# imkaywu/MVSKit

Hardware: AMD Instinct MI355X
Metric: patches/s (propagate+optim iteration), 12-view 1080p (higher is better)
Workload: dtype f32

## Files before the change

include/mvskit_engine.h:

```cpp
#ifndef MVSKIT_ENGINE_H
#define MVSKIT_ENGINE_H

#include <stddef.h>
#include <stdint.h>

#ifdef __cplusplus
extern "C" {
#endif

#ifndef MVS_MAX_IMAGES
#define MVS_MAX_IMAGES 32
#endif
#define MVS_LIST_CAP 16

typedef enum mvs_status {
    MVS_OK = 0,
    MVS_ERR_ARG = -1,
    MVS_ERR_STATE = -2,
    MVS_ERR_HIP = -3,
    MVS_ERR_CAPACITY = -4,
    MVS_ERR_NO_DEVICE = -5
} mvs_status;

typedef struct mvs_patch {
// ... 141 lines not shown
typedef struct mvs_fused_point {
    float xyz[3];
    float normal[3];
    float conf;
    uint8_t rgb[3];
    uint8_t view;
} mvs_fused_point;
int mvs_engine_fused_points(mvs_engine* e, const mvs_maps_config* c, int64_t cap, mvs_fused_point* out , int64_t* n);

typedef struct mvs_volume {
    float origin[3];
    float voxel;
    int32_t dims[3];
    float trunc;
    int32_t min_count;
    int32_t pad;
} mvs_volume;
int mvs_engine_tsdf(mvs_engine* e, const mvs_maps_config* c, const mvs_volume* vol, float* tsdf , int32_t* count );
int mvs_engine_extract_mesh(mvs_engine* e, const mvs_volume* vol, const float* tsdf, const int32_t* count , int64_t cap_v,
                            float* verts , int64_t cap_t, int32_t* tris , int64_t* n_v, int64_t* n_t);
int mvs_engine_mesh(mvs_engine* e, const mvs_maps_config* c, const mvs_volume* vol, int64_t cap_v, float* verts, int64_t cap_t, int32_t* tris,
                    int64_t* n_v, int64_t* n_t);

int mvs_engine_propagate(mvs_engine* e, int iter, mvs_counters* out);

int mvs_engine_filter(mvs_engine* e, int64_t* removed4);
typedef struct mvs_filter_stats {
    float outside_ms, exact_ms, neighbor_ms, groups_ms;
    float rebuild_ms;
    float total_ms;
    int64_t patches_in;
    int64_t exact_patches;
    int64_t exact_view_evals;
    int64_t neighbor_patches;
    int64_t neighbor_tasks;
    int64_t neighbor_entries;
    int64_t neighbor_visited;
    int64_t neighbor_accepted;
    int64_t neighbor_retried;
    int64_t exchange_bytes;
} mvs_filter_stats;
int mvs_engine_filter_stats(mvs_engine* e, mvs_filter_stats* out);

int mvs_engine_pass(mvs_engine* e, int iter, int pass, mvs_counters* out);
int mvs_engine_export_counts(mvs_engine* e, int64_t* n_new, int64_t* n_kill, int32_t* per_view_new );
int mvs_engine_export_device(mvs_engine* e, void* d_new_records, int64_t cap_new, void* d_kill_ids, int64_t cap_kill);
int mvs_engine_commit_device(mvs_engine* e, const void* d_new_records, int64_t n_new, const void* d_kill_ids, int64_t n_kill);
int mvs_engine_commit_local(mvs_engine* e);

#define MVS_COMM_ID_BYTES 128
int mvs_comm_unique_id(void* id_out );
int mvs_engine_comm_init(mvs_engine* e, const void* id , int rank, int world);
int mvs_engine_comm_attach(mvs_engine* e, void* nccl_comm , int rank, int world);
int mvs_engine_comm_release(mvs_engine* e);
int mvs_engine_exchange(mvs_engine* e);
int mvs_engine_comm_info(mvs_engine* e, int* rank, int* world, int* comm_count, int* comm_rank);

int mvs_engine_depth_normal_map(mvs_engine* e, int view, int kind, float* depth, float* normal, int32_t* ids);

typedef enum mvs_probe_op {
    MVS_PROBE_NCC = 0,
    MVS_PROBE_PREPROCESS = 1,
    MVS_PROBE_REFINE = 2,
    MVS_PROBE_POSTPROCESS = 3,
    MVS_PROBE_COST = 4,
    MVS_PROBE_MATH = 5,
    MVS_PROBE_REFINE_X = 6
} mvs_probe_op;
int mvs_engine_probe(mvs_engine* e, int op, int64_t n, const mvs_patch* in_rec, const float* in_f,
                     mvs_patch* out_rec, float* out_f, int32_t* out_i);

typedef struct mvs_timing {
    float index_ms;
    float sweep_ms;
    float commit_ms;
    int32_t sweep_launches;
    float exchange_ms;
    int32_t sweep_jobs_listed;
    int64_t exchange_bytes;
    int64_t check_retried_cells;
} mvs_timing;
int mvs_engine_last_timing(mvs_engine* e, mvs_timing* t);

#ifdef __cplusplus
}
#endif
#endif
```

mvskit_amd/csrc/mvs_device.cuh:

```cuda
#pragma once
#include <hip/hip_runtime.h>
#include <limits.h>
#include "mvs_types.h"

namespace mvsdev {

struct F3 { float x, y, z; };
struct F4 { float x, y, z, w; };

#define DEV __device__ __forceinline__

DEV int lane_id() { return (int)(threadIdx.x & 63u); }
DEV float fma_(float a, float b, float c) { return __builtin_fmaf(a, b, c); }
DEV int rli(int x, int l) { return __builtin_amdgcn_readlane(x, l); }
DEV float rlf(float x, int l) { return __int_as_float(__builtin_amdgcn_readlane(__float_as_int(x), l)); }
DEV int rfl(int x) { return __builtin_amdgcn_readfirstlane(x); }
DEV unsigned long long ballot(bool p) { return __ballot(p); }
#if MVS_LISTCAP > 32
typedef unsigned long long vmask_t;
DEV int vpop(vmask_t m) { return __popcll(m); }
#define MVS_VBITS 64
#else
typedef unsigned vmask_t;
DEV int vpop(vmask_t m) { return __popc(m); }
// ... 69 lines not shown
#define MVS_PIO4 0.78539816339744830962f
#define MVS_PI 3.14159265358979323846f
DEV float k_sinf(float x) {
    float z = x * x;
    float p = -1.9515295891e-4f * z + 8.3321608736e-3f;
    p = p * z - 1.6666654611e-1f;
    return x + x * z * p;
}
DEV float k_cosf(float x) {
    float z = x * x;
    float p = 2.443315711809948e-5f * z - 1.388731625493765e-3f;
    p = p * z + 4.166664568298827e-2f;
    return (1.0f - 0.5f * z) + z * z * p;
}
DEV float pm_sinf(float x) {
    float a = fabsf(x), r;
    if (a <= MVS_PIO4) r = k_sinf(a);
    else if (a <= 3.0f * MVS_PIO4) r = k_cosf((MVS_PIO2_HI - a) + MVS_PIO2_LO);
    else r = k_sinf(MVS_PI - a);
    return x < 0.0f ? -r : r;
}
DEV float pm_cosf(float x) {
    float a = fabsf(x);
    if (a <= MVS_PIO4) return k_cosf(a);
    if (a <= 3.0f * MVS_PIO4) return k_sinf((MVS_PIO2_HI - a) + MVS_PIO2_LO);
    return -k_cosf(MVS_PI - a);
}
DEV void pm_sincosf(float x, float& s, float& c) {
    const float a = fabsf(x);
    const bool r0 = a <= MVS_PIO4, r1 = a <= 3.0f * MVS_PIO4;
    const float t = r0 ? a : (r1 ? (MVS_PIO2_HI - a) + MVS_PIO2_LO : MVS_PI - a);
    const float ks = k_sinf(t), kc = k_cosf(t);
    const float sr = (r0 || !r1) ? ks : kc;
    s = x < 0.0f ? -sr : sr;
    c = r0 ? kc : (r1 ? ks : -kc);
}
DEV float pm_asinf(float x) {
    float a = fabsf(x);
    if (a > 1.0f) a = 1.0f;
    float z, xx;
    bool flag = a > 0.5f;
    if (flag) { z = 0.5f * (1.0f - a); xx = sqrt_rn(z); }
    else { z = a * a; xx = a; }
    float p = 4.2163199048e-2f * z + 2.4181311049e-2f;
    p = p * z + 4.5470025998e-2f;
    p = p * z + 7.4953002686e-2f;
    p = p * z + 1.6666752422e-1f;
    float r = p * z * xx + xx;
    if (flag) { r = r + r; r = (MVS_PIO2_HI - r) + MVS_PIO2_LO; }
    return x < 0.0f ? -r : r;
}
DEV float pm_acosf(float x) {
    if (x < -0.5f) return MVS_PI - 2.0f * pm_asinf(sqrt_rn(0.5f * (1.0f + x)));
    if (x > 0.5f) return 2.0f * pm_asinf(sqrt_rn(0.5f * (1.0f - x)));
    return MVS_PIO2_HI - pm_asinf(x);
}
DEV float pm_atanf(float v) {
    float x = fabsf(v), y;
    if (x > 2.414213562373095f) { y = MVS_PIO2_HI; x = -(1.0f / x); }
    else if (x > 0.4142135623730950f) { y = MVS_PIO4; x = (x - 1.0f) / (x + 1.0f); }
    else y = 0.0f;
    float z = x * x;
    float p = 8.05374449538e-2f * z - 1.38776856032e-1f;
    p = p * z + 1.99777106478e-1f;
    p = p * z - 3.33329491539e-1f;
    y = y + (p * z * x + x);
    return v < 0.0f ? -y : y;
}

DEV uint32_t mix32(uint32_t h) {
    h ^= h >> 16; h *= 0x7feb352du; h ^= h >> 15; h *= 0x846ca68bu; h ^= h >> 16;
    return h;
}
DEV float rng_uniform(uint32_t seed, uint32_t a, uint32_t b, uint32_t c, uint32_t d, uint32_t e) {
    uint32_t h = mix32(seed ^ 0x9e3779b9u);
    h = mix32(h ^ a) + 0x85ebca6bu;
    h = mix32(h ^ b) + 0xc2b2ae35u;
    h = mix32(h ^ c) + 0x27d4eb2fu;
    h = mix32(h ^ d) + 0x165667b1u;
    h = mix32(h ^ e);
    return (float)(h >> 8) * (1.0f / 16777216.0f) - 0.5f;
}

DEV F3 project(const DView* vw, F4 X, int level) {
    const float* P = vw->P[level];
    float r0 = fma_(P[3], X.w, fma_(P[2], X.z, fma_(P[1], X.y, P[0] * X.x)));
    float r1 = fma_(P[7], X.w, fma_(P[6], X.z, fma_(P[5], X.y, P[4] * X.x)));
    float r2 = fma_(P[11], X.w, fma_(P[10], X.z, fma_(P[9], X.y, P[8] * X.x)));
    if (r2 <= 0.0f) return {-65535.0f, -65535.0f, -1.0f};
    const float lo = (float)(INT_MIN + 3.0f), hi = (float)(INT_MAX - 3.0f);
    const float inv = rcp_rn(r2);
    F3 ic{r0 * inv, r1 * inv, 1.0f};
    ic.x = fmaxf(lo, fminf(hi, ic.x));
    ic.y = fmaxf(lo, fminf(hi, ic.y));
    return ic;
}
DEV F3 project_regs(const float (&P)[12], F4 X) {
    const float r0 = fma_(P[3], X.w, fma_(P[2], X.z, fma_(P[1], X.y, P[0] * X.x)));
    const float r1 = fma_(P[7], X.w, fma_(P[6], X.z, fma_(P[5], X.y, P[4] * X.x)));
    const float r2 = fma_(P[11], X.w, fma_(P[10], X.z, fma_(P[9], X.y, P[8] * X.x)));
    const float lo = (float)(INT_MIN + 3.0f), hi = (float)(INT_MAX - 3.0f);
    const float inv = rcp_rn(r2);
    F3 ic{fmaxf(lo, fminf(hi, r0 * inv)), fmaxf(lo, fminf(hi, r1 * inv)), 1.0f};
    if (r2 <= 0.0f) ic = {-65535.0f, -65535.0f, -1.0f};
    return ic;
}
DEV void load_P(const DView* vw, int level, float (&P)[12]) {
#pragma unroll
    for (int k = 0; k < 12; ++k) P[k] = vw->P[level][k];
}
DEV F4 unproject(const DView* vw, F3 ic, int level) {
    const float* P = vw->P[level];
    const float* M = vw->Minv;
    F3 b{ic.x - P[3], ic.y - P[7], ic.z - P[11]};
    return {fma_(M[2], b.z, fma_(M[1], b.y, M[0] * b.x)), fma_(M[5], b.z, fma_(M[4], b.y, M[3] * b.x)),
            fma_(M[8], b.z, fma_(M[7], b.y, M[6] * b.x)), 1.0f};
}
DEV float get_unit(const DParams& prm, const DView* vw, F4 coord) {
    const float fz = norm4(sub4(coord, ld4(vw->center)));
    const float ips = vw->ipscale;
    if (ips == 0.0f) return 1.0f;
    return div_rn(2.0f * fz * (float)(1 << prm.level), ips);
}
DEV void cell_of(const DParams& prm, const DView* vw, F4 coord, int& ix, int& iy) {
    float P[12];
    load_P(vw, prm.level, P);
    const F3 ic = project_regs(P, coord);
    ix = ((int)floorf(ic.x + 0.5f)) / prm.csize;
    iy = ((int)floorf(ic.y + 0.5f)) / prm.csize;
}
template <int LANE> DEV float row_bcast_f(float x) {
    return __int_as_float(__builtin_amdgcn_update_dpp(0, __float_as_int(x), 0x150 + LANE, 0xf, 0xf, false));
}
DEV void get_paxes(const DParams& prm, const DView* vw, F4 coord, F4 normal, F4& px, F4& py) {
    const F4 ctr = ld4(vw->center);
    const float ips = vw->ipscale;
    const F3 xax = ld3(vw->xaxis);
    float P[12];
    load_P(vw, prm.level, P);
    float pscale = 1.0f;
    if (ips != 0.0f) pscale = div_rn(2.0f * norm4(sub4(coord, ctr)) * (float)(1 << prm.level), ips);
    F3 n3{normal.x, normal.y, normal.z};
    F3 y3 = cross3(n3, xax);
    y3 = nrm3(y3);
    F3 x3 = cross3(y3, n3);
    px = {x3.x * pscale, x3.y * pscale, x3.z * pscale, 0.0f};
    py = {y3.x * pscale, y3.y * pscale, y3.z * pscale, 0.0f};
    const int j = lane_id() & 15;
    const float a = j == 1 ? 1.0f : 0.0f, b = j == 2 ? 1.0f : 0.0f;
    const F4 X{fma_(b, py.x, fma_(a, px.x, coord.x)), fma_(b, py.y, fma_(a, px.y, coord.y)), fma_(b, py.z, fma_(a, px.z, coord.z)), coord.w};
    const F3 ic = project_regs(P, X);
    const F3 c0{row_bcast_f<0>(ic.x), row_bcast_f<0>(ic.y), row_bcast_f<0>(ic.z)};
    const float inv = rcp_rn(norm3(sub3(ic, c0)));
    px = scl4(px, row_bcast_f<1>(inv));
    py = scl4(py, row_bcast_f<2>(inv));
}
DEV float robustincc(float incc) { return div_rn(incc, 1 + 3 * incc); }
DEV float unrobustincc(float r) { return div_rn(r, 1 - 3 * r); }

struct Frame {
    float tlx, tly, dxx, dxy, dyx, dyy;
    int w;
    int ok;
    unsigned img_lo, img_hi;
};
DEV int level_diff(const DParams& prm, float ratio) {
    static_assert(0x3504F3 == (0x3FB504F3 & 0x7FFFFF), "mantissa of 1.414213562373095f");
    const int k = ((__float_as_int(ratio) + (0x800000 - 0x3504F3)) >> 23) - 127;
    const int ld = max(-4, min(2, k));
    return max(-prm.level, min(2, ld));
}
DEV float pow2_level(int ld) { return __int_as_float((127 + ld) << 23); }
DEV Frame make_frame(const DParams& prm, F4 coord, F4 px, F4 py, F4 pz, int v, bool active) {
    const DView* vw = prm.views + (active ? v : 0);
    const F4 ctr = ld4(vw->center);
    float P[12];
#pragma unroll
    for (int k = 0; k < 12; ++k) P[k] = vw->P[prm.level][k];
    const int W0 = vw->W[0], H0 = vw->H[0];
    const unsigned long long base_level = (unsigned long long)vw->img[prm.level];
    const F4 ray = nrm4(sub4(ctr, coord));
    const float weight = fmaxf(0.0f, dot4(ray, pz));
    F3 center = project_regs(P, coord);
    F3 dx = sub3(project_regs(P, add4(coord, px)), center);
    F3 dy = sub3(project_regs(P, add4(coord, py)), center);
    const float ratio = (norm3(dx) + norm3(dy)) / 2.0f;
    const int ld = level_diff(prm, ratio);
    const float iscale = pow2_level(-ld);
    const int newLevel = prm.level + ld;
    const unsigned long long base_new = (unsigned long long)vw->img[newLevel];
    center = scl3(center, iscale);
    dx = scl3(dx, iscale);
    dy = scl3(dy, iscale);
    const float m = (float)(prm.wsize / 2);
    const float ax = dx.x * m, bx = dy.x * m, ay = dx.y * m, by = dy.y * m;
    const float tlx = (center.x - ax) - bx, tly = (center.y - ay) - by;
    const float minx = (center.x - fabsf(ax)) - fabsf(bx), maxx = (center.x + fabsf(ax)) + fabsf(bx);
    const float miny = (center.y - fabsf(ay)) - fabsf(by), maxy = (center.y + fabsf(ay)) + fabsf(by);
    const int margin2 = 2;
    const int W = W0 >> newLevel, H = H0 >> newLevel;
    const bool inside = !(minx < margin2 || W - 1 - margin2 <= maxx || miny < margin2 || H - 1 - margin2 <= maxy);
    const bool ok = active && !(weight < prm.cosAngle1) && inside;
    Frame f;
    f.tlx = ok ? tlx : 0.0f; f.tly = ok ? tly : 0.0f;
    f.dxx = ok ? dx.x : 0.0f; f.dxy = ok ? dx.y : 0.0f; f.dyx = ok ? dy.x : 0.0f; f.dyy = ok ? dy.y : 0.0f;
    f.w = ok ? W : (W0 >> prm.level);
    f.ok = ok ? 1 : 0;
    const unsigned long long a = ok ? base_new : base_level;
    f.img_lo = (unsigned)(a & 0xffffffffull); f.img_hi = (unsigned)(a >> 32);
    return f;
}

struct __attribute__((packed, aligned(4))) Texel2 { uint32_t a, b; };

struct ClsConst {
    unsigned cs[3];
    int fb;
    int xbase, nx;
};
struct WaveCtx {
    int lane;
    ClsConst cc;
    unsigned evals, view_evals;
#ifdef MVS_STAGE_TIMING
    unsigned long long st_acc[8];
    unsigned long long st_t;
#endif
};
#ifdef MVS_STAGE_TIMING
#define WC_T0(wc) { (wc).st_t = (unsigned long long)__builtin_amdgcn_s_memtime(); }
#define WC_ADD(wc, k) { const unsigned long long t1_ = (unsigned long long)__builtin_amdgcn_s_memtime(); (wc).st_acc[k] += t1_ - (wc).st_t; (wc).st_t = t1_; }
#else
#define WC_T0(wc)
#define WC_ADD(wc, k)
#endif

#define MVS_PIVOT_LDS4 192
#define MVS_FRAME_LDS_BYTES (64 * 48 + 16 * 16)
// ... 73 lines not shown
#define MVS_ROW_STEP(x, C) x = x + dpp_f<C>(x);
#define MVS_ROW_STEP5(C) { const float t0 = dpp0_f<C>(s1r), t1 = dpp0_f<C>(s1g), t2 = dpp0_f<C>(s1b), t3 = dpp0_f<C>(s2), t4 = dpp0_f<C>(s01); \
                           s1r = s1r + t0; s1g = s1g + t1; s1b = s1b + t2; s2 = s2 + t3; s01 = s01 + t4; }
#define MVS_ROW_STEP4(C) { const float t0 = dpp0_f<C>(s1r), t1 = dpp0_f<C>(s1g), t2 = dpp0_f<C>(s1b), t3 = dpp0_f<C>(s2); \
                           s1r = s1r + t0; s1g = s1g + t1; s1b = s1b + t2; s2 = s2 + t3; }
DEV void eval_steps4(const DParams& prm, WaveCtx& wc, const ClsConst& cc, const Frame& f, int n, unsigned (&okm)[4], float& incc_l) {
    frames_publish(wc, f, 64);
    const unsigned long long okb = ballot(f.ok != 0);
#pragma unroll
    for (int g = 0; g < 4; ++g) okm[g] = (unsigned)((okb >> (16 * g)) & 0xffffull);
#pragma unroll
    for (int g = 0; g < 4; ++g) wc.view_evals += (okm[g] & 1u) ? (unsigned)__popc(okm[g]) : 0u;
    const int fb = cc.fb;
    const int lc = wc.lane & 15;
    float c0[3][3];
    ClsPend pend[3];
    float P1r, P1g, P1b, P2, P01 = 0.0f;
    const int vlast = max(n - 1, 0);
    {
        const ClsFrame fr = cls_frame(fb);
#pragma unroll
        for (int j = 0; j < 3; ++j) pend[j] = cls_issue(fr, cls_opaque(cc.cs[j]));
    }
    {
        const float4 pv = mvs_dyn_lds4[MVS_PIVOT_LDS4];
        const ClsFrame fn = cls_frame(fb + min(1, vlast));
        float s1r = 0.0f, s1g = 0.0f, s1b = 0.0f, s2 = 0.0f;
#pragma unroll
        for (int j = 0; j < 3; ++j) {
            const unsigned cs = cls_opaque(cc.cs[j]);
            float r, g, b;
            cls_colour(pend[j], cs, pv.x, pv.y, pv.z, r, g, b);
            pend[j] = cls_issue(fn, cs);
            c0[j][0] = r; c0[j][1] = g; c0[j][2] = b;
            s1r += r; s1g += g; s1b += b;
            s2 = fma_(r, r, s2); s2 = fma_(g, g, s2); s2 = fma_(b, b, s2);
        }
        MVS_ROW_STEP4(0xB1) MVS_ROW_STEP4(0x4E) MVS_ROW_STEP4(0x141) MVS_ROW_STEP4(0x140)
        P1r = s1r; P1g = s1g; P1b = s1b; P2 = s2;
    }
    for (int k = 1; k < n; ++k) {
        const float4 pv = mvs_dyn_lds4[MVS_PIVOT_LDS4 + k];
        const ClsFrame fn = cls_frame(fb + min(k + 1, vlast));
        float s1r = 0.0f, s1g = 0.0f, s1b = 0.0f, s2 = 0.0f, s01 = 0.0f;
#pragma unroll
        for (int j = 0; j < 3; ++j) {
            const unsigned cs = cls_opaque(cc.cs[j]);
            float r, g, b;
            cls_colour(pend[j], cs, pv.x, pv.y, pv.z, r, g, b);
            pend[j] = cls_issue(fn, cs);
            s1r += r; s1g += g; s1b += b;
            s2 = fma_(r, r, s2); s2 = fma_(g, g, s2); s2 = fma_(b, b, s2);
            s01 = fma_(r, c0[j][0], s01); s01 = fma_(g, c0[j][1], s01); s01 = fma_(b, c0[j][2], s01);
        }
        MVS_ROW_STEP5(0xB1) MVS_ROW_STEP5(0x4E) MVS_ROW_STEP5(0x141) MVS_ROW_STEP5(0x140)
        if (lc == k) { P1r = s1r; P1g = s1g; P1b = s1b; P2 = s2; P01 = s01; }
    }
    const int a0 = (wc.lane & 48) << 2;
    if (cc.nx > 0) {
        const float4 pv = mvs_dyn_lds4[MVS_PIVOT_LDS4 + lc];
        ClsFrame fr;
        fr.tlx = f.tlx; fr.tly = f.tly; fr.dxx = f.dxx; fr.dxy = f.dxy; fr.dyx = f.dyx; fr.dyy = f.dyy; fr.w = f.w;
        fr.base = ((unsigned long long)f.img_hi << 32) | (unsigned long long)f.img_lo;
        {
            const int q = cc.xbase;
            const unsigned cs = (unsigned)(q % prm.wsize) | ((unsigned)(q / prm.wsize) << 8) | (1u << 16);
            const ClsPend pe = cls_issue(fr, cs);
            float r, g, b;
            cls_colour(pe, cs, pv.x, pv.y, pv.z, r, g, b);
            const float r0 = bperm_f(a0, r), g0 = bperm_f(a0, g), b0 = bperm_f(a0, b);
            P1r += r; P1g += g; P1b += b;
            P2 = fma_(r, r, P2); P2 = fma_(g, g, P2); P2 = fma_(b, b, P2);
            P01 = fma_(r, r0, P01); P01 = fma_(g, g0, P01); P01 = fma_(b, b0, P01);
        }
    }
    const float m_r = P1r * prm.inv_sz, m_g = P1g * prm.inv_sz, m_b = P1b * prm.inv_sz;
    const float ssd = fmaxf(P2 - fma_(P1b, m_b, fma_(P1g, m_g, P1r * m_r)), 0.0f);
    const float inv_l = inv_msd(prm, ssd);
    const float m0r = bperm_f(a0, m_r), m0g = bperm_f(a0, m_g), m0b = bperm_f(a0, m_b), inv0 = bperm_f(a0, inv_l);
    const float dot = P01 - fma_(P1b, m0b, fma_(P1g, m0g, P1r * m0r));
    incc_l = 1.0f - (dot * (inv0 * inv_l)) * prm.inv_3sz;
}

DEV void cls_raw(const ClsPend& p, unsigned cs, float& r, float& g, float& b) {
    const Texel2 q0 = p.q0, q1 = p.q1;
    const float fm = cvt_ub2(cs);
    const float dx1 = p.dx1 * fm, dx0 = fm - dx1, dy1 = p.dy1, dy0 = 1.0f - dy1;
    const float f00 = dx0 * dy0, f01 = dx0 * dy1, f10 = dx1 * dy0, f11 = dx1 * dy1;
    r = fma_((float)(q1.b & 255u), f11, fma_((float)(q0.b & 255u), f10, fma_((float)(q1.a & 255u), f01, (float)(q0.a & 255u) * f00)));
    g = fma_((float)((q1.b >> 8) & 255u), f11, fma_((float)((q0.b >> 8) & 255u), f10, fma_((float)((q1.a >> 8) & 255u), f01, (float)((q0.a >> 8) & 255u) * f00)));
    b = fma_((float)((q1.b >> 16) & 255u), f11, fma_((float)((q0.b >> 16) & 255u), f10, fma_((float)((q1.a >> 16) & 255u), f01, (float)((q0.a >> 16) & 255u) * f00)));
}
#define MVS_ROW_STEP3(C) { const float t0 = dpp0_f<C>(s1r), t1 = dpp0_f<C>(s1g), t2 = dpp0_f<C>(s1b); s1r = s1r + t0; s1g = s1g + t1; s1b = s1b + t2; }
#define MVS_ROW_STEP2(C) { const float t0 = dpp0_f<C>(sq), t1 = dpp0_f<C>(dt); sq = sq + t0; dt = dt + t1; }

#define MVS_PAIR_MFMA (MVS_LISTCAP > 16)
#if MVS_PAIR_MFMA
#define MVS_GRAM_SCRATCH (MVS_LISTCAP > 32 ? 2 : 1)
#define MVS_GRAM_CH 16
#define MVS_GRAM_NCH (MVS_LISTCAP / 16)
#define MVS_GRAM_NT (MVS_GRAM_NCH * (MVS_GRAM_NCH + 1) / 2)
#define MVS_GRAM_KSP 40
#define MVS_GRAM_T(p, c) ((c) * ((c) + 1) / 2 + (p))
#define MVS_GRAM_KK 4
#define MVS_GRAM_KS ((147 + MVS_GRAM_KK - 1) / MVS_GRAM_KK)
#define MVS_GRAM_NACC 4
typedef float gram_acc_t __attribute__((ext_vector_type(MVS_GRAM_NACC)));
DEV gram_acc_t gram_mfma(float a, float b, gram_acc_t c) { return __builtin_amdgcn_mfma_f32_16x16x4f32(a, b, c, 0, 0, 0); }
DEV int gram_col(int lane) { return lane & 15; }
DEV int gram_row(int lane, int r) { return (lane >> 4) * 4 + r; }
template <int N> struct GramIC { static constexpr int value = N; };
#endif
template <bool PIV = false>
DEV void eval_views(const DParams& prm, WaveCtx& wc, const Frame& f, int n, vmask_t (&okm)[1], float& incc_l, float* piv = nullptr,
                    float* texs = nullptr, int tstride = 0, float* ssd_out = nullptr) {
#if MVS_PAIR_MFMA
#if MVS_GRAM_SCRATCH == 2
    float gops[MVS_GRAM_NCH * MVS_GRAM_KSP];
#elif MVS_GRAM_SCRATCH
    gram_acc_t gacc[MVS_GRAM_NT];
    float gops[(MVS_GRAM_NCH - 1) * MVS_GRAM_KSP];
#pragma unroll
    for (int q = 0; q < MVS_GRAM_NT; ++q)
#pragma unroll
        for (int r = 0; r < MVS_GRAM_NACC; ++r) gacc[q][r] = 0.0f;
#endif
    const int gK = 3 * prm.wsz, gtp = 3 * tstride;
    const int gk0 = wc.lane / MVS_GRAM_CH;
    const float* const grow = texs + (wc.lane & (MVS_GRAM_CH - 1)) * gtp;
#endif
    const ClsConst& cc = wc.cc;
    frames_publish(wc, f, MVS_LISTCAP > 16 ? MVS_LISTCAP : 16);
    okm[0] = vballot(f.ok != 0);
    wc.view_evals += (okm[0] & 1u) ? (unsigned)vpop(okm[0]) : 0u;
    const int row = wc.lane >> 4, lc = wc.lane & 15;
    float fxr = 0.0f, fxg = 0.0f, fxb = 0.0f;
    unsigned xcs = 0u;
    ClsPend pe;
    if (cc.nx > 0) {
        ClsFrame fr;
        fr.tlx = f.tlx; fr.tly = f.tly; fr.dxx = f.dxx; fr.dxy = f.dxy; fr.dyx = f.dyx; fr.dyy = f.dyy; fr.w = f.w;
        fr.base = ((unsigned long long)f.img_hi << 32) | (unsigned long long)f.img_lo;
        xcs = (unsigned)(cc.xbase % prm.wsize) | ((unsigned)(cc.xbase / prm.wsize) << 8) | (1u << 16);
        pe = cls_issue(fr, xcs);
    }
    float d0[3][3], d0x[3] = {0.0f, 0.0f, 0.0f};
    float ssd_l = 1.0f, dot_l = 0.0f, mr_l = 128.0f, mg_l = 128.0f, mb_l = 128.0f;
    ClsPend pend[3];
    {
        const int last = max(n - 1, 0);
        const ClsFrame fr = cls_frame(min(row, last));
#pragma unroll
        for (int j = 0; j < 3; ++j) pend[j] = cls_issue(fr, cls_opaque(cc.cs[j]));
    }
    if (cc.nx > 0) cls_raw(pe, xcs, fxr, fxg, fxb);
    const int rounds = (n + 3) >> 2;
    auto round_body = [&](const int t) {
        const int v = 4 * t + row, vq = min(v, max(n - 1, 0));
        const ClsFrame fn = cls_frame(min(v + 4, max(n - 1, 0)));
        float cr[3], cg[3], cb[3];
        float s1r = 0.0f, s1g = 0.0f, s1b = 0.0f;
#pragma unroll
        for (int j = 0; j < 3; ++j) {
            const unsigned cs = cls_opaque(cc.cs[j]);
            cls_raw(pend[j], cs, cr[j], cg[j], cb[j]);
            pend[j] = cls_issue(fn, cs);
// ... 491 lines not shown
    float incc_l;
    fv[1] = fv[2] = fv[3] = 2.0;
    if (four) {
        wc.evals += (unsigned)__popc(rows);
        unsigned okm[4];
        eval_steps4(prm, wc, *cc, f, sz, okm, incc_l);
        const float val_l = robustincc(incc_l);
        const int gl = wc.lane & 3;
        const unsigned okl = gl == 1 ? okm[1] : (gl == 2 ? okm[2] : (gl == 3 ? okm[3] : okm[0]));
        double num = 0.0;
        int den = 0;
        for (int i = 1; i < sz; ++i) {
            const float v = bperm_f(4 * (16 * gl + i), val_l);
            const bool ok = (okl >> i) & 1u;
            num = ok ? num + (double)v : num;
            den += ok ? 1 : 0;
        }
        const double q = num / (double)den;
#pragma unroll
        for (int j = 0; j < 4; ++j) fv[j] = ((okm[j] & 1u) && rli(den, j) >= minimum - 1) ? rld(q, j) : 2.0;
    } else {
        wc.evals += 1;
        vmask_t okm[1];
        if (piv) eval_views<true>(prm, wc, f, sz, okm, incc_l, piv);
        else eval_views(prm, wc, f, sz, okm, incc_l);
        const float val_l = robustincc(incc_l);
        fv[0] = cost_of_group(prm, wc, (unsigned)okm[0], val_l, 0, sz, minimum);
    }
}
DEV void refine_patch(const DParams& prm, WaveCtx& wc, Cand& c, uint32_t k0, uint32_t k1, uint32_t k2, uint32_t k3, float* w_out = nullptr) {
    RefineCtx rc;
    rc.center = c.coord;
    rc.ref = rli(c.img, 0);
    rc.ray = nrm4(sub4(c.coord, ld4((prm.views + rc.ref)->center)));
    rc.dscale = c.dscale;
    rc.ascale = prm.ascaleConst;
    const float w = compute_weights(prm, wc, c.coord, c.normal, c.img, c.nimg);
    const int imgx = __shfl(c.img, wc.lane & 15);
    float x[3];
    encode(prm, rc, c.coord, c.normal, x);
    const float amin = -23.99999f, amax = 23.99999f;
    x[1] = fmaxf(fminf(x[1], amax), amin);
    x[2] = fmaxf(fminf(x[2], amax), amin);
    float bx0 = x[0], bx1 = x[1], bx2 = x[2];
    double fv[4];
    float piv[3] = {128.0f, 128.0f, 128.0f};
    cost_func4(prm, wc, rc, imgx, c.nimg, false, bx0, bx1, bx2, fv, piv);
    __syncthreads();
    if (wc.lane < 16) mvs_dyn_lds4[MVS_PIVOT_LDS4 + wc.lane] = make_float4(piv[0], piv[1], piv[2], 0.0f);
    __syncthreads();
    double fbest = fv[0];
    const ClsConst cc = wc.cc;
    float rd = prm.rd0, ra = prm.ra0;
    const int g = wc.lane >> 4;
    const uint32_t gj = (uint32_t)min(g, 2);
    for (int k = 0; k < prm.refine_steps; ++k) {
        const uint32_t draw = 16u + ((uint32_t)(k * 3) + gj) * 3u;
        const float u0 = 2.0f * rng_uniform(prm.seed, k0, k1, k2, k3, draw + 0);
        const float u1 = 2.0f * rng_uniform(prm.seed, k0, k1, k2, k3, draw + 1);
        const float u2 = 2.0f * rng_uniform(prm.seed, k0, k1, k2, k3, draw + 2);
        float cx0 = (gj == 1u) ? bx0 : fma_(u0, rd, bx0);
        float cx1 = (gj == 0u) ? bx1 : fmaxf(fminf(fma_(u1, ra, bx1), amax), amin);
        float cx2 = (gj == 0u) ? bx2 : fmaxf(fminf(fma_(u2, ra, bx2), amax), amin);
        if (g == 3) {
            cx0 = bx0 - (cx0 - bx0);
            cx1 = fmaxf(fminf(bx1 - (cx1 - bx1), amax), amin);
            cx2 = fmaxf(fminf(bx2 - (cx2 - bx2), amax), amin);
        }
        cost_func4(prm, wc, rc, imgx, c.nimg, true, cx0, cx1, cx2, fv, nullptr, &cc);
        int jb = 0;
        double fstep = fv[0];
#pragma unroll
        for (int j = 1; j < 4; ++j) if (fv[j] < fstep) { fstep = fv[j]; jb = j; }
        if (fstep < fbest) { fbest = fstep; bx0 = rlf(cx0, 16 * jb); bx1 = rlf(cx1, 16 * jb); bx2 = rlf(cx2, 16 * jb); }
        rd *= 0.5f; ra *= 0.5f;
    }
    x[0] = bx0; x[1] = bx1; x[2] = bx2;
    decode(prm, rc, x[0], x[1], x[2], c.coord, c.normal);
    c.normal.w = 0.0f;
    if (w_out) *w_out = w;
    else c.ncc = 1.0f - unrobustincc(compute_incc(prm, wc, c.coord, c.normal, c.img, c.nimg, w, 1));
}

DEV int refine_patch_simplex(const DParams& prm, WaveCtx& wc, Cand& c, int max_evals, float xtol, float* w_out = nullptr,
                               float* x_out = nullptr, double* f_out = nullptr) {
    RefineCtx rc;
    rc.center = c.coord;
    rc.ref = rli(c.img, 0);
    rc.ray = nrm4(sub4(c.coord, ld4((prm.views + rc.ref)->center)));
    rc.dscale = c.dscale;
    rc.ascale = prm.ascaleConst;
    const float w = compute_weights(prm, wc, c.coord, c.normal, c.img, c.nimg);
    const int imgx = __shfl(c.img, wc.lane & 15);
    float x[3];
    encode(prm, rc, c.coord, c.normal, x);
    const float amin = -23.99999f, amax = 23.99999f;
    x[1] = fmaxf(fminf(x[1], amax), amin);
    x[2] = fmaxf(fminf(x[2], amax), amin);
    double fv[4];
    float piv[3] = {128.0f, 128.0f, 128.0f};
    cost_func4(prm, wc, rc, imgx, c.nimg, false, x[0], x[1], x[2], fv, piv);
    __syncthreads();
    if (wc.lane < 16) mvs_dyn_lds4[MVS_PIVOT_LDS4 + wc.lane] = make_float4(piv[0], piv[1], piv[2], 0.0f);
    __syncthreads();
    const double f0 = fv[0];
    const ClsConst cc = wc.cc;
    const int g = wc.lane >> 4;
    float vx0 = g == 1 ? x[0] + prm.rd0 : x[0];
    float vx1 = g == 2 ? fmaxf(fminf(x[1] + prm.ra0, amax), amin) : x[1];
    float vx2 = g == 3 ? fmaxf(fminf(x[2] + prm.ra0, amax), amin) : x[2];
    cost_func4(prm, wc, rc, imgx, c.nimg, true, vx0, vx1, vx2, fv, nullptr, &cc, 0xEu);
    double vf = g == 0 ? f0 : (g == 1 ? fv[1] : (g == 2 ? fv[2] : fv[3]));
    int evals = 4;
    bool ok = false;
    int b = 0;
    for (;;) {
        double f[4];
#pragma unroll
        for (int j = 0; j < 4; ++j) f[j] = rld(vf, 16 * j);
        b = 0;
        int wv = 0;
#pragma unroll
        for (int j = 1; j < 4; ++j) {
            if (f[j] < (b == 1 ? f[1] : (b == 2 ? f[2] : f[0]))) b = j;
            if (f[j] >= (wv == 1 ? f[1] : (wv == 2 ? f[2] : f[0]))) wv = j;
        }
        const float b0 = rlf(vx0, 16 * b), b1 = rlf(vx1, 16 * b), b2 = rlf(vx2, 16 * b);
        {
            float lo0 = rlf(vx0, 0), hi0 = lo0, lo1 = rlf(vx1, 0), hi1 = lo1, lo2 = rlf(vx2, 0), hi2 = lo2;
#pragma unroll
            for (int j = 1; j < 4; ++j) {
                const float a0 = rlf(vx0, 16 * j), a1 = rlf(vx1, 16 * j), a2 = rlf(vx2, 16 * j);
                lo0 = fminf(lo0, a0); hi0 = fmaxf(hi0, a0);
                lo1 = fminf(lo1, a1); hi1 = fmaxf(hi1, a1);
                lo2 = fminf(lo2, a2); hi2 = fmaxf(hi2, a2);
            }
            if (hi0 - lo0 <= xtol * fmaxf(1.0f, fabsf(b0)) && hi1 - lo1 <= xtol * fmaxf(1.0f, fabsf(b1)) &&
                hi2 - lo2 <= xtol * fmaxf(1.0f, fabsf(b2))) { ok = true; break; }
        }
        if (evals + 4 > max_evals) break;
        const double fb = rld(vf, 16 * b), fw = rld(vf, 16 * wv);
        double fsw = wv == 0 ? f[1] : f[0];
#pragma unroll
        for (int j = 0; j < 4; ++j) if (j != wv) fsw = fmax(fsw, f[j]);
        const int r0 = wv == 0 ? 1 : 0, r1 = wv <= 1 ? 2 : 1, r2 = wv <= 2 ? 3 : 2;
        const float c0 = ((rlf(vx0, 16 * r0) + rlf(vx0, 16 * r1)) + rlf(vx0, 16 * r2)) / 3.0f;
        const float c1 = ((rlf(vx1, 16 * r0) + rlf(vx1, 16 * r1)) + rlf(vx1, 16 * r2)) / 3.0f;
        const float c2 = ((rlf(vx2, 16 * r0) + rlf(vx2, 16 * r1)) + rlf(vx2, 16 * r2)) / 3.0f;
        const float d0 = c0 - rlf(vx0, 16 * wv), d1 = c1 - rlf(vx1, 16 * wv), d2 = c2 - rlf(vx2, 16 * wv);
        const float k = g == 0 ? 1.0f : (g == 1 ? 2.0f : (g == 2 ? 0.5f : -0.5f));
        const float t0 = c0 + k * d0;
        const float t1 = fmaxf(fminf(c1 + k * d1, amax), amin);
        const float t2 = fmaxf(fminf(c2 + k * d2, amax), amin);
        cost_func4(prm, wc, rc, imgx, c.nimg, true, t0, t1, t2, fv, nullptr, &cc);
        evals += 4;
        int acc = -1;
        if (fv[0] < fb) acc = fv[1] < fv[0] ? 1 : 0;
        else if (fv[0] < fsw) acc = 0;
        else if (fv[0] < fw) acc = fv[2] <= fv[0] ? 2 : -1;
        else acc = fv[3] < fw ? 3 : -1;
        if (acc >= 0) {
            const float a0 = rlf(t0, 16 * acc), a1 = rlf(t1, 16 * acc), a2 = rlf(t2, 16 * acc);
            const double fa = acc == 0 ? fv[0] : (acc == 1 ? fv[1] : (acc == 2 ? fv[2] : fv[3]));
            if (g == wv) { vx0 = a0; vx1 = a1; vx2 = a2; vf = fa; }
            continue;
        }
// ... 288 lines not shown
```

mvskit_amd/csrc/mvs_engine.cpp:

```cpp
#include <hip/hip_runtime.h>
#include <dlfcn.h>
#include <rccl/rccl.h>

#include <algorithm>
#include <climits>
#include <cmath>
#include <cstdio>
#include <cstdlib>
#include <cstring>
#include <string>
#include <vector>

#include "mvskit_engine.h"
#include "mvs_kernels.h"
#include "mvs_types.h"

static_assert(sizeof(mvs_patch) == sizeof(DPatch), "mvs_patch and DPatch must be the same bytes");
static_assert((MVS_LISTCAP == 16 || MVS_LISTCAP == 32 || MVS_LISTCAP == 64) && MVS_LISTCAP <= MVS_MAXI && MVS_MAX_IMAGES == MVS_MAXI, "limits out of sync");

namespace {
thread_local std::string g_err;

#define HIPCHK(expr)                                                                                       \
    do {                                                                                                   \
// ... 89 lines not shown
    MVS_SYM(GroupEnd, "ncclGroupEnd"); MVS_SYM(GetErrorString, "ncclGetErrorString");
    MVS_SYM(CommCount, "ncclCommCount"); MVS_SYM(CommUserRank, "ncclCommUserRank");
#undef MVS_SYM
    r.ok = r.GetUniqueId && r.CommInitRank && r.CommDestroy && r.AllGather && r.Broadcast && r.GroupStart && r.GroupEnd && r.GetErrorString;
    return r;
}
#define NCCLCHK(expr)                                                                                      \
    do {                                                                                                   \
        ncclResult_t _r = (expr);                                                                          \
        if (_r != ncclSuccess) {                                                                           \
            g_err = std::string(#expr) + ": " + rccl().GetErrorString(_r);                                 \
            return MVS_ERR_HIP;                                                                            \
        }                                                                                                  \
    } while (0)

struct Roctx {
    int (*push)(const char*) = nullptr;
    int (*pop)() = nullptr;
};
Roctx& roctx() {
    static Roctx r;
    static bool tried = false;
    if (tried) return r;
    tried = true;
    void* h = nullptr;
    const char* names[] = {"libroctx64.so", "libroctx64.so.4", "/opt/rocm/lib/libroctx64.so.4"};
    for (const char* n : names) if (!h) h = dlopen(n, RTLD_NOW | RTLD_NOLOAD);
    for (const char* n : names) if (!h) h = dlopen(n, RTLD_NOW | RTLD_LOCAL);
    if (!h) return r;
    r.push = reinterpret_cast<int (*)(const char*)>(dlsym(h, "roctxRangePushA"));
    r.pop = reinterpret_cast<int (*)()>(dlsym(h, "roctxRangePop"));
    if (!r.push || !r.pop) { r.push = nullptr; r.pop = nullptr; }
    return r;
}
struct Range {
    bool on;
    explicit Range(const char* name) : on(roctx().push != nullptr) { if (on) roctx().push(name); }
    ~Range() { if (on) roctx().pop(); }
    Range(const Range&) = delete;
    Range& operator=(const Range&) = delete;
};
}

struct mvs_engine {
    mvs_config cfg{};
    mvs_refiner refiner{MVS_REFINE_HALVING, 500, 1e-4f};
    DParams prm{};
    hipStream_t stream = nullptr;
    bool have_views = false;
    std::vector<DView> hviews;
    DevBuf<DView> dviews;
    std::vector<DevBuf<uint32_t>> img_bufs;
    std::vector<DevBuf<uint8_t>> mask_bufs;
    int total_cells = 0;
    DevBuf<DPatch> pool, pool_alt;
    DevBuf<uint8_t> kill;
    int64_t pool_n = 0;
    bool ncc_dirty = false;
    DevBuf<int32_t> cnt, cursor, vcnt, vcursor;
    DevBuf<csr_off_t> start, vstart;
    DevBuf<csr_off_t> start_raw;
    DevBuf<int32_t> id32_raw;
    DevBuf<int64_t> scan_tmp;
    DevBuf<unsigned long long> ids;
    DevBuf<ListKey> key;
    DevBuf<int32_t> id32, vid32;
    DevBuf<int32_t> uf_parent, uf_size;
    DevBuf<int32_t> group_edges;
    DevBuf<int32_t> cnt_alive, vcnt_alive;
    DevBuf<unsigned long long> dpgrid, best;
    DevBuf<uint32_t> dirty;
    bool dirty_marked = false;
    DevBuf<float4> geo;
    DevBuf<uint8_t> geo_ref;
    bool geo_valid = false;
    bool lists_dense[2] = {false, false};
    DevBuf<DPatch> staging;
    DevBuf<int32_t> job_stage, job_nstage, job_cnt, job_base_scan, kill_cnt, kill_base;
    DevBuf<unsigned long long> misc;
    DevBuf<DCounters> counters;
    DevBuf<int32_t> error_flag;
    DevBuf<int32_t> big_tables, retry_jobs;
    DevBuf<int32_t> job_list;
    int64_t retried_cells = 0;
    int64_t pass_retried = 0;
    SweepArgs sa{};
    bool staged = false;
    bool counted = false;
    int64_t n_new = 0, n_kill = 0;
    std::vector<int32_t> h_per_view;
    DevBuf<DPatch> tmp_rec_in, tmp_rec_out;
    DevBuf<float> tmp_f_in, tmp_f_out;
    DevBuf<int32_t> tmp_i;
    DevBuf<uint8_t> tmp_bytes;
    hipEvent_t ev[6] = {nullptr, nullptr, nullptr, nullptr, nullptr, nullptr};
    mvs_timing timing{};
    mvs_filter_stats fstats{};
    int64_t fstats_exchange_bytes = 0;
    DevBuf<unsigned long long> fstat_buf;
    hipEvent_t fev[10] = {nullptr, nullptr, nullptr, nullptr, nullptr, nullptr, nullptr, nullptr, nullptr, nullptr};
    ncclComm_t comm = nullptr;
    bool comm_owned = false;
    int comm_rank = 0, comm_world = 1;
    DevBuf<int64_t> comm_counts;
    DevBuf<int32_t> comm_kill_ids;
    int pass_status = MVS_OK;
    std::string pass_error;
    bool fault_fired = false;
};

namespace {

RefineSel refine_sel(const mvs_engine* e) {
    return RefineSel{e->refiner.mode == MVS_REFINE_CONVERGED ? 1 : 0, e->refiner.max_evals, e->refiner.xtol};
}

void derive_params(mvs_engine* e) {
    const mvs_config& c = e->cfg;
    DParams& p = e->prm;
    p.nviews = c.nviews; p.level = c.level; p.csize = c.csize; p.wsize = c.wsize; p.wsz = c.wsize * c.wsize;
    p.minImageNum = c.minImageNum;
    p.tau = std::min(c.minImageNum * 2, c.nviews);
    p.max_propag = c.max_propag;
    p.cap = c.max_propag * c.csize * c.csize;
    p.depth = c.depth; p.enable_check = c.enable_check; p.view_propagation = c.view_propagation ? 1 : 0;
    p.seed = c.seed; p.refine_steps = c.refine_steps; p.rd0 = c.refine_rd0; p.ra0 = c.refine_ra0;
    p.nccThreshold = c.nccThreshold;
    p.nccThresholdBefore = c.nccThreshold - 0.3f;
    volatile float a0 = (float)(60.0f * M_PI / 180.0f), a1 = (float)(60.0f * M_PI / 180.0f);
    volatile double amin = (double)c.maxAngleThreshold, amax = (double)a1;
    volatile float typo = (float)(120.0f / M_PI * 180.0f);
    volatile double d120 = 120.0f * M_PI / 180.0f, d10 = 10.0f * M_PI / 180.0f;
    p.cosAngle0 = cosf(a0);
    p.cosAngle1 = cosf(a1);
    p.cosMinAngle = (float)cos(amin);
    p.cosMaxAngle = (float)cos(amax);
    p.cosNeighborTypo = cosf(typo);
    p.cosNeighbor120 = (float)cos(d120);
    p.sortThreshold = (float)(1.0f - cos(d10));
    p.ascaleConst = (float)(M_PI / 48.0f);
    p.inv_sz = 1.0f / (float)(c.wsize * c.wsize);
    p.inv_3sz = 1.0f / (float)(3 * c.wsize * c.wsize);
    p.neighborThreshold = 0.5f; p.neighborThreshold1 = 1.0f;
    p.quadThreshold = c.quadThreshold;
    p.list_n = std::min<int>(MVS_LISTCAP, c.nviews);
    p.gram_ld = (p.list_n + 15) / 16 * 16;
}

void invert3(const float* P, float* Minv) {
    double a = P[0], b = P[1], c = P[2], d = P[4], e = P[5], f = P[6], g = P[8], h = P[9], i = P[10];
    double A = e * i - f * h, B = -(d * i - f * g), C = d * h - e * g;
    double det = a * A + b * B + c * C;
    double inv[9] = {A, -(b * i - c * h), b * f - c * e, B, a * i - c * g, -(a * f - c * d), C, -(a * h - b * g), a * e - b * d};
    for (int k = 0; k < 9; ++k) Minv[k] = (float)(inv[k] / det);
}
inline float hfma(float a, float b, float c) { return __builtin_fmaf(a, b, c); }
inline float hdot3(const float* a, const float* b) { return hfma(a[2], b[2], hfma(a[1], b[1], a[0] * b[0])); }
inline float hdot4(const float* a, const float* b) { return hfma(a[3], b[3], hfma(a[2], b[2], hfma(a[1], b[1], a[0] * b[0]))); }
inline void hcross(const float* a, const float* b, float* o) {
    o[0] = a[1] * b[2] - a[2] * b[1]; o[1] = a[2] * b[0] - a[0] * b[2]; o[2] = a[0] * b[1] - a[1] * b[0];
}

void setup_camera(const mvs_engine* e, DView& vw, const float* P0) {
    const int maxLevel = e->cfg.level + 3;
    for (int k = 0; k < 12; ++k) vw.P[0][k] = P0[k];
    for (int l = 1; l < maxLevel; ++l) {
// ... 1398 lines not shown
        a.sweep_views[a.nsweep_views] = v;
        a.job_base[a.nsweep_views] = (int32_t)nj;
        ++a.nsweep_views;
        nj += (int64_t)((e->hviews[v].gw + 1) / 2) * e->hviews[v].gh;
    }
    a.njobs = nj;
    a.job_lo = 0; a.job_hi = nj;
    if (ranged) {
        const int split_mode = getenv("MVS_SPLIT_PROXY") ? atoi(getenv("MVS_SPLIT_PROXY")) : 2;
        const int N = e->cfg.shard_count, R = e->cfg.shard_index;
        std::vector<int32_t> cuts(N + 1, -1);
        int64_t total_work = 0;
        if (split_mode > 0 && nj > 0) {
            const DParams p0 = current_params(e);
            int shift = 0;
            while ((((int64_t)3 * e->prm.cap * e->prm.max_propag * 32 * nj) >> shift) + nj >= (int64_t)INT32_MAX) ++shift;
            mvsk_job_work(p0, a, split_mode, shift, e->job_cnt.p, st);
            mvsk_exclusive_scan(e->job_cnt.p, e->job_base_scan.p, nj, reinterpret_cast<int32_t*>(e->scan_tmp.p), st);
            if (int r = e->tmp_i.ensure(N + 1)) return r;
            HIPCHK(hipMemsetAsync(e->tmp_i.p, 0xff, (size_t)(N + 1) * sizeof(int32_t), st));
            mvsk_job_cuts(e->job_base_scan.p, nj, N, e->tmp_i.p, st);
            int32_t tw = 0;
            HIPCHK(hipMemcpyAsync(cuts.data(), e->tmp_i.p, (size_t)(N + 1) * sizeof(int32_t), hipMemcpyDeviceToHost, st));
            HIPCHK(hipMemcpyAsync(&tw, e->job_base_scan.p + nj, sizeof tw, hipMemcpyDeviceToHost, st));
            HIPCHK(hipStreamSynchronize(st));
            total_work = tw;
        }
        cuts[0] = 0; cuts[N] = (int32_t)nj;
        for (int r = 1; r < N; ++r) {
            if (total_work <= 0 || cuts[r] < 0) cuts[r] = (int32_t)(nj * r / N);
            cuts[r] = std::max(cuts[r], cuts[r - 1]);
        }
        a.job_lo = cuts[R];
        a.job_hi = cuts[R + 1];
    }
    a.staging = e->staging.p; a.staging_cap = e->staging.cap;
    a.stage_counter = e->misc.p + misc::stage_counter;
    a.job_stage = e->job_stage.p; a.job_nstage = e->job_nstage.p;
    a.maxstage = (e->prm.view_propagation ? 3 : 2) * e->prm.cap * e->prm.max_propag;
    a.kill = e->kill.p;
    a.counters = e->counters.p;
    a.error_flag = e->error_flag.p;
    if (want_vgrid(e)) {
        if (int r = e->big_tables.ensure((int64_t)256 * 16384)) return r;
        if (int r = e->retry_jobs.ensure(std::max<int64_t>(nj, 16))) return r;
    }
    a.big_tables = e->big_tables.p; a.retry_jobs = e->retry_jobs.p; a.nretry = reinterpret_cast<int32_t*>(e->misc.p + misc::sweep_retry);
    HIPCHK(hipMemsetAsync(e->misc.p + misc::sweep_retry, 0, sizeof(unsigned long long), st));
    HIPCHK(hipMemsetAsync(e->misc.p + misc::stage_counter, 0, sizeof(unsigned long long), st));
    a.cursors = reinterpret_cast<uint32_t*>(e->misc.p + misc::sweep_cursors);
    HIPCHK(hipMemsetAsync(e->misc.p + misc::sweep_cursors, 0, (misc::sweep_cursor_words + misc::sweep_list_bound_words) * sizeof(unsigned long long), st));
    HIPCHK(hipMemsetAsync(e->counters.p, 0, MVS_COUNTER_SLOTS * sizeof(DCounters), st));
    HIPCHK(hipMemsetAsync(e->error_flag.p, 0, sizeof(int32_t), st));
    const DParams p = current_params(e);
    const RefineSel rs = refine_sel(e);
    if (int r = e->job_list.ensure(std::max<int64_t>(nj, 16))) return r;
    if (e->job_cnt.ensure(nj + misc::job_list_pad) || e->job_base_scan.ensure(nj + misc::job_list_pad)) return MVS_ERR_HIP;
    int32_t* list_bounds = reinterpret_cast<int32_t*>(e->misc.p + misc::sweep_list_bounds);
    a.job_list = e->job_list.p; a.list_bounds = list_bounds;
    mvsk_job_list(p, a, e->job_cnt.p, e->job_base_scan.p, reinterpret_cast<int32_t*>(e->scan_tmp.p), e->job_list.p, list_bounds, st);
    HIPCHK(hipEventRecord(e->ev[1], st));
    Range rg_sweep(pass & 1 ? "mvs:sweep colour 1" : "mvs:sweep colour 0");
    mvsk_sweep(p, a, rs, st);
    e->pass_retried = 0;
    if (want_vgrid(e)) {
        int32_t nretry = 0;
        HIPCHK(hipMemcpyAsync(&nretry, a.nretry, sizeof nretry, hipMemcpyDeviceToHost, st));
        HIPCHK(hipStreamSynchronize(st));
        e->pass_retried = nretry;
        if (nretry > 0) { mvsk_sweep_retry(p, a, nretry, rs, st); e->retried_cells += nretry; }
    }
    HIPCHK(hipEventRecord(e->ev[2], st));
    std::vector<DCounters> hcs(MVS_COUNTER_SLOTS);
    int32_t herr = 0;
    unsigned long long fill[2] = {0, 0};
    HIPCHK(hipMemcpyAsync(fill, e->misc.p + misc::fill_evals, sizeof fill, hipMemcpyDeviceToHost, st));
    HIPCHK(hipMemcpyAsync(hcs.data(), e->counters.p, hcs.size() * sizeof(DCounters), hipMemcpyDeviceToHost, st));
    HIPCHK(hipMemcpyAsync(&herr, e->error_flag.p, sizeof herr, hipMemcpyDeviceToHost, st));
    int32_t hbounds[MVS_SWEEP_QUEUES + 1];
    HIPCHK(hipMemcpyAsync(hbounds, list_bounds, sizeof hbounds, hipMemcpyDeviceToHost, st));
    HIPCHK(hipStreamSynchronize(st));
    HIPCHK(hipGetLastError());
    mvs_counters sum{};
    for (const DCounters& c : hcs) add_counters(sum, c);
    sum.evals += fill[0]; sum.view_evals += fill[1]; sum.trimmed = (int64_t)trimmed;
    float ms = 0.0f;
    (void)hipEventElapsedTime(&ms, e->ev[0], e->ev[1]); e->timing.index_ms = ms;
    (void)hipEventElapsedTime(&ms, e->ev[1], e->ev[2]); e->timing.sweep_ms = ms;
    e->timing.commit_ms = 0.0f; e->timing.sweep_launches = 1; e->timing.exchange_ms = 0.0f; e->timing.exchange_bytes = 0;
    e->timing.check_retried_cells = e->pass_retried;
    e->timing.sweep_jobs_listed = hbounds[MVS_SWEEP_QUEUES];
    e->staged = true; e->counted = false;
    if (out) *out = sum;
#ifdef MVS_JOBLIST_COUNTS
    fprintf(stderr, "[job list] iter %d colour %d: jobs %lld, with any source entry %llu, listed %llu\n", iter, pass & 1, (long long)(a.job_hi - a.job_lo),
            hcs[0].stage[0], hcs[0].stage[1]);
#endif
#ifdef MVS_STAGE_TIMING
    {
        unsigned long long stage[16] = {0};
        for (const DCounters& c : hcs)
            for (int k = 0; k < 16; ++k) stage[k] = (k == 12 || k == 13) ? std::max(stage[k], c.stage[k]) : stage[k] + c.stage[k];
        static const char* nm[8] = {"wave", "generate", "pre", "refine", "post", "check", "stage", "prologue"};
        fprintf(stderr, "[stage cycles]");
        for (int k = 0; k < 8; ++k) fprintf(stderr, " %s %.1f%%", nm[k], 100.0 * (double)stage[k] / (double)(stage[0] ? stage[0] : 1));
        static const char* nm2[4] = {"gain", "search", "sort", "quad"};
        for (int k = 0; k < 4; ++k) fprintf(stderr, " %s %.1f%%", nm2[k], 100.0 * (double)stage[8 + k] / (double)(stage[0] ? stage[0] : 1));
        fprintf(stderr, " setRefImage pairs %.1f%% choice %.1f%%", 100.0 * (double)stage[14] / (double)(stage[0] ? stage[0] : 1), 100.0 * (double)stage[15] / (double)(stage[0] ? stage[0] : 1));
        fprintf(stderr, "  (wave cycles %.3e; max visited %llu, max neighbours %llu)\n", (double)stage[0], stage[12], stage[13]);
    }
#endif
#ifdef MVS_FAULT_INJECTION
    if (const char* f = getenv("MVS_FAULT_PASS")) {
        int fr = -1, fi = -1, fp = -1;
        if (!e->fault_fired && sscanf(f, "%d:%d:%d", &fr, &fi, &fp) == 3 && fr == (e->cfg.shard_count > 1 ? e->cfg.shard_index : 0) && fi == iter && fp == pass) {
            e->fault_fired = true;
            g_err = "mvs_engine_pass: capacity failure injected by MVS_FAULT_PASS";
            return MVS_ERR_CAPACITY;
        }
    }
#endif
    if (herr & 3) { g_err = "mvs_engine_pass: staging capacity exceeded (raise mvs_config.max_patches)"; return MVS_ERR_CAPACITY; }
    if (herr & 4) {
        g_err = "mvs_engine_pass: Optim::check met more than 14336 patches around one patch, or more than 4064 neighbours (engine limit)";
        return MVS_ERR_CAPACITY;
    }
    return MVS_OK;
}

int mvs_engine_export_counts(mvs_engine* e, int64_t* n_new, int64_t* n_kill, int32_t* per_view_new) {
    if (!e || !e->staged) { g_err = "mvs_engine_export_counts: no pass to export"; return MVS_ERR_STATE; }
    HIPCHK(hipSetDevice(e->cfg.device));
    if (int r = ensure_counts(e)) return r;
    if (n_new) *n_new = e->n_new;
    if (n_kill) *n_kill = e->n_kill;
    if (per_view_new) for (int v = 0; v < e->cfg.nviews; ++v) per_view_new[v] = e->h_per_view[v];
    return MVS_OK;
}

int mvs_engine_export_device(mvs_engine* e, void* d_new, int64_t cap_new, void* d_kill, int64_t cap_kill) {
    if (!e || !e->staged) { g_err = "mvs_engine_export_device: no pass to export"; return MVS_ERR_STATE; }
    HIPCHK(hipSetDevice(e->cfg.device));
    if (int r = ensure_counts(e)) return r;
    if (e->n_new > cap_new || e->n_kill > cap_kill) { g_err = "mvs_engine_export_device: buffers too small"; return MVS_ERR_CAPACITY; }
    if (e->n_new > 0) mvsk_commit_copy(e->sa, e->job_base_scan.p, (DPatch*)d_new, cap_new, nullptr, 1, e->stream);
    if (e->n_kill > 0) mvsk_kill_export(e->kill.p, e->pool_n, e->kill_base.p, (int32_t*)d_kill, cap_kill, e->stream);
    HIPCHK(hipStreamSynchronize(e->stream));
    return MVS_OK;
}

int mvs_engine_commit_device(mvs_engine* e, const void* d_new, int64_t n_new, const void* d_kill, int64_t n_kill) {
    if (!e || !e->have_views) return MVS_ERR_STATE;
    HIPCHK(hipSetDevice(e->cfg.device));
    hipStream_t st = e->stream;
    if (e->pool_n + n_new > e->pool.cap) { g_err = "mvs_engine_commit_device: patch pool capacity exceeded (raise mvs_config.max_patches)"; return MVS_ERR_CAPACITY; }
    return commit_pool(e, [&](int64_t* added) -> int {
        mvsk_apply_kill_ids(e->pool.p, (const int32_t*)d_kill, n_kill, e->pool_n, st);
        mvsk_append_records(e->pool.p, e->pool_n, (const DPatch*)d_new, n_new, st);
        if (e->pool_n > 0) HIPCHK(hipMemsetAsync(e->kill.p, 0, (size_t)e->pool_n, st));
        *added = n_new;
        return MVS_OK;
    });
}

int mvs_engine_commit_local(mvs_engine* e) {
    if (!e || !e->staged) { g_err = "mvs_engine_commit_local: no pass to commit"; return MVS_ERR_STATE; }
    HIPCHK(hipSetDevice(e->cfg.device));
// ... 255 lines not shown
            if (fr.live()) mvsk_filter_neighbor_retry(current_params(e), e->kill.p, e->uf_parent.p, nr, e->error_flag.p, e->fstat_buf.p + fstat::neighbor_parts, st);
            FRHIP(hipGetLastError());
            FRHIP(hipEventRecord(e->fev[5], st));
#ifdef MVS_STAGE_TIMING
            if (fr.live()) {
                unsigned long long hc[16] = {0};
                (void)hipMemcpyAsync(hc, e->fstat_buf.p + fstat::neighbor_cycles, sizeof hc, hipMemcpyDeviceToHost, st);
                (void)hipStreamSynchronize(st);
                const double w = (double)(hc[0] ? hc[0] : 1);
                fprintf(stderr, "[filterNeighbor cycles] load + grids %.1f%% set build %.1f%% gather + predicate %.1f%% filterQuad %.1f%% (wave cycles %.3e)\n",
                        100.0 * hc[1] / w, 100.0 * hc[9] / w, 100.0 * hc[10] / w, 100.0 * hc[11] / w, (double)hc[0]);
            }
#endif
        }
        filter_fault_point(fr, 3);
        if (filter_exchange(fr, true, false)) break;
        FR(apply_kills(e, &rem[2], true));
        if (rem[2] > 0) { if (filter_rebuild(fr, 1, false, true, 2)) break; }
        {
            int64_t alive = 0;
            FR(mvs_engine_num_patches(e, &alive));
            FR(e->uf_parent.ensure(e->pool.cap));
            FR(e->uf_size.ensure(e->pool.cap));
            const int threshold = (int)std::max<int64_t>(20, alive / 10000);
            FRHIP(hipEventRecord(e->fev[6], st));
            if (fr.live()) {
                if (!e->cfg.literal_groups) mvsk_groups(current_params(e), e->uf_parent.p, e->uf_size.p, threshold, e->kill.p, st);
                else fr.note(literal_small_groups(e, threshold));
            }
            FRHIP(hipEventRecord(e->fev[7], st));
            FR(apply_kills(e, &rem[3], true));
        }
        if (rem[3] > 0) { if (filter_rebuild(fr, 1, false, false, 2)) break; }
        FR(compact_pool(e));
        FRHIP(hipMemcpyAsync(&herr, e->error_flag.p, sizeof herr, hipMemcpyDeviceToHost, st));
        FRHIP(hipEventRecord(e->ev[1], st));
        FRHIP(hipStreamSynchronize(st));
        FRHIP(hipGetLastError());
        if (fr.live() && (herr & 4)) {
            g_err = "mvs_engine_filter: more than 14336 patches around one patch, or more than 4064 neighbours (engine limit)";
            fr.note(MVS_ERR_CAPACITY);
        }
    } while (0);
    const int status = filter_agree(fr);
    e->geo_valid = false;
    if (status != MVS_OK) {
        const std::string keep = g_err;
        if (e->kill.p && e->pool_n > 0) (void)hipMemsetAsync(e->kill.p, 0, (size_t)e->pool_n, st);
        (void)hipStreamSynchronize(st);
        (void)hipGetLastError();
        e->dirty_marked = false;
        g_err = keep;
        return status;
    }
    float ms = 0.0f;
    (void)hipEventElapsedTime(&ms, e->ev[0], e->ev[1]);
    e->timing = mvs_timing{};
    e->timing.index_ms = ms;
    {
        mvs_filter_stats& f = e->fstats;
        f.total_ms = ms;
        (void)hipEventElapsedTime(&f.outside_ms, e->fev[0], e->fev[1]);
        (void)hipEventElapsedTime(&f.exact_ms, e->fev[2], e->fev[3]);
        (void)hipEventElapsedTime(&f.neighbor_ms, e->fev[4], e->fev[5]);
        (void)hipEventElapsedTime(&f.groups_ms, e->fev[6], e->fev[7]);
        f.rebuild_ms = f.total_ms - f.outside_ms - f.exact_ms - f.neighbor_ms - f.groups_ms;
        std::vector<unsigned long long> part(fstat::neighbor_cycles - fstat::neighbor_parts);
        HIPCHK(hipMemcpy(part.data(), e->fstat_buf.p + fstat::neighbor_parts, part.size() * sizeof(unsigned long long), hipMemcpyDeviceToHost));
        unsigned long long sum4[4] = {0, 0, 0, 0};
        for (size_t k = 0; k < part.size(); ++k) sum4[k & 3] += part[k];
        f.neighbor_tasks = (int64_t)sum4[0]; f.neighbor_entries = (int64_t)sum4[1]; f.neighbor_visited = (int64_t)sum4[2]; f.neighbor_accepted = (int64_t)sum4[3];
    }
    e->fstats.exchange_bytes = e->fstats_exchange_bytes;
    if (removed4) for (int k = 0; k < 4; ++k) removed4[k] = rem[k];
    return MVS_OK;
}

int mvs_engine_filter_stats(mvs_engine* e, mvs_filter_stats* out) {
    if (!e || !out) return MVS_ERR_ARG;
    *out = e->fstats;
    return MVS_OK;
}

int mvs_engine_last_timing(mvs_engine* e, mvs_timing* t) {
    if (!e || !t) return MVS_ERR_ARG;
    *t = e->timing;
    return MVS_OK;
}

int mvs_engine_depth_normal_map(mvs_engine* e, int view, int kind, float* depth, float* normal, int32_t* ids) {
    if (!e || !e->have_views || view < 0 || view >= e->cfg.nviews || kind < 0 || kind > 1) { g_err = "mvs_engine_depth_normal_map: bad argument"; return MVS_ERR_ARG; }
    HIPCHK(hipSetDevice(e->cfg.device));
    hipStream_t st = e->stream;
    const DView& vw = e->hviews[view];
    const int ncells = vw.gw * vw.gh;
    const DParams p = current_params(e);
    const unsigned long long* sel = nullptr;
    if (kind == 0) {
        HIPCHK(hipMemsetAsync(e->dpgrid.p, 0xff, (size_t)e->total_cells * sizeof(unsigned long long), st));
        mvsk_depth_maps(p, e->dpgrid.p, nullptr, st);
        sel = e->dpgrid.p + vw.cell_base;
    } else {
        HIPCHK(hipMemsetAsync(e->best.p, 0, (size_t)ncells * sizeof(unsigned long long), st));
        mvsk_best_ncc_map(p, view, e->best.p, st);
        sel = e->best.p;
    }
    if (e->tmp_f_out.ensure((int64_t)ncells * 4) || e->tmp_i.ensure(ncells)) return MVS_ERR_HIP;
    mvsk_map_extract(p, view, kind, sel, e->tmp_f_out.p, e->tmp_f_out.p + ncells, e->tmp_i.p, ncells, st);
    if (depth) HIPCHK(hipMemcpyAsync(depth, e->tmp_f_out.p, (size_t)ncells * sizeof(float), hipMemcpyDeviceToHost, st));
    if (normal) HIPCHK(hipMemcpyAsync(normal, e->tmp_f_out.p + ncells, (size_t)ncells * 3 * sizeof(float), hipMemcpyDeviceToHost, st));
    if (ids) HIPCHK(hipMemcpyAsync(ids, e->tmp_i.p, (size_t)ncells * sizeof(int32_t), hipMemcpyDeviceToHost, st));
    HIPCHK(hipStreamSynchronize(st));
    return MVS_OK;
}

int mvs_engine_probe(mvs_engine* e, int op, int64_t n, const mvs_patch* in_rec, const float* in_f, mvs_patch* out_rec, float* out_f, int32_t* out_i) {
    if (!e || !e->have_views || n < 0 || op < 0 || op > 6) { g_err = "mvs_engine_probe: bad argument / views not set"; return MVS_ERR_ARG; }
    const RefineSel rs = refine_sel(e);
    if (op == MVS_PROBE_REFINE_X && !rs.simplex) { g_err = "mvs_engine_probe: MVS_PROBE_REFINE_X needs the CONVERGED refiner"; return MVS_ERR_STATE; }
    if (n == 0) return MVS_OK;
    HIPCHK(hipSetDevice(e->cfg.device));
    hipStream_t st = e->stream;
    if (op == MVS_PROBE_POSTPROCESS && e->prm.depth > 0) if (int r = build_index(e, nullptr)) return r;
    const int64_t nf_out = op == MVS_PROBE_MATH ? 5 * n : ((op == MVS_PROBE_REFINE || op == MVS_PROBE_REFINE_X) && rs.simplex ? 4 * n : n);
    if (e->tmp_rec_in.ensure(n) || e->tmp_rec_out.ensure(n) || e->tmp_f_in.ensure(n) || e->tmp_f_out.ensure(nf_out) || e->tmp_i.ensure(n + 1)) return MVS_ERR_HIP;
    if (op == MVS_PROBE_MATH) {
        if (!in_f || !out_f) return MVS_ERR_ARG;
        HIPCHK(hipMemcpyAsync(e->tmp_f_in.p, in_f, (size_t)n * sizeof(float), hipMemcpyHostToDevice, st));
    } else {
        if (!in_rec) return MVS_ERR_ARG;
        HIPCHK(hipMemcpyAsync(e->tmp_rec_in.p, in_rec, (size_t)n * sizeof(mvs_patch), hipMemcpyHostToDevice, st));
    }
    HIPCHK(hipMemsetAsync(e->tmp_i.p, 0, (size_t)(n + 1) * sizeof(int32_t), st));
    const DParams p = current_params(e);
    mvsk_probe(p, op, n, e->tmp_rec_in.p, e->tmp_f_in.p, e->tmp_rec_out.p, e->tmp_f_out.p, e->tmp_i.p, rs, st);
    if (out_rec && (op == MVS_PROBE_PREPROCESS || op == MVS_PROBE_REFINE || op == MVS_PROBE_POSTPROCESS || op == MVS_PROBE_REFINE_X))
        HIPCHK(hipMemcpyAsync(out_rec, e->tmp_rec_out.p, (size_t)n * sizeof(mvs_patch), hipMemcpyDeviceToHost, st));
    if (out_f && (op == MVS_PROBE_NCC || op == MVS_PROBE_COST || op == MVS_PROBE_MATH || op == MVS_PROBE_REFINE_X))
        HIPCHK(hipMemcpyAsync(out_f, e->tmp_f_out.p, (size_t)nf_out * sizeof(float), hipMemcpyDeviceToHost, st));
    if (out_i) HIPCHK(hipMemcpyAsync(out_i, e->tmp_i.p, (size_t)n * sizeof(int32_t), hipMemcpyDeviceToHost, st));
    HIPCHK(hipStreamSynchronize(st));
    HIPCHK(hipGetLastError());
    return MVS_OK;
}

}
```

mvskit_amd/csrc/mvs_kernels.hip:

```cpp
#include <hip/hip_runtime.h>
#include <algorithm>
#include "mvs_device.cuh"
#include "mvs_check.cuh"
#include "mvs_kernels.h"

using namespace mvsdev;

__global__ void k_rgb_to_rgba(const uint8_t* __restrict__ rgb, uint32_t* __restrict__ out, int64_t n) {
    const int64_t i = (int64_t)blockIdx.x * blockDim.x + threadIdx.x;
    if (i >= n) return;
    const uint8_t* p = rgb + 3 * i;
    out[i] = (uint32_t)p[0] | ((uint32_t)p[1] << 8) | ((uint32_t)p[2] << 16);
}
__global__ void k_rgba_to_rgb(const uint32_t* __restrict__ in, uint8_t* __restrict__ rgb, int64_t n) {
    const int64_t i = (int64_t)blockIdx.x * blockDim.x + threadIdx.x;
    if (i >= n) return;
    const uint32_t t = in[i];
    rgb[3 * i] = t & 255u; rgb[3 * i + 1] = (t >> 8) & 255u; rgb[3 * i + 2] = (t >> 16) & 255u;
}
__global__ void k_pyr_down(const uint32_t* __restrict__ src, int pw, int ph, uint32_t* __restrict__ dst, int w, int h) {
    const int x = blockIdx.x * blockDim.x + threadIdx.x, y = blockIdx.y * blockDim.y + threadIdx.y;
    if (x >= w || y >= h) return;
    const float base[4] = {1.0f, 3.0f, 3.0f, 1.0f};
    float c0 = 0.0f, c1 = 0.0f, c2 = 0.0f;
// ... 327 lines not shown
}
__global__ void k_job_work(DParams prm, SweepArgs a, int mode, int shift, int32_t* __restrict__ work) {
    const int64_t job = (int64_t)blockIdx.x * blockDim.x + threadIdx.x;
    if (job >= a.njobs) return;
    int dest;
    const int n = job_trial_sources(prm, a, job, &dest);
    int w = 0;
    if (dest >= 0) {
        if (mode == 1) w = n;
        else {
            const int trials = n * prm.max_propag;
            const int room = max(prm.cap - prm.csr_cnt[dest], 0);
            const int full = min(trials, (room * 5 + 3) / 4);
            w = 32 * full + 2 * (trials - full);
        }
    }
    work[job] = (w + (1 << shift) - 1) >> shift;
}
__global__ void k_job_cuts(const int32_t* __restrict__ scan, int64_t njobs, int n, int32_t* __restrict__ cuts) {
    const int64_t job = (int64_t)blockIdx.x * blockDim.x + threadIdx.x;
    if (job >= njobs) return;
    const long long total = scan[njobs], p0 = scan[job], p1 = scan[job + 1];
    if (p0 == p1) return;
    for (int r = 1; r < n; ++r) {
        const long long target = total * r / n;
        if (p0 <= target && target < p1) cuts[r] = (int32_t)job;
    }
}

#ifndef MVS_XCD_CHUNK
#define MVS_XCD_CHUNK 128
#endif
DEV int64_t list_slot_job(const SweepArgs& a, int64_t slot, int seg) {
    const int64_t q = slot / seg, r = slot % seg;
    return a.job_lo + ((r / MVS_XCD_CHUNK) * MVS_SWEEP_QUEUES + q) * MVS_XCD_CHUNK + r % MVS_XCD_CHUNK;
}
__global__ void k_job_list(DParams prm, SweepArgs a, int seg, int32_t* __restrict__ flags) {
    const int64_t t = (int64_t)blockIdx.x * blockDim.x + threadIdx.x;
    if (t < a.njobs) a.job_nstage[t] = 0;
    if (t >= (int64_t)MVS_SWEEP_QUEUES * seg) return;
    const int64_t job = list_slot_job(a, t, seg);
    int dest = -1;
    const int n = job < a.job_hi ? job_trial_sources(prm, a, job, &dest) : 0;
    flags[t] = n > 0 ? 1 : 0;
#ifdef MVS_JOBLIST_COUNTS
    bool any = false;
    if (dest >= 0) {
        int v, cx, cy;
        job_cell(prm, a, job, v, cx, cy);
        const DView* vw = prm.views + v;
        const int sxs[3] = {cx, cx - a.inc, cx}, sys[3] = {cy - a.inc, cy, cy};
        for (int k = 0; k < (prm.view_propagation ? 3 : 2); ++k)
            if (0 <= sxs[k] && sxs[k] < vw->gw && 0 <= sys[k] && sys[k] < vw->gh) any |= prm.csr_cnt[vw->cell_base + sys[k] * vw->gw + sxs[k]] > 0;
    }
    const unsigned long long m_any = __ballot(any), m_listed = __ballot(n > 0);
    if ((threadIdx.x & 63) == 0) {
        if (m_any) atomicAdd(&a.counters->stage[0], (unsigned long long)__popcll(m_any));
        if (m_listed) atomicAdd(&a.counters->stage[1], (unsigned long long)__popcll(m_listed));
    }
#endif
}
__global__ void k_job_scatter(SweepArgs a, int seg, const int32_t* __restrict__ scan, int32_t* __restrict__ list, int32_t* __restrict__ bounds) {
    const int64_t t = (int64_t)blockIdx.x * blockDim.x + threadIdx.x;
    const int64_t nslots = (int64_t)MVS_SWEEP_QUEUES * seg;
    if (t >= nslots) return;
    const int32_t pos = scan[t];
    if (t % seg == 0) bounds[t / seg] = pos;
    if (t == nslots - 1) bounds[MVS_SWEEP_QUEUES] = scan[nslots];
    if (scan[t + 1] != pos) list[pos] = (int32_t)list_slot_job(a, t, seg);
}

#ifndef MVS_SWEEP_WAVES
#define MVS_SWEEP_WAVES 3
#endif
#ifdef MVS_STAGE_TIMING
#define ST_NOW() ((unsigned long long)__builtin_amdgcn_s_memtime())
#define ST_ADD(k, t0) { const unsigned long long t1_ = ST_NOW(); st_acc[k] += t1_ - (t0); (t0) = t1_; }
#else
#define ST_ADD(k, t0)
#endif
struct SweepAcc {
    unsigned cand, pref, patch, f0, f1, ins, rep;
    unsigned long long evals, view_evals;
#ifdef MVS_STAGE_TIMING
    unsigned long long stage[16];
#endif
};
DEV SweepAcc sweep_acc_zero() {
    SweepAcc acc;
    acc.cand = acc.pref = acc.patch = acc.f0 = acc.f1 = acc.ins = acc.rep = 0u;
    acc.evals = acc.view_evals = 0ull;
#ifdef MVS_STAGE_TIMING
    for (int k = 0; k < 16; ++k) acc.stage[k] = 0ull;
#endif
    return acc;
}
DEV void sweep_acc_flush(const SweepArgs& a, const SweepAcc& acc, unsigned slot) {
    DCounters* C = a.counters + slot;
    if (acc.cand) atomicAdd(&C->candidates, (unsigned long long)acc.cand);
    if (acc.pref) atomicAdd(&C->prefiltered, (unsigned long long)acc.pref);
    if (acc.patch) atomicAdd(&C->patches, (unsigned long long)acc.patch);
    if (acc.f0) atomicAdd(&C->fail0, (unsigned long long)acc.f0);
    if (acc.f1) atomicAdd(&C->fail1, (unsigned long long)acc.f1);
    if (acc.ins) atomicAdd(&C->inserted, (unsigned long long)acc.ins);
    if (acc.rep) atomicAdd(&C->replaced, (unsigned long long)acc.rep);
    if (acc.evals) atomicAdd(&C->evals, acc.evals);
    if (acc.view_evals) atomicAdd(&C->view_evals, acc.view_evals);
#ifdef MVS_STAGE_TIMING
    for (int k = 0; k < 12; ++k) if (acc.stage[k]) atomicAdd(&C->stage[k], acc.stage[k]);
    atomicMax(&C->stage[12], acc.stage[12]); atomicMax(&C->stage[13], acc.stage[13]);
    atomicAdd(&C->stage[14], acc.stage[14]); atomicAdd(&C->stage[15], acc.stage[15]);
#endif
}
template <bool BIG, bool SIMPLEX = false>
DEV void sweep_cell(const DParams& prm, const SweepArgs& a, WaveCtx& wc, SweepAcc* acc, const int64_t job, int* s_scratch, float* s_texs,
                    int* big_table, int max_evals = 0, float xtol = 0.0f) {
#ifdef MVS_STAGE_TIMING
    unsigned long long st_acc[16] = {0, 0, 0, 0, 0, 0, 0, 0, 0, 0, 0, 0, 0, 0, 0, 0};
    const unsigned long long st_begin = ST_NOW();
    unsigned long long st_t = st_begin;
    for (int k = 0; k < 8; ++k) wc.st_acc[k] = 0;
#endif
    int v, cx, cy;
    job_cell(prm, a, job, v, cx, cy);
    const DView* vw = prm.views + v;
    const int gw = vw->gw, gh = vw->gh;
    wc.evals = 0; wc.view_evals = 0;
    const int cell = cy * gw + cx;
    const int inc = a.inc;
    const int sxs[2] = {cx, cx - inc}, sys[2] = {cy - inc, cy};

    const int tstride = prm.wsz;
    unsigned n_cand = 0, n_pref = 0, n_patch = 0, n_f0 = 0, n_f1 = 0, n_ins = 0, n_rep = 0;
    int L_id = -1;
    float L_ncc = 0.0f;
    int L_n = 0;
    {
        const int g = vw->cell_base + cell;
        const csr_off_t fb = prm.csr_start[g];
        L_n = min(prm.csr_cnt[g], MVS_CAPMAX);
        if (wc.lane < L_n) { L_id = pgrid_id(prm, fb + wc.lane); L_ncc = pgrid_ncc(prm, fb + wc.lane); }
    }
    int ns = 0;
    bool gave_up = false;
    const float icx = (float)(prm.csize * (2 * cx + 1) - 1) / 2.0f, icy = (float)(prm.csize * (2 * cy + 1) - 1) / 2.0f;

    const int nsrc = prm.view_propagation ? 3 : 2;
    for (int sidx = 0; sidx < nsrc; ++sidx) {
        const int scx = sidx < 2 ? sxs[sidx] : cx, scy = sidx < 2 ? sys[sidx] : cy;
        if (scx < 0 || gw <= scx || scy < 0 || gh <= scy) continue;
        const int g = vw->cell_base + scy * gw + scx;
        const csr_off_t sb = prm.csr_start[g];
        const int sn = min(prm.csr_cnt[g], MVS_CAPMAX);
        const int as_view = sidx == 2 ? v : -1;
        int E_id = 0;
        bool E_take = false;
        if (wc.lane < sn) { E_id = pgrid_id(prm, sb + wc.lane); E_take = (pgrid_ref(prm, sb + wc.lane) == v) != (sidx == 2); }
        unsigned todo = (unsigned)ballot(E_take);
        while (todo) {
            const int n = __ffs((int)todo) - 1;
            todo &= todo - 1u;
            const DPatch* sp = prm.pool + rli(E_id, n);
            const int srcslot = sidx * prm.cap + n;
            for (int it = 0; it < prm.max_propag; ++it) {
                ST_ADD(7, st_t)
                const int np = L_n;
                const uint32_t k0 = (uint32_t)a.iter, k1 = (uint32_t)v, k2 = (uint32_t)cell, k3 = (uint32_t)(srcslot * 16 + it);
                Cand c;
                int worst = -1;
                float worst_ncc = 0.0f;
                F3 ic;
                if (np < prm.cap) {
                    const float ra = rng_uniform(prm.seed, k0, k1, k2, k3, 0) * (float)prm.csize;
                    const float rb = rng_uniform(prm.seed, k0, k1, k2, k3, 1) * (float)prm.csize;
                    ic = {icx + ra, icy + rb, 1.0f};
                } else {
                    worst = rli(L_id, prm.cap - 1);
                    worst_ncc = rlf(L_ncc, prm.cap - 1);
                    const DPatch* wp = worst >= MVS_NEWBASE ? a.staging + (worst - MVS_NEWBASE) : prm.pool + worst;
                    ic = project(vw, ld4(wp->coord), prm.level);
                }
                {
                    Cand src;
                    load_cand(sp, wc, src);
                    const bool gen_ok = generate_patch(prm, wc, s_scratch, src, ic, c, as_view, np >= prm.cap);
                    ST_ADD(1, st_t)
                    if (!gen_ok) continue;
                }
                ++n_cand;
                if (np >= prm.cap && c.ncc < worst_ncc) { ++n_pref; continue; }
                ++n_patch;
                const int pre_r = pre_process(prm, wc, s_scratch, c);
                ST_ADD(2, st_t)
                if (pre_r == -1) { ++n_f0; continue; }
                float keep_w;
                if constexpr (SIMPLEX) (void)refine_patch_simplex(prm, wc, c, max_evals, xtol, &keep_w);
                else refine_patch(prm, wc, c, k0, k1, k2, k3, &keep_w);
                ST_ADD(3, st_t)
                const int post_r = post_process(prm, wc, s_scratch, s_texs, tstride, c, keep_w, true);
                ST_ADD(4, st_t)
                if (post_r == -1) { ++n_f1; continue; }
                if (prm.depth >= 2 && prm.enable_check) {
                    __syncthreads();
                    if (wc.lane < MVS_CAPMAX) s_scratch[wc.lane] = L_id;
                    __syncthreads();
                    #ifdef MVS_STAGE_TIMING
                    const CheckCtx cx{a.staging, v, cell, L_n, s_scratch, st_acc};
#else
                    const CheckCtx cx{a.staging, v, cell, L_n, s_scratch, nullptr};
#endif
                    const int chk_r = check_patch<BIG>(prm, wc, cx, c, s_texs, a.error_flag, big_table);
                    ST_ADD(5, st_t)
                    if (!BIG && chk_r < 0) { gave_up = true; break; }
                    if (chk_r) { ++n_f1; continue; }
                }
                unsigned long long slot64 = 0;
                if (wc.lane == 0) slot64 = atomicAdd(a.stage_counter, 1ull);
                const int64_t slot = ((int64_t)rfl((int)(slot64 >> 32)) << 32) | (uint32_t)rfl((int)(slot64 & 0xffffffffull));
                if (slot >= a.staging_cap || ns >= a.maxstage) {
                    if (wc.lane == 0) atomicOr(a.error_flag, 1);
                    continue;
                }
                if (np == prm.cap) {
                    if (wc.lane == 0) {
                        if (worst >= MVS_NEWBASE) a.staging[worst - MVS_NEWBASE].flags &= ~1;
                        else a.kill[worst] = 1;
                    }
                    --L_n;
                    ++n_rep;
                } else ++n_ins;
                store_cand(a.staging + slot, wc, c, 1 | (v << 8), cell);
                if (wc.lane == 0) a.job_stage[job * a.maxstage + ns] = (int32_t)slot;
                ++ns;
                const bool lands = ballot(wc.lane < c.nimg && c.img == v && c.gy * gw + c.gx == cell) != 0ull;
                if (lands) {
                    const int nid = MVS_NEWBASE + (int)slot;
                    const int pos = __popcll(ballot(wc.lane < L_n && rank_before(L_ncc, L_id, c.ncc, nid)));
                    const int up_id = __shfl_up(L_id, 1);
                    const float up_ncc = __shfl_up(L_ncc, 1);
                    if (wc.lane > pos) { L_id = up_id; L_ncc = up_ncc; }
                    if (wc.lane == pos) { L_id = nid; L_ncc = c.ncc; }
                    ++L_n;
                }
                ST_ADD(6, st_t)
            }
            if (gave_up) break;
        }
        if (gave_up) break;
    }
    if (!BIG && gave_up) {
        if (wc.lane == 0) { a.job_nstage[job] = 0; a.retry_jobs[atomicAdd(a.nretry, 1)] = (int32_t)job; }
        return;
    }
    if (wc.lane == 0) a.job_nstage[job] = ns;
    {
        acc->cand += n_cand; acc->pref += n_pref; acc->patch += n_patch; acc->f0 += n_f0; acc->f1 += n_f1; acc->ins += n_ins; acc->rep += n_rep;
        acc->evals += wc.evals; acc->view_evals += wc.view_evals;
#ifdef MVS_STAGE_TIMING
        st_acc[0] = ST_NOW() - st_begin;
        for (int k = 0; k < 12; ++k) acc->stage[k] += st_acc[k];
        acc->stage[12] = max(acc->stage[12], st_acc[12]); acc->stage[13] = max(acc->stage[13], st_acc[13]);
        acc->stage[14] += wc.st_acc[3]; acc->stage[15] += wc.st_acc[4];
#endif
    }
}

template <bool SIMPLEX>
DEV void sweep_resident(const DParams& prm, const SweepArgs& a, int* s_scratch, float* s_texs, int max_evals, float xtol) {
    WaveCtx wc = make_wave_ctx(prm);
    SweepAcc acc = sweep_acc_zero();
    for (unsigned step = 0; step < MVS_SWEEP_QUEUES; ++step) {
        const unsigned q = (blockIdx.x + step) & (MVS_SWEEP_QUEUES - 1u);
        const int32_t qbegin = a.list_bounds[q];
        const unsigned ntake = (unsigned)(a.list_bounds[q + 1] - qbegin);
        if (ntake == 0u) continue;
        for (;;) {
            unsigned k = 0;
            if (wc.lane == 0) k = atomicAdd(a.cursors + q * MVS_SWEEP_CURSOR_STRIDE, 1u);
            k = (unsigned)rfl((int)k);
            if (k >= ntake) break;
            const int64_t job = a.job_list[qbegin + (int32_t)k];
            __syncthreads();
            sweep_cell<false, SIMPLEX>(prm, a, wc, &acc, job, s_scratch, s_texs, nullptr, max_evals, xtol);
        }
    }
    if (wc.lane == 0) sweep_acc_flush(a, acc, blockIdx.x & (MVS_COUNTER_SLOTS - 1));
}
__global__ __launch_bounds__(64, MVS_SWEEP_WAVES) void k_sweep(DParams prm, SweepArgs a) {
    __shared__ int s_scratch[192];
    extern __shared__ float s_texs[];
    sweep_resident<false>(prm, a, s_scratch, s_texs, 0, 0.0f);
}
__global__ __launch_bounds__(64, MVS_SWEEP_WAVES) void k_sweep_simplex(DParams prm, SweepArgs a, int max_evals, float xtol) {
    __shared__ int s_scratch[192];
    extern __shared__ float s_texs[];
    sweep_resident<true>(prm, a, s_scratch, s_texs, max_evals, xtol);
}
template <bool SIMPLEX>
DEV void sweep_retry_cell(const DParams& prm, const SweepArgs& a, const int64_t job, int* s_scratch, float* s_texs, int* big_table, int max_evals, float xtol) {
    WaveCtx wc = make_wave_ctx(prm);
    SweepAcc acc = sweep_acc_zero();
    sweep_cell<true, SIMPLEX>(prm, a, wc, &acc, job, s_scratch, s_texs, big_table, max_evals, xtol);
    if (wc.lane == 0) sweep_acc_flush(a, acc, (unsigned)(job & (MVS_COUNTER_SLOTS - 1)));
}
__global__ __launch_bounds__(64, 1) void k_sweep_retry(DParams prm, SweepArgs a, int nretry) {
    __shared__ int s_scratch[192];
    extern __shared__ float s_texs[];
    int* big_table = a.big_tables + (size_t)blockIdx.x * MVS_FILTER2_HASH_CAP;
    for (int k = blockIdx.x; k < nretry; k += gridDim.x) {
        __syncthreads();
        sweep_retry_cell<false>(prm, a, (int64_t)a.retry_jobs[k], s_scratch, s_texs, big_table, 0, 0.0f);
    }
}
__global__ __launch_bounds__(64, 1) void k_sweep_retry_simplex(DParams prm, SweepArgs a, int nretry, int max_evals, float xtol) {
    __shared__ int s_scratch[192];
    extern __shared__ float s_texs[];
    int* big_table = a.big_tables + (size_t)blockIdx.x * MVS_FILTER2_HASH_CAP;
    for (int k = blockIdx.x; k < nretry; k += gridDim.x) {
        __syncthreads();
        sweep_retry_cell<true>(prm, a, (int64_t)a.retry_jobs[k], s_scratch, s_texs, big_table, max_evals, xtol);
    }
}

__global__ void k_commit_count(SweepArgs a, int32_t* __restrict__ cnt) {
    const int64_t job = (int64_t)blockIdx.x * blockDim.x + threadIdx.x;
    if (job >= a.njobs) return;
    const int ns = a.job_nstage[job];
    int c = 0;
    for (int k = 0; k < ns; ++k) c += a.staging[a.job_stage[job * a.maxstage + k]].flags & 1;
    cnt[job] = c;
}
__global__ void k_commit_copy(SweepArgs a, const int32_t* __restrict__ base, DPatch* __restrict__ dst, int64_t dst_cap, int32_t* __restrict__ per_view,
                              int keep_key) {
    const int64_t job = (int64_t)blockIdx.x * blockDim.x + threadIdx.x;
    if (job >= a.njobs) return;
    const int ns = a.job_nstage[job];
    int r = 0;
    for (int k = 0; k < ns; ++k) {
        const DPatch* sp = a.staging + a.job_stage[job * a.maxstage + k];
        if (!(sp->flags & 1)) continue;
        const int64_t o = (int64_t)base[job] + r++;
        if (o >= dst_cap) { atomicOr(a.error_flag, 2); return; }
        const uint4* s4 = reinterpret_cast<const uint4*>(sp);
        uint4* d4 = reinterpret_cast<uint4*>(dst + o);
        for (int w = 0; w < (int)MVS_REC_U4; ++w) d4[w] = s4[w];
        if (per_view) atomicAdd(&per_view[(sp->flags >> 8) & 0xff], 1);
        if (!keep_key) { dst[o].flags = 1; dst[o].id = 0; }
    }
}
__global__ void k_kill_count(const uint8_t* __restrict__ kill, int64_t n, int32_t* __restrict__ cnt) {
    const int64_t i = (int64_t)blockIdx.x * blockDim.x + threadIdx.x;
    if (i < n) cnt[i] = kill[i] ? 1 : 0;
}
__global__ void k_kill_export(const uint8_t* __restrict__ kill, int64_t n, const int32_t* __restrict__ base, int32_t* __restrict__ ids, int64_t cap) {
    const int64_t i = (int64_t)blockIdx.x * blockDim.x + threadIdx.x;
    if (i < n && kill[i] && base[i] < cap) ids[base[i]] = (int32_t)i;
}
__global__ void k_apply_kill_flags(DPatch* pool, uint8_t* kill, int64_t n) {
    const int64_t i = (int64_t)blockIdx.x * blockDim.x + threadIdx.x;
    if (i < n && kill[i]) { pool[i].flags &= ~1; kill[i] = 0; }
}
__global__ void k_apply_kill_ids(DPatch* pool, const int32_t* __restrict__ ids, int64_t n, int64_t pool_n) {
    const int64_t i = (int64_t)blockIdx.x * blockDim.x + threadIdx.x;
    if (i < n && ids[i] >= 0 && ids[i] < pool_n) pool[ids[i]].flags &= ~1;
}
__global__ void k_append_records(DPatch* pool, int64_t pool_n, const DPatch* __restrict__ recs, int64_t n) {
    const int64_t i = (int64_t)blockIdx.x * blockDim.x + threadIdx.x;
    if (i >= n) return;
    const uint4* s4 = reinterpret_cast<const uint4*>(recs + i);
    uint4* d4 = reinterpret_cast<uint4*>(pool + pool_n + i);
    for (int w = 0; w < (int)MVS_REC_U4; ++w) d4[w] = s4[w];
    pool[pool_n + i].flags = 1;
    pool[pool_n + i].id = 0;
}
__global__ void k_alive_count(const DPatch* __restrict__ pool, int64_t n, int32_t* __restrict__ cnt) {
    const int64_t i = (int64_t)blockIdx.x * blockDim.x + threadIdx.x;
    if (i < n) cnt[i] = pool[i].flags & 1;
}
__global__ void k_alive_gather(const DPatch* __restrict__ pool, int64_t n, const int32_t* __restrict__ base, DPatch* __restrict__ out, int64_t cap) {
    const int64_t i = (int64_t)blockIdx.x * blockDim.x + threadIdx.x;
    if (i >= n || !(pool[i].flags & 1) || base[i] >= cap) return;
    const uint4* s4 = reinterpret_cast<const uint4*>(pool + i);
    uint4* d4 = reinterpret_cast<uint4*>(out + base[i]);
    for (int w = 0; w < (int)MVS_REC_U4; ++w) d4[w] = s4[w];
    out[base[i]].id = (int32_t)i;
}

DEV void set_vgrids(const DParams& prm, const WaveCtx& wc, Cand& c) {
    c.vgx = 0; c.vgy = 0;
    if (wc.lane < c.nvimg) cell_of(prm, prm.views + c.vimg, c.coord, c.vgx, c.vgy);
}
DEV void store_lists(DPatch* p, const WaveCtx& wc, const Cand& c) {
    if (wc.lane == 0) { p->nimages = c.nimg; p->nvimages = c.nvimg; }
    if (wc.lane < MVS_MAXI) {
        p->images[wc.lane] = (uint8_t)(wc.lane < c.nimg ? c.img : 0);
        p->vimages[wc.lane] = (uint8_t)(wc.lane < c.nvimg ? c.vimg : 0);
    }
}
template <int GL>
__global__ __launch_bounds__(64) void k_filter_vimages(DParams prm, int additive, int64_t first, int64_t last, const uint32_t* __restrict__ dirty) {
    __shared__ int s_new[64];
    const int lane = (int)threadIdx.x, g = lane / GL, i = lane % GL;
    const int64_t id = first + (int64_t)blockIdx.x * (64 / GL) + g;
// ... 394 lines not shown
    if (i >= n) return;
    WaveCtx wc = make_wave_ctx(prm);
    Cand c;
    load_cand(in + i, wc, c);
    refine_patch(prm, wc, c, 0u, 0u, (uint32_t)i, 0u);
    store_cand(out + i, wc, c, 1, (int)i);
}
__global__ __launch_bounds__(64, MVS_SWEEP_WAVES) void k_probe_refine_simplex(DParams prm, int64_t n, const DPatch* __restrict__ in, DPatch* __restrict__ out,
                                                                              float* __restrict__ out_f, int32_t* __restrict__ out_i, int max_evals, float xtol) {
    const int64_t i = blockIdx.x;
    if (i >= n) return;
    WaveCtx wc = make_wave_ctx(prm);
    Cand c;
    load_cand(in + i, wc, c);
    float x[3];
    double f;
    const int r = refine_patch_simplex(prm, wc, c, max_evals, xtol, nullptr, x, &f);
    store_cand(out + i, wc, c, 1, (int)i);
    if (wc.lane == 0) {
        out_f[4 * i] = x[0]; out_f[4 * i + 1] = x[1]; out_f[4 * i + 2] = x[2]; out_f[4 * i + 3] = (float)f;
        out_i[i] = r;
    }
}

static inline unsigned nblk(int64_t n, int b) { return (unsigned)((n + b - 1) / b); }

void mvsk_rgb_to_rgba(const uint8_t* rgb, uint32_t* out, int64_t n, hipStream_t st) { hipLaunchKernelGGL(k_rgb_to_rgba, dim3(nblk(n, 256)), dim3(256), 0, st, rgb, out, n); }
void mvsk_rgba_to_rgb(const uint32_t* in, uint8_t* rgb, int64_t n, hipStream_t st) { hipLaunchKernelGGL(k_rgba_to_rgb, dim3(nblk(n, 256)), dim3(256), 0, st, in, rgb, n); }
void mvsk_pyr_down(const uint32_t* src, int pw, int ph, uint32_t* dst, int w, int h, hipStream_t st) {
    hipLaunchKernelGGL(k_pyr_down, dim3((w + 63) / 64, (h + 3) / 4), dim3(64, 4), 0, st, src, pw, ph, dst, w, h);
}
void mvsk_mask_down(const uint8_t* src, int pw, int ph, uint8_t* dst, int w, int h, hipStream_t st) {
    hipLaunchKernelGGL(k_mask_down, dim3((w + 63) / 64, (h + 3) / 4), dim3(64, 4), 0, st, src, pw, ph, dst, w, h);
}
void mvsk_mask_binarise(uint8_t* m, int64_t n, hipStream_t st) { hipLaunchKernelGGL(k_mask_binarise, dim3(nblk(n, 256)), dim3(256), 0, st, m, n); }
void mvsk_exclusive_scan(const int32_t* in, int32_t* out, int64_t n, int32_t* tmp, hipStream_t st) { launch_exclusive_scan<int32_t, int32_t>(in, out, n, tmp, st); }
void mvsk_exclusive_scan_off(const int32_t* in, csr_off_t* out, int64_t n, csr_off_t* tmp, hipStream_t st) { launch_exclusive_scan<int32_t, csr_off_t>(in, out, n, tmp, st); }
void mvsk_index_count(const DParams& prm, int32_t* cnt, int32_t* vcnt, unsigned long long* total, hipStream_t st) {
    if (prm.pool_n > 0) hipLaunchKernelGGL(k_index_count, dim3(nblk(prm.pool_n, 256)), dim3(256), 0, st, prm, cnt, vcnt, total);
}
void mvsk_index_fill(const DParams& prm, int vgrid, const csr_off_t* start, int32_t* cursor, unsigned long long* ids, hipStream_t st) {
    if (prm.pool_n > 0) hipLaunchKernelGGL(k_index_fill, dim3(nblk(prm.pool_n, 256)), dim3(256), 0, st, prm, vgrid, start, cursor, ids);
}
void mvsk_index_fill_direct(const DParams& prm, int vgrid, const csr_off_t* start, int32_t* cursor, int32_t* id32, hipStream_t st) {
    if (prm.pool_n > 0) hipLaunchKernelGGL(k_index_fill_direct, dim3(nblk(prm.pool_n, 256)), dim3(256), 0, st, prm, vgrid, start, cursor, id32);
}
void mvsk_index_sort_trim(const DParams& prm, const csr_off_t* start, unsigned long long* ids, int do_trim, unsigned long long* trimmed, hipStream_t st) {
    hipLaunchKernelGGL(k_index_sort_trim, dim3(nblk(prm.total_cells, 256)), dim3(256), 0, st, prm, start, ids, do_trim, trimmed);
}
void mvsk_index_finalize(const DParams& prm, int vgrid, const csr_off_t* start, unsigned long long* ids, int32_t* id32, int32_t* cnt_alive, hipStream_t st) {
    hipLaunchKernelGGL(k_index_finalize, dim3(nblk(prm.total_cells, 256)), dim3(256), 0, st, prm, vgrid, start, ids, id32, cnt_alive);
}
void mvsk_index_pack(const DParams& prm, const csr_off_t* start, const csr_off_t* start2, const int32_t* cnt_alive, const unsigned long long* ids, const int32_t* id32_in,
                     ListKey* key, int32_t* id32_out, hipStream_t st) {
    hipLaunchKernelGGL(k_index_pack, dim3(nblk(prm.total_cells, 256)), dim3(256), 0, st, prm, start, start2, cnt_alive, ids, id32_in, key, id32_out);
}
void mvsk_depth_maps(const DParams& prm, unsigned long long* dp, const uint32_t* dirty, hipStream_t st) {
    if (prm.pool_n > 0) hipLaunchKernelGGL(k_depth_maps, dim3(nblk(prm.pool_n, 64)), dim3(256), 0, st, prm, dp, dirty);
}
void mvsk_depth_mark_dirty(const DParams& prm, const uint8_t* kill, unsigned long long* dp, uint32_t* dirty, hipStream_t st) {
    if (prm.pool_n > 0) hipLaunchKernelGGL(k_depth_mark_dirty, dim3(nblk(prm.pool_n, 64)), dim3(256), 0, st, prm, kill, dp, dirty);
}
void mvsk_best_ncc_map(const DParams& prm, int view, unsigned long long* best, hipStream_t st) {
    if (prm.pool_n > 0) hipLaunchKernelGGL(k_best_ncc_map, dim3(nblk(prm.pool_n, 256)), dim3(256), 0, st, prm, view, best);
}
void mvsk_map_extract(const DParams& prm, int view, int kind, const unsigned long long* sel, float* depth, float* normal, int32_t* ids, int ncells, hipStream_t st) {
    hipLaunchKernelGGL(k_map_extract, dim3(nblk(ncells, 256)), dim3(256), 0, st, prm, view, kind, sel, depth, normal, ids, ncells);
}
void mvsk_fill_ncc(const DParams& prm, unsigned long long* evals, hipStream_t st) {
    if (prm.pool_n > 0) hipLaunchKernelGGL(k_fill_ncc, dim3((unsigned)((prm.pool_n + 63) / 64)), dim3(64), MVS_FRAME_LDS_BYTES, st, prm, evals);
}
size_t mvsk_sweep_lds_bytes(const DParams& prm) {
#if MVS_PAIR_MFMA
    const size_t tex_f = (size_t)MVS_GRAM_CH * 3 * prm.wsz, gram_f = (size_t)prm.gram_ld * prm.gram_ld;
    const size_t texs = MVS_FRAME1_LDS_BYTES + (tex_f > gram_f ? tex_f : gram_f) * sizeof(float);
#else
    const size_t ln = (size_t)prm.list_n;
    const size_t texs = MVS_FRAME1_LDS_BYTES + (ln * 3 * prm.wsz + ln * (ln - 1) / 2) * sizeof(float);
#endif
    const size_t chk = (size_t)MVS_CHECK_LDS_FLOATS * sizeof(float);
    const size_t need = texs > chk ? texs : chk;
    return need > (size_t)MVS_FRAME_LDS_BYTES ? need : (size_t)MVS_FRAME_LDS_BYTES;
}
void mvsk_sweep(const DParams& prm, const SweepArgs& a, const RefineSel& rs, hipStream_t st) {
    const int64_t nloc = a.job_hi - a.job_lo;
    if (nloc <= 0) return;
    static const size_t pad = getenv("MVS_SWEEP_LDS_PAD") ? (size_t)atol(getenv("MVS_SWEEP_LDS_PAD")) : 0;
    const size_t lds = mvsk_sweep_lds_bytes(prm) + pad;
    int dev = 0, cus = 0;
    (void)hipGetDevice(&dev);
    if (hipDeviceGetAttribute(&cus, hipDeviceAttributeMultiprocessorCount, dev) != hipSuccess || cus <= 0) { (void)hipGetLastError(); cus = 256; }
    int64_t nblocks = (int64_t)cus * 4 * MVS_SWEEP_WAVES;
    nblocks = std::min(nblocks, nloc);
    if (const char* g = getenv("MVS_SWEEP_GRID")) {
        const long cap = atol(g);
        if (cap > 0) nblocks = std::min<int64_t>(nblocks, cap);
    }
    if (rs.simplex) hipLaunchKernelGGL(k_sweep_simplex, dim3((unsigned)nblocks), dim3(64), lds, st, prm, a, rs.max_evals, rs.xtol);
    else hipLaunchKernelGGL(k_sweep, dim3((unsigned)nblocks), dim3(64), lds, st, prm, a);
}
void mvsk_job_work(const DParams& prm, const SweepArgs& a, int mode, int shift, int32_t* work, hipStream_t st) {
    if (a.njobs > 0) hipLaunchKernelGGL(k_job_work, dim3(nblk(a.njobs, 256)), dim3(256), 0, st, prm, a, mode, shift, work);
}
int mvsk_job_list_seg(const SweepArgs& a) {
    const int64_t nchunks = (std::max<int64_t>(a.job_hi - a.job_lo, 0) + MVS_XCD_CHUNK - 1) / MVS_XCD_CHUNK;
    return (int)((nchunks + MVS_SWEEP_QUEUES - 1) / MVS_SWEEP_QUEUES) * MVS_XCD_CHUNK;
}
void mvsk_job_list(const DParams& prm, const SweepArgs& a, int32_t* flags, int32_t* scan, int32_t* scan_tmp, int32_t* list, int32_t* bounds, hipStream_t st) {
    const int seg = mvsk_job_list_seg(a);
    const int64_t nslots = (int64_t)MVS_SWEEP_QUEUES * seg, nthreads = std::max(nslots, a.njobs);
    if (nthreads <= 0) return;
    hipLaunchKernelGGL(k_job_list, dim3(nblk(nthreads, 256)), dim3(256), 0, st, prm, a, seg, flags);
    if (nslots <= 0) return;
    launch_exclusive_scan<int32_t, int32_t>(flags, scan, nslots, scan_tmp, st);
    hipLaunchKernelGGL(k_job_scatter, dim3(nblk(nslots, 256)), dim3(256), 0, st, a, seg, scan, list, bounds);
}
void mvsk_job_cuts(const int32_t* scan, int64_t njobs, int n, int32_t* cuts, hipStream_t st) {
    if (njobs > 0) hipLaunchKernelGGL(k_job_cuts, dim3(nblk(njobs, 256)), dim3(256), 0, st, scan, njobs, n, cuts);
}
void mvsk_sweep_retry(const DParams& prm, const SweepArgs& a, int nretry, const RefineSel& rs, hipStream_t st) {
    if (nretry <= 0) return;
    const dim3 grid((unsigned)std::min(nretry, MVS_BIG_SLOTS));
    if (rs.simplex) hipLaunchKernelGGL(k_sweep_retry_simplex, grid, dim3(64), mvsk_sweep_lds_bytes(prm), st, prm, a, nretry, rs.max_evals, rs.xtol);
    else hipLaunchKernelGGL(k_sweep_retry, grid, dim3(64), mvsk_sweep_lds_bytes(prm), st, prm, a, nretry);
}
void mvsk_commit_count(const SweepArgs& a, int32_t* cnt, hipStream_t st) { hipLaunchKernelGGL(k_commit_count, dim3(nblk(a.njobs, 256)), dim3(256), 0, st, a, cnt); }
void mvsk_commit_copy(const SweepArgs& a, const int32_t* base, DPatch* dst, int64_t dst_cap, int32_t* per_view, int keep_key, hipStream_t st) {
    hipLaunchKernelGGL(k_commit_copy, dim3(nblk(a.njobs, 256)), dim3(256), 0, st, a, base, dst, dst_cap, per_view, keep_key);
}
void mvsk_kill_count(const uint8_t* kill, int64_t n, int32_t* cnt, hipStream_t st) { if (n > 0) hipLaunchKernelGGL(k_kill_count, dim3(nblk(n, 256)), dim3(256), 0, st, kill, n, cnt); }
void mvsk_kill_export(const uint8_t* kill, int64_t n, const int32_t* base, int32_t* ids, int64_t cap, hipStream_t st) {
    if (n > 0) hipLaunchKernelGGL(k_kill_export, dim3(nblk(n, 256)), dim3(256), 0, st, kill, n, base, ids, cap);
}
void mvsk_apply_kill_flags(DPatch* pool, uint8_t* kill, int64_t n, hipStream_t st) { if (n > 0) hipLaunchKernelGGL(k_apply_kill_flags, dim3(nblk(n, 256)), dim3(256), 0, st, pool, kill, n); }
void mvsk_apply_kill_ids(DPatch* pool, const int32_t* ids, int64_t n, int64_t pool_n, hipStream_t st) {
    if (n > 0) hipLaunchKernelGGL(k_apply_kill_ids, dim3(nblk(n, 256)), dim3(256), 0, st, pool, ids, n, pool_n);
}
void mvsk_append_records(DPatch* pool, int64_t pool_n, const DPatch* recs, int64_t n, hipStream_t st) {
    if (n > 0) hipLaunchKernelGGL(k_append_records, dim3(nblk(n, 256)), dim3(256), 0, st, pool, pool_n, recs, n);
}
void mvsk_alive_count(const DPatch* pool, int64_t n, int32_t* cnt, hipStream_t st) { if (n > 0) hipLaunchKernelGGL(k_alive_count, dim3(nblk(n, 256)), dim3(256), 0, st, pool, n, cnt); }
void mvsk_alive_gather(const DPatch* pool, int64_t n, const int32_t* base, DPatch* out, int64_t cap, hipStream_t st) {
    if (n > 0) hipLaunchKernelGGL(k_alive_gather, dim3(nblk(n, 256)), dim3(256), 0, st, pool, n, base, out, cap);
}
void mvsk_filter_vimages(const DParams& prm, int additive, int64_t first, int64_t last, const uint32_t* dirty, hipStream_t st) {
    if (last <= first) return;
    const int gl = std::max(prm.nviews <= 16 ? 16 : (prm.nviews <= 32 ? 32 : 64), (int)MVS_LISTCAP);
    const unsigned nb = (unsigned)((last - first + 64 / gl - 1) / (64 / gl));
    if (gl == 16) hipLaunchKernelGGL(k_filter_vimages<16>, dim3(nb), dim3(64), 0, st, prm, additive, first, last, dirty);
    else if (gl == 32) hipLaunchKernelGGL(k_filter_vimages<32>, dim3(nb), dim3(64), 0, st, prm, additive, first, last, dirty);
    else hipLaunchKernelGGL(k_filter_vimages<64>, dim3(nb), dim3(64), 0, st, prm, additive, first, last, dirty);
}
void mvsk_geo_pack(const DPatch* pool, int64_t n, float4* geo, uint8_t* ref, int* bad, hipStream_t st) {
    if (n <= 0) return;
    hipLaunchKernelGGL(k_geo_pack, dim3((unsigned)((n + 255) / 256)), dim3(256), 0, st, pool, n, geo, ref, bad);
}
void mvsk_filter_outside(const DParams& prm, uint8_t* kill, int64_t first, int64_t last, hipStream_t st) {
    if (last > first) hipLaunchKernelGGL(k_filter_outside, dim3((unsigned)(last - first)), dim3(64), 0, st, prm, kill, first);
}
size_t mvsk_texs_lds_bytes(const DParams& prm) {
#if MVS_PAIR_MFMA
    const size_t tex_f = (size_t)MVS_GRAM_CH * 3 * prm.wsz, gram_f = (size_t)prm.gram_ld * prm.gram_ld;
    const size_t texs = MVS_FRAME1_LDS_BYTES + (tex_f > gram_f ? tex_f : gram_f) * sizeof(float);
#else
    const size_t ln = (size_t)prm.list_n;
    const size_t texs = MVS_FRAME1_LDS_BYTES + (ln * 3 * prm.wsz + ln * (ln - 1) / 2) * sizeof(float);
#endif
    return texs > (size_t)MVS_FRAME_LDS_BYTES ? texs : (size_t)MVS_FRAME_LDS_BYTES;
}
void mvsk_filter_exact(const DParams& prm, uint8_t* kill, unsigned long long* evals, unsigned long long* stage, int64_t first, int64_t last, hipStream_t st) {
    if (last > first) hipLaunchKernelGGL(k_filter_exact, dim3((unsigned)((last - first + MVS_FE_PATCHES - 1) / MVS_FE_PATCHES)), dim3(64), mvsk_texs_lds_bytes(prm), st, prm, kill, evals, stage, first, last);
}
void mvsk_filter_neighbor(const DParams& prm, uint8_t* kill, int32_t* retry, int32_t* nretry, int32_t* overflow, unsigned long long* stats, int64_t first, int64_t last, hipStream_t st) {
    if (last <= first) return;
    hipLaunchKernelGGL((k_filter_neighbor<MVS_FILTER_HASH_CAP, MVS_FILTER_ROW_CAP>), dim3((unsigned)(last - first)), dim3(64),
                       (size_t)(MVS_SET_LDS_FLOATS(MVS_FILTER_HASH_CAP, MVS_FILTER_ROW_CAP) + 64) * sizeof(float), st, prm, kill, (const int32_t*)nullptr, 0, retry, nretry, overflow, stats, first);
}
void mvsk_filter_neighbor_retry(const DParams& prm, uint8_t* kill, const int32_t* todo, int32_t ntodo, int32_t* overflow, unsigned long long* stats, hipStream_t st) {
    if (ntodo <= 0) return;
    hipLaunchKernelGGL((k_filter_neighbor<MVS_FILTER2_HASH_CAP, MVS_FILTER2_ROW_CAP>), dim3((unsigned)ntodo), dim3(64),
                       (size_t)MVS_SET_LDS_FLOATS(MVS_FILTER2_HASH_CAP, MVS_FILTER2_ROW_CAP) * sizeof(float), st, prm, kill, todo, ntodo, (int32_t*)nullptr, (int32_t*)nullptr, overflow, stats, (int64_t)0);
}
void mvsk_groups(const DParams& prm, int* parent, int* size, int threshold, uint8_t* kill, hipStream_t st) {
    if (prm.pool_n <= 0) return;
    hipLaunchKernelGGL(k_groups_init, dim3(nblk(prm.pool_n, 256)), dim3(256), 0, st, parent, size, prm.pool_n);
    hipLaunchKernelGGL(k_groups_edges<0>, dim3(nblk(prm.pool_n, 4)), dim3(256), 0, st, prm, parent, (int2*)nullptr, (int*)nullptr, 0);
    hipLaunchKernelGGL(k_groups_count, dim3(nblk(prm.pool_n, 256)), dim3(256), 0, st, prm, parent, size, threshold);
    hipLaunchKernelGGL(k_groups_kill, dim3(nblk(prm.pool_n, 256)), dim3(256), 0, st, prm, parent, size, threshold, kill);
}
void mvsk_groups_literal_edges(const DParams& prm, int* parent, int* size, int* edges2, int* nedges, int cap, hipStream_t st) {
    if (prm.pool_n <= 0) return;
    hipLaunchKernelGGL(k_groups_init, dim3(nblk(prm.pool_n, 256)), dim3(256), 0, st, parent, size, prm.pool_n);
    hipLaunchKernelGGL(k_groups_edges<1>, dim3(nblk(prm.pool_n, 4)), dim3(256), 0, st, prm, parent, (int2*)nullptr, (int*)nullptr, 0);
    hipLaunchKernelGGL(k_groups_count, dim3(nblk(prm.pool_n, 256)), dim3(256), 0, st, prm, parent, size, INT_MAX);
    hipLaunchKernelGGL(k_groups_edges<2>, dim3(nblk(prm.pool_n, 4)), dim3(256), 0, st, prm, parent, reinterpret_cast<int2*>(edges2), nedges, cap);
}
__global__ void k_gather_i32(const int32_t* __restrict__ src, const int32_t* __restrict__ idx, int32_t* __restrict__ out, int64_t n) {
    const int64_t i = (int64_t)blockIdx.x * blockDim.x + threadIdx.x;
    if (i < n) out[i] = src[idx[i]];
}
__global__ void k_scatter_i32(int32_t* __restrict__ dst, const int32_t* __restrict__ idx, const int32_t* __restrict__ val, int64_t n) {
    const int64_t i = (int64_t)blockIdx.x * blockDim.x + threadIdx.x;
    if (i < n) dst[idx[i]] = val[i];
}
void mvsk_gather_i32(const int32_t* src, const int32_t* idx, int32_t* out, int64_t n, hipStream_t st) { if (n > 0) hipLaunchKernelGGL(k_gather_i32, dim3(nblk(n, 256)), dim3(256), 0, st, src, idx, out, n); }
void mvsk_scatter_i32(int32_t* dst, const int32_t* idx, const int32_t* val, int64_t n, hipStream_t st) { if (n > 0) hipLaunchKernelGGL(k_scatter_i32, dim3(nblk(n, 256)), dim3(256), 0, st, dst, idx, val, n); }
void mvsk_groups_kill(const DParams& prm, const int* parent, const int* size, int threshold, uint8_t* kill, hipStream_t st) {
// ... 12 lines not shown
```

mvskit_amd/csrc/mvs_types.h:

```cpp
#pragma once
#include <stdint.h>

#define MVS_WAVE 64
#define MVS_MAXLEV 7
#ifndef MVS_LISTCAP
#define MVS_LISTCAP 16
#endif
#if MVS_LISTCAP > 32
#define MVS_MAXI 64
#else
#define MVS_MAXI 32
#endif
#define MVS_MAXVIEWS 64
#define MVS_CAPMAX 32
#define MVS_NEWBASE 0x40000000

#define MVS_FLAG_ALIVE 1
#define MVS_FLAG_SETTLED 2
struct DPatch {
    float coord[4];
    float normal[4];
    float ncc, dscale, ascale, tmp;
    int32_t nimages, nvimages, flags, id;
    uint8_t images[MVS_MAXI];
    uint8_t vimages[MVS_MAXI];
};
static_assert(sizeof(DPatch) == 64 + 2 * MVS_MAXI, "record is 128 bytes (192 in the 64-view build)");
#define MVS_REC_U4 (sizeof(DPatch) / 16)

typedef int64_t csr_off_t;
struct ListKey {
    float ncc;
    int32_t ref;
};
static_assert(sizeof(ListKey) == 8, "list key is 8 bytes");

struct DView {
    float P[MVS_MAXLEV][12];
    float Minv[9];
    float center[4];
    float oaxis[4];
    float xaxis[3], yaxis[3], zaxis[3];
    float ipscale;
    int32_t W[MVS_MAXLEV], H[MVS_MAXLEV];
    const uint32_t* img[MVS_MAXLEV];
    const uint8_t* mask;
    int32_t gw, gh;
    int32_t cell_base;
    int32_t pad;
};

struct DParams {
    int32_t nviews, level, csize, wsize, wsz, minImageNum, tau, cap, max_propag, depth, enable_check, view_propagation;
    uint32_t seed;
    int32_t refine_steps;
    float rd0, ra0;
    float nccThreshold, nccThresholdBefore;
    float cosAngle0, cosAngle1, cosMinAngle, cosMaxAngle, cosNeighborTypo, cosNeighbor120;
    float sortThreshold, ascaleConst, neighborThreshold, neighborThreshold1, quadThreshold;
    float inv_sz, inv_3sz;
    int32_t total_cells;
    int32_t list_n;
    int32_t gram_ld;
    const DView* views;
    DPatch* pool;
    int64_t pool_n;
    const csr_off_t* csr_start;
    const int32_t* csr_cnt;
    const ListKey* csr_key;
    const int32_t* csr_id32;
    const csr_off_t* vcsr_start;
    const int32_t* vcsr_cnt;
    const int32_t* vcsr_id32;
    const float4* geo;
    const uint8_t* geo_ref;
    const unsigned long long* dpgrid;
};

#ifndef MVS_COUNTER_SLOTS
#define MVS_COUNTER_SLOTS 256
#endif
#define MVS_SWEEP_QUEUES 8
#define MVS_SWEEP_CURSOR_STRIDE 32
struct DCounters {
    unsigned long long candidates, prefiltered, patches, fail0, fail1, inserted, replaced, evals, view_evals, trimmed;
    unsigned long long stage[16];
};

struct SweepArgs {
    int32_t iter, inc, colour;
    int32_t nsweep_views;
    int32_t sweep_views[MVS_MAXVIEWS];
    int32_t job_base[MVS_MAXVIEWS];
    int32_t halfw_max, gh_max;
    int64_t njobs;
    int64_t job_lo, job_hi;
    DPatch* staging;
    int64_t staging_cap;
    unsigned long long* stage_counter;
    int32_t* job_stage;
    int32_t* job_nstage;
    int32_t maxstage;
    uint8_t* kill;
    DCounters* counters;
    int32_t* error_flag;
    int32_t* big_tables;
    int32_t* retry_jobs;
    int32_t* nretry;
    uint32_t* cursors;
    const int32_t* job_list;
    const int32_t* list_bounds;
};

struct SeedChainArgs {
    int32_t K;
    float min_ncc;
    int32_t simplex, max_evals;
    float xtol;
};

struct SeedPointsArgs {
    SeedChainArgs chain;
    int64_t first;
    int32_t n;
};
```

mvskit_amd/engine.py:

```python
from __future__ import annotations

import ctypes as C
import math
import os

import numpy as np

from . import build
from . import synth
from .synth import MAX_IMAGES, PATCH_DTYPE

PROBE_NCC, PROBE_PREPROCESS, PROBE_REFINE, PROBE_POSTPROCESS, PROBE_COST, PROBE_MATH, PROBE_REFINE_X = range(7)
REFINE_HALVING, REFINE_CONVERGED = 0, 1

EXPORTS = [
    "mvs_last_error", "mvs_device_count", "mvs_default_config", "mvs_engine_create", "mvs_engine_destroy",
    "mvs_engine_set_views", "mvs_engine_grid_dims", "mvs_engine_get_pyramid", "mvs_engine_set_thresholds",
    "mvs_engine_get_thresholds", "mvs_engine_update_threshold", "mvs_engine_upload_patches",
    "mvs_engine_clear_patches", "mvs_engine_num_patches", "mvs_engine_download_patches", "mvs_engine_propagate",
    "mvs_engine_pass", "mvs_engine_export_counts", "mvs_engine_export_device", "mvs_engine_commit_device",
    "mvs_engine_commit_local", "mvs_engine_depth_normal_map", "mvs_engine_probe", "mvs_engine_last_timing",
    "mvs_engine_filter", "mvs_comm_unique_id", "mvs_engine_comm_init", "mvs_engine_comm_attach", "mvs_engine_comm_release",
    "mvs_engine_exchange", "mvs_list_cap", "mvs_engine_filter_stats", "mvs_patch_bytes", "mvs_engine_reserve", "mvs_engine_comm_info",
    "mvs_default_refiner", "mvs_engine_set_refiner", "mvs_engine_export_ply", "mvs_engine_seed_patches",
    "mvs_default_seed_random", "mvs_engine_seed_random", "mvs_engine_seed_random_hypotheses",
    "mvs_default_seed_points", "mvs_engine_seed_points", "mvs_engine_seed_points_hypotheses", "mvs_engine_depth_ranges",
    "mvs_default_maps_config", "mvs_engine_render_maps", "mvs_engine_fused_points",
    "mvs_engine_tsdf", "mvs_engine_extract_mesh", "mvs_engine_mesh",
]
PLY_ASCII, PLY_BINARY_LE = 0, 1
PLY_VERTEX_DTYPE = np.dtype([("xyz", "<f4", (3,)), ("normal", "<f4", (3,)), ("rgb", "u1", (3,))])
FUSED_POINT_DTYPE = np.dtype([("xyz", "<f4", (3,)), ("normal", "<f4", (3,)), ("conf", "<f4"), ("rgb", "u1", (3,)), ("view", "u1")])


class Config(C.Structure):
    _fields_ = [("nviews", C.c_int32), ("level", C.c_int32), ("csize", C.c_int32), ("wsize", C.c_int32),
                ("minImageNum", C.c_int32), ("max_propag", C.c_int32), ("nccThreshold", C.c_float),
                ("maxAngleThreshold", C.c_float), ("quadThreshold", C.c_float), ("depth", C.c_int32),
                ("seed", C.c_uint32), ("refine_steps", C.c_int32), ("refine_rd0", C.c_float), ("refine_ra0", C.c_float),
                ("enable_check", C.c_int32), ("view_begin", C.c_int32), ("view_stride", C.c_int32),
                ("device", C.c_int32), ("view_propagation", C.c_int32), ("shard_index", C.c_int32), ("shard_count", C.c_int32),
                ("literal_groups", C.c_int32), ("max_patches", C.c_int64)]


class Refiner(C.Structure):
    _fields_ = [("mode", C.c_int32), ("max_evals", C.c_int32), ("xtol", C.c_float)]


class ViewDesc(C.Structure):
    _fields_ = [("width", C.c_int32), ("height", C.c_int32), ("P", C.c_float * 12), ("rgb", C.c_void_p),
                ("mask", C.c_void_p)]


class SeedView(C.Structure):
    _fields_ = [("normals", C.c_void_p), ("mask", C.c_void_p)]


class SeedRandom(C.Structure):
    _fields_ = [("hypotheses", C.c_int32), ("seed", C.c_uint32), ("max_tilt", C.c_float), ("min_ncc", C.c_float),
                ("depth_min", C.c_void_p), ("depth_max", C.c_void_p)]


class SeedPoints(C.Structure):
    _fields_ = [("hypotheses", C.c_int32), ("min_ncc", C.c_float)]


class MapsConfig(C.Structure):
    _fields_ = [("source", C.c_int32), ("min_consistent", C.c_int32), ("depth_tol", C.c_float), ("normal_cos", C.c_float),
                ("dedupe", C.c_int32), ("pad", C.c_int32)]


class ViewMaps(C.Structure):
    _fields_ = [("depth", C.c_void_p), ("normal", C.c_void_p), ("conf", C.c_void_p), ("ids", C.c_void_p), ("agree", C.c_void_p)]


class Volume(C.Structure):
    _fields_ = [("origin", C.c_float * 3), ("voxel", C.c_float), ("dims", C.c_int32 * 3), ("trunc", C.c_float), ("min_count", C.c_int32),
                ("pad", C.c_int32)]

    @property
    def shape(self):
        return self.dims[2], self.dims[1], self.dims[0]


class Counters(C.Structure):
    _fields_ = [(n, C.c_int64) for n in ("candidates", "prefiltered", "patches", "fail0", "fail1", "inserted",
                                         "replaced", "evals", "view_evals", "trimmed")]

    def as_dict(self):
        return {n: int(getattr(self, n)) for n, _ in self._fields_}


class Timing(C.Structure):
    _fields_ = [("index_ms", C.c_float), ("sweep_ms", C.c_float), ("commit_ms", C.c_float), ("sweep_launches", C.c_int32),
                ("exchange_ms", C.c_float), ("sweep_jobs_listed", C.c_int32), ("exchange_bytes", C.c_int64), ("check_retried_cells", C.c_int64)]


class FilterStats(C.Structure):
    _fields_ = [(n, C.c_float) for n in ("outside_ms", "exact_ms", "neighbor_ms", "groups_ms", "rebuild_ms", "total_ms")] + \
               [(n, C.c_int64) for n in ("patches_in", "exact_patches", "exact_view_evals", "neighbor_patches", "neighbor_tasks", "neighbor_entries",
                                         "neighbor_visited", "neighbor_accepted", "neighbor_retried", "exchange_bytes")]


class EngineError(RuntimeError):

    def __init__(self, msg, status=None):
        super().__init__(msg)
        self.status = status


_libs = {}


def load_library(cap32: bool = False, cap: int = 0):
    cap = cap or (32 if cap32 else 16)
    default = build.ENGINE_LIBS[cap]
    LIB_PATH = os.environ.get({16: "MVS_ENGINE_LIB", 32: "MVS_ENGINE_LIB32", 64: "MVS_ENGINE_LIB64"}[cap], default)
    if LIB_PATH in _libs:
        return _libs[LIB_PATH]
    if not os.path.exists(LIB_PATH):
        raise EngineError(f"{LIB_PATH} is missing: run `python -m mvskit_amd.build` (the engine has no CPU fallback)")
    try:
        import torch
    except ImportError:
        pass
    L = C.CDLL(LIB_PATH)
    vp = C.c_void_p
    L.mvs_last_error.restype = C.c_char_p
    L.mvs_device_count.restype = C.c_int
    L.mvs_default_config.argtypes = [C.POINTER(Config)]
    L.mvs_engine_create.argtypes = [C.POINTER(Config), C.POINTER(vp)]
    L.mvs_engine_destroy.argtypes = [vp]
    L.mvs_engine_set_views.argtypes = [vp, C.c_int, C.POINTER(ViewDesc)]
    L.mvs_engine_grid_dims.argtypes = [vp, C.c_int, C.POINTER(C.c_int), C.POINTER(C.c_int)]
    L.mvs_engine_get_pyramid.argtypes = [vp, C.c_int, C.c_int, vp, C.POINTER(C.c_int), C.POINTER(C.c_int)]
    L.mvs_engine_set_thresholds.argtypes = [vp, C.c_float, C.c_float, C.c_int]
    L.mvs_engine_get_thresholds.argtypes = [vp, C.POINTER(C.c_float), C.POINTER(C.c_float), C.POINTER(C.c_int)]
    L.mvs_engine_update_threshold.argtypes = [vp]
    L.mvs_engine_upload_patches.argtypes = [vp, C.c_int64, vp]
    L.mvs_engine_clear_patches.argtypes = [vp]
    L.mvs_engine_num_patches.argtypes = [vp, C.POINTER(C.c_int64)]
    L.mvs_engine_download_patches.argtypes = [vp, C.c_int64, vp, C.POINTER(C.c_int64)]
    L.mvs_engine_propagate.argtypes = [vp, C.c_int, C.POINTER(Counters)]
    L.mvs_engine_pass.argtypes = [vp, C.c_int, C.c_int, C.POINTER(Counters)]
    L.mvs_engine_export_counts.argtypes = [vp, C.POINTER(C.c_int64), C.POINTER(C.c_int64), vp]
    L.mvs_engine_export_device.argtypes = [vp, vp, C.c_int64, vp, C.c_int64]
    L.mvs_engine_commit_device.argtypes = [vp, vp, C.c_int64, vp, C.c_int64]
    L.mvs_engine_commit_local.argtypes = [vp]
    L.mvs_engine_depth_normal_map.argtypes = [vp, C.c_int, C.c_int, vp, vp, vp]
    L.mvs_engine_probe.argtypes = [vp, C.c_int, C.c_int64, vp, vp, vp, vp, vp]
    L.mvs_engine_last_timing.argtypes = [vp, C.POINTER(Timing)]
    L.mvs_engine_filter.argtypes = [vp, vp]
    L.mvs_comm_unique_id.argtypes = [vp]
    L.mvs_engine_comm_init.argtypes = [vp, vp, C.c_int, C.c_int]
    L.mvs_engine_comm_attach.argtypes = [vp, vp, C.c_int, C.c_int]
    L.mvs_engine_comm_release.argtypes = [vp]
    L.mvs_engine_exchange.argtypes = [vp]
    L.mvs_list_cap.restype = C.c_int
    L.mvs_patch_bytes.restype = C.c_int
    L.mvs_engine_reserve.argtypes = [vp, C.c_int64]
    L.mvs_engine_filter_stats.argtypes = [vp, C.POINTER(FilterStats)]
    if hasattr(L, "mvs_engine_set_refiner"):
        L.mvs_default_refiner.argtypes = [C.POINTER(Refiner)]
        L.mvs_default_refiner.restype = None
        L.mvs_engine_set_refiner.argtypes = [vp, C.POINTER(Refiner)]
    if hasattr(L, "mvs_engine_export_ply"):
        L.mvs_engine_export_ply.argtypes = [vp, C.c_int, C.c_int64, vp, C.POINTER(C.c_int64)]
    if hasattr(L, "mvs_engine_seed_patches"):
        L.mvs_engine_seed_patches.argtypes = [vp, C.c_int64, vp, C.POINTER(SeedView), C.POINTER(C.c_int64)]
    if hasattr(L, "mvs_engine_seed_random"):
        L.mvs_default_seed_random.argtypes = [C.POINTER(SeedRandom)]
        L.mvs_default_seed_random.restype = None
        L.mvs_engine_seed_random.argtypes = [vp, C.POINTER(SeedRandom), C.POINTER(C.c_int64)]
        L.mvs_engine_seed_random_hypotheses.argtypes = [vp, C.POINTER(SeedRandom), C.c_int, C.c_int64, vp, vp]
    if hasattr(L, "mvs_engine_seed_points"):
        L.mvs_default_seed_points.argtypes = [C.POINTER(SeedPoints)]
        L.mvs_default_seed_points.restype = None
        L.mvs_engine_seed_points.argtypes = [vp, C.POINTER(SeedPoints), C.c_int64, vp, C.POINTER(C.c_int64)]
        L.mvs_engine_seed_points_hypotheses.argtypes = [vp, C.POINTER(SeedPoints), C.c_int64, vp, vp, vp]
        L.mvs_engine_depth_ranges.argtypes = [vp, C.c_int64, vp, C.c_float, vp, vp, vp]
    if hasattr(L, "mvs_engine_render_maps"):
        L.mvs_default_maps_config.argtypes = [C.POINTER(MapsConfig)]
        L.mvs_default_maps_config.restype = None
        L.mvs_engine_render_maps.argtypes = [vp, C.POINTER(MapsConfig), C.POINTER(ViewMaps), vp]
        L.mvs_engine_fused_points.argtypes = [vp, C.POINTER(MapsConfig), C.c_int64, vp, C.POINTER(C.c_int64)]
    if hasattr(L, "mvs_engine_tsdf"):
        L.mvs_engine_tsdf.argtypes = [vp, C.POINTER(MapsConfig), C.POINTER(Volume), vp, vp]
        L.mvs_engine_extract_mesh.argtypes = [vp, C.POINTER(Volume), vp, vp, C.c_int64, vp, C.c_int64, vp, C.POINTER(C.c_int64), C.POINTER(C.c_int64)]
        L.mvs_engine_mesh.argtypes = [vp, C.POINTER(MapsConfig), C.POINTER(Volume), C.c_int64, vp, C.c_int64, vp, C.POINTER(C.c_int64), C.POINTER(C.c_int64)]
    _libs[LIB_PATH] = L
    return L


def _ptr(a):
    return a.ctypes.data_as(C.c_void_p) if a is not None else None


class Engine:

    def __init__(self, nviews, list_cap=None, **kw):
        if list_cap is None:
            list_cap = 16 if nviews <= 16 else (32 if nviews <= 32 else 64)
        self.L = load_library(cap=list_cap)
        self.list_cap = self.L.mvs_list_cap()
        self.dtype = synth.patch_dtype((self.L.mvs_patch_bytes() - 64) // 2)
        self.cfg = Config()
        self.L.mvs_default_config(C.byref(self.cfg))
        self.cfg.nviews = nviews
        for k, v in kw.items():
            if not hasattr(self.cfg, k):
                raise AttributeError(k)
            setattr(self.cfg, k, v)
        self.h = C.c_void_p()
        self._check(self.L.mvs_engine_create(C.byref(self.cfg), C.byref(self.h)))
        self._keep = None

    def _check(self, status):
        if status != 0:
            raise EngineError(f"mvskit engine error {status}: {self.L.mvs_last_error().decode()}", status)

    def close(self):
        if getattr(self, "h", None) is not None and self.h:
            self.L.mvs_engine_destroy(self.h)
            self.h = None

    def __del__(self):
        try:
            self.close()
        except Exception:
            pass

    def set_scene(self, scene, masks=None, sizes=None):
        n = scene.nviews
        descs = (ViewDesc * n)()
        keep = []
        for v in range(n):
            w, h = (scene.W, scene.H) if sizes is None else sizes[v]
            img = np.ascontiguousarray(np.asarray(scene.images[v], dtype=np.uint8)[:h, :w])
            keep.append(img)
            descs[v].width, descs[v].height = w, h
            P = np.ascontiguousarray(scene.P[v], dtype=np.float32).ravel()
            for k in range(12):
                descs[v].P[k] = float(P[k])
            descs[v].rgb = img.ctypes.data
            descs[v].mask = None
            if masks is not None and masks[v] is not None:
                m = np.ascontiguousarray(np.asarray(masks[v], dtype=np.uint8)[:h, :w])
                keep.append(m)
                descs[v].mask = m.ctypes.data
        self._check(self.L.mvs_engine_set_views(self.h, n, descs))
        self._view_shapes = [(scene.H, scene.W)] * n if sizes is None else [(h, w) for w, h in sizes]

    def grid_dims(self, v):
        gw, gh = C.c_int(), C.c_int()
        self._check(self.L.mvs_engine_grid_dims(self.h, v, C.byref(gw), C.byref(gh)))
        return gw.value, gh.value

    def pyramid(self, v, level):
        w, h = C.c_int(), C.c_int()
        self._check(self.L.mvs_engine_get_pyramid(self.h, v, level, None, C.byref(w), C.byref(h)))
        out = np.empty((h.value, w.value, 3), dtype=np.uint8)
        self._check(self.L.mvs_engine_get_pyramid(self.h, v, level, _ptr(out), C.byref(w), C.byref(h)))
        return out

    def set_refiner(self, mode="halving", max_evals=500, xtol=1e-4):
        modes = {"halving": REFINE_HALVING, "converged": REFINE_CONVERGED}
        if mode not in modes:
            raise ValueError(f"refiner mode {mode!r}: 'halving' or 'converged'")
# ... 182 lines not shown
        else:
            self._check(call(0, None, 0, None, C.byref(nv), C.byref(nt)))
        verts, tris = np.zeros((nv.value, 3), np.float32), np.zeros((nt.value, 3), np.int32)
        if nv.value or nt.value:
            self._check(call(nv.value, _ptr(verts), nt.value, _ptr(tris), C.byref(nv), C.byref(nt)))
        return verts, tris

    def extract_mesh(self, volume, tsdf, count=None):
        tsdf = np.ascontiguousarray(tsdf, dtype=np.float32)
        count = None if count is None else np.ascontiguousarray(count, dtype=np.int32)
        if tsdf.size != np.prod(volume.shape) or (count is not None and count.size != tsdf.size):
            raise ValueError("extract_mesh: tsdf and count must have one value per lattice point")
        return self._mesh(lambda *a: self.L.mvs_engine_extract_mesh(self.h, C.byref(volume), _ptr(tsdf), _ptr(count), *a))

    def mesh(self, volume, source=0, min_consistent=1, depth_tol=0.01, normal_cos=0.9, cap_v=0, cap_t=0):
        c = self._maps_config(source, min_consistent, depth_tol, normal_cos, 0)
        return self._mesh(lambda *a: self.L.mvs_engine_mesh(self.h, C.byref(c), C.byref(volume), *a), int(cap_v), int(cap_t))

    def propagate(self, it):
        c = Counters()
        self._check(self.L.mvs_engine_propagate(self.h, it, C.byref(c)))
        return c.as_dict()

    def filter(self):
        r = np.zeros(4, dtype=np.int64)
        self._check(self.L.mvs_engine_filter(self.h, _ptr(r)))
        return {"outside": int(r[0]), "exact": int(r[1]), "neighbor": int(r[2]), "groups": int(r[3])}

    def filter_stats(self):
        f = FilterStats()
        self._check(self.L.mvs_engine_filter_stats(self.h, C.byref(f)))
        return {n: getattr(f, n) for n, _ in f._fields_}

    def engine_pass(self, it, p):
        c = Counters()
        self._check(self.L.mvs_engine_pass(self.h, it, p, C.byref(c)))
        return c.as_dict()

    def export_counts(self):
        a, b = C.c_int64(), C.c_int64()
        pv = np.zeros(self.cfg.nviews, dtype=np.int32)
        self._check(self.L.mvs_engine_export_counts(self.h, C.byref(a), C.byref(b), _ptr(pv)))
        return a.value, b.value, pv

    def export_device(self, new_ptr, cap_new, kill_ptr, cap_kill):
        self._check(self.L.mvs_engine_export_device(self.h, new_ptr, cap_new, kill_ptr, cap_kill))

    def commit_device(self, new_ptr, n_new, kill_ptr, n_kill):
        self._check(self.L.mvs_engine_commit_device(self.h, new_ptr, n_new, kill_ptr, n_kill))

    def commit_local(self):
        self._check(self.L.mvs_engine_commit_local(self.h))

    COMM_ID_BYTES = 128

    def comm_unique_id(self):
        buf = C.create_string_buffer(self.COMM_ID_BYTES)
        self._check(self.L.mvs_comm_unique_id(buf))
        return buf.raw

    def comm_init(self, uid: bytes, rank: int, world: int):
        assert len(uid) == self.COMM_ID_BYTES
        self._check(self.L.mvs_engine_comm_init(self.h, C.c_char_p(uid), rank, world))

    def comm_info(self):
        r, w, cc, cr = C.c_int(), C.c_int(), C.c_int(), C.c_int()
        self.L.mvs_engine_comm_info.argtypes = [C.c_void_p] + [C.POINTER(C.c_int)] * 4
        self._check(self.L.mvs_engine_comm_info(self.h, C.byref(r), C.byref(w), C.byref(cc), C.byref(cr)))
        return {"rank": r.value, "world": w.value, "comm_count": cc.value, "comm_rank": cr.value}

    def comm_release(self):
        self._check(self.L.mvs_engine_comm_release(self.h))

    def exchange(self):
        self._check(self.L.mvs_engine_exchange(self.h))

    def timing(self):
        t = Timing()
        self._check(self.L.mvs_engine_last_timing(self.h, C.byref(t)))
        return {"index_ms": t.index_ms, "sweep_ms": t.sweep_ms, "commit_ms": t.commit_ms, "sweep_launches": t.sweep_launches,
                "exchange_ms": t.exchange_ms, "exchange_bytes": int(t.exchange_bytes), "check_retried_cells": int(t.check_retried_cells),
                "sweep_jobs_listed": int(t.sweep_jobs_listed)}

    def depth_normal_map(self, view, kind):
        gw, gh = self.grid_dims(view)
        d = np.zeros((gh, gw), np.float32)
        n = np.zeros((gh, gw, 3), np.float32)
        ids = np.zeros((gh, gw), np.int32)
        self._check(self.L.mvs_engine_depth_normal_map(self.h, view, kind, _ptr(d), _ptr(n), _ptr(ids)))
        return d, n, ids

    def probe(self, op, recs=None, values=None):
        if op == PROBE_MATH:
            x = np.ascontiguousarray(values, dtype=np.float32)
            out = np.zeros((x.shape[0], 5), np.float32)
            self._check(self.L.mvs_engine_probe(self.h, op, x.shape[0], None, _ptr(x), None, _ptr(out), None))
            return out
        recs = synth.convert_records(recs, self.dtype)
        n = recs.shape[0]
        out_rec = np.zeros(n, dtype=self.dtype)
        out_f = np.zeros((n, 4) if op == PROBE_REFINE_X else n, np.float32)
        out_i = np.zeros(n, np.int32)
        self._check(self.L.mvs_engine_probe(self.h, op, n, _ptr(recs), None, _ptr(out_rec), _ptr(out_f), _ptr(out_i)))
        return out_rec, out_f, out_i


def make_volume(origin, voxel, dims, trunc, min_count=1):
    v = Volume()
    for k in range(3):
        v.origin[k], v.dims[k] = float(origin[k]), int(dims[k])
    v.voxel, v.trunc, v.min_count, v.pad = float(voxel), float(trunc), int(min_count), 0
    return v


def volume_around(xyz, voxel, trunc_voxels=4, pad_voxels=2, min_count=1):
    xyz = np.asarray(xyz, dtype=np.float64).reshape(-1, 3)
    if xyz.shape[0] == 0 or not np.isfinite(xyz).all() or not voxel > 0:
        raise ValueError("volume_around: needs finite points and a positive voxel")
    lo = xyz.min(axis=0) - pad_voxels * voxel
    dims = np.ceil((xyz.max(axis=0) + pad_voxels * voxel - lo) / voxel).astype(np.int64) + 1
    if (dims < 2).any() or (dims > 1024).any() or int(np.prod(dims)) > 1 << 28:
        raise ValueError(f"volume_around: {dims.tolist()} lattice points: each dimension must lie in 2..1024, their product must not exceed 2^28")
    return make_volume(lo, voxel, dims, trunc_voxels * voxel, min_count)


def write_mesh_ply(path, verts, tris, binary=True):
    verts = np.ascontiguousarray(verts, dtype="<f4").reshape(-1, 3)
    tris = np.ascontiguousarray(tris, dtype="<i4").reshape(-1, 3)
    head = (f"ply\nformat {'binary_little_endian' if binary else 'ascii'} 1.0\nelement vertex {verts.shape[0]}\nproperty float x\n"
            f"property float y\nproperty float z\nelement face {tris.shape[0]}\nproperty list uchar int vertex_indices\nend_header\n")
    with open(path, "wb") as f:
        f.write(head.encode("ascii"))
        if binary:
            faces = np.zeros(tris.shape[0], dtype=np.dtype([("n", "u1"), ("v", "<i4", (3,))]))
            faces["n"], faces["v"] = 3, tris
            f.write(verts.tobytes())
            f.write(faces.tobytes())
        else:
            f.write("".join(f"{x:.9g} {y:.9g} {z:.9g}\n" for x, y, z in verts.tolist()).encode("ascii"))
            f.write("".join(f"3 {a} {b} {c}\n" for a, b, c in tris.tolist()).encode("ascii"))
```

Before: 29.90 million.

## Pair two candidate patches per wave in sweep refinement using half-row layouts

Adds a paired refinement path in which one 64-lane wave refines two candidate patches at once. Each half-row of 8 lanes handles one patch's views, using DPP half-row broadcasts, a paired NCC evaluation, and a pending-candidate LDS stash. It is enabled by default through a new SweepArgs.pair switch (env MVS_SWEEP_PAIR) and adds counters recording why patches were or weren't paired. The aim is better lane utilisation when view lists are short. The cost is extra LDS, more __syncthreads, and pairing bookkeeping overhead.

```diff
diff --git a/include/mvskit_engine.h b/include/mvskit_engine.h
--- a/include/mvskit_engine.h
+++ b/include/mvskit_engine.h
@@ -247,6 +247,8 @@
 } mvs_timing;
 int mvs_engine_last_timing(mvs_engine* e, mvs_timing* t);
 
+int mvs_engine_sweep_pairs(mvs_engine* e, int64_t out[6]);
+
 #ifdef __cplusplus
 }
 #endif
diff --git a/mvskit_amd/csrc/mvs_device.cuh b/mvskit_amd/csrc/mvs_device.cuh
--- a/mvskit_amd/csrc/mvs_device.cuh
+++ b/mvskit_amd/csrc/mvs_device.cuh
@@ -175,6 +175,18 @@
     return (float)(h >> 8) * (1.0f / 16777216.0f) - 0.5f;
 }
 
+DEV uint32_t rng_prefix(uint32_t seed, uint32_t a, uint32_t b, uint32_t c, uint32_t d) {
+    uint32_t h = mix32(seed ^ 0x9e3779b9u);
+    h = mix32(h ^ a) + 0x85ebca6bu;
+    h = mix32(h ^ b) + 0xc2b2ae35u;
+    h = mix32(h ^ c) + 0x27d4eb2fu;
+    return mix32(h ^ d) + 0x165667b1u;
+}
+DEV float rng_tail(uint32_t h, uint32_t e) {
+    h = mix32(h ^ e);
+    return (float)(h >> 8) * (1.0f / 16777216.0f) - 0.5f;
+}
+
 DEV F3 project(const DView* vw, F4 X, int level) {
     const float* P = vw->P[level];
     float r0 = fma_(P[3], X.w, fma_(P[2], X.z, fma_(P[1], X.y, P[0] * X.x)));
@@ -225,6 +237,14 @@
 template <int LANE> DEV float row_bcast_f(float x) {
     return __int_as_float(__builtin_amdgcn_update_dpp(0, __float_as_int(x), 0x150 + LANE, 0xf, 0xf, false));
 }
+template <int LANE, int BANKS> DEV float row_bcast_banks_f(float old, float x) {
+    return __int_as_float(__builtin_amdgcn_update_dpp(__float_as_int(old), __float_as_int(x), 0x150 + LANE, 0xf, BANKS, false));
+}
+template <int LANE, bool PAIR> DEV float half_bcast_f(float x) {
+    if constexpr (PAIR) return row_bcast_banks_f<8 + LANE, 0xC>(row_bcast_banks_f<LANE, 0x3>(x, x), x);
+    else return row_bcast_f<LANE>(x);
+}
+template <bool PAIR = false>
 DEV void get_paxes(const DParams& prm, const DView* vw, F4 coord, F4 normal, F4& px, F4& py) {
     const F4 ctr = ld4(vw->center);
     const float ips = vw->ipscale;
@@ -239,14 +259,14 @@
     F3 x3 = cross3(y3, n3);
     px = {x3.x * pscale, x3.y * pscale, x3.z * pscale, 0.0f};
     py = {y3.x * pscale, y3.y * pscale, y3.z * pscale, 0.0f};
-    const int j = lane_id() & 15;
+    const int j = lane_id() & (PAIR ? 7 : 15);
     const float a = j == 1 ? 1.0f : 0.0f, b = j == 2 ? 1.0f : 0.0f;
     const F4 X{fma_(b, py.x, fma_(a, px.x, coord.x)), fma_(b, py.y, fma_(a, px.y, coord.y)), fma_(b, py.z, fma_(a, px.z, coord.z)), coord.w};
     const F3 ic = project_regs(P, X);
-    const F3 c0{row_bcast_f<0>(ic.x), row_bcast_f<0>(ic.y), row_bcast_f<0>(ic.z)};
+    const F3 c0{half_bcast_f<0, PAIR>(ic.x), half_bcast_f<0, PAIR>(ic.y), half_bcast_f<0, PAIR>(ic.z)};
     const float inv = rcp_rn(norm3(sub3(ic, c0)));
-    px = scl4(px, row_bcast_f<1>(inv));
-    py = scl4(py, row_bcast_f<2>(inv));
+    px = scl4(px, half_bcast_f<1, PAIR>(inv));
+    py = scl4(py, half_bcast_f<2, PAIR>(inv));
 }
 DEV float robustincc(float incc) { return div_rn(incc, 1 + 3 * incc); }
 DEV float unrobustincc(float r) { return div_rn(r, 1 - 3 * r); }
@@ -486,6 +506,90 @@
     incc_l = 1.0f - (dot * (inv0 * inv_l)) * prm.inv_3sz;
 }
 
+DEV unsigned long long eval_steps4_pair(const DParams& prm, WaveCtx& wc, const ClsConst& cc, const Frame& f, int n0, int n1, unsigned (&okm)[2][4], float& incc_l) {
+    frames_publish(wc, f, 64);
+    const unsigned long long okb = ballot(f.ok != 0);
+#pragma unroll
+    for (int g = 0; g < 4; ++g) { okm[0][g] = (unsigned)((okb >> (16 * g)) & 0xffull); okm[1][g] = (unsigned)((okb >> (16 * g + 8)) & 0xffull); }
+#pragma unroll
+    for (int g = 0; g < 4; ++g)
+        wc.view_evals += ((okm[0][g] & 1u) ? (unsigned)__popc(okm[0][g]) : 0u) + ((okm[1][g] & 1u) ? (unsigned)__popc(okm[1][g]) : 0u);
+    const int lc = wc.lane & 15;
+    float P1r = 0.0f, P1g = 0.0f, P1b = 0.0f, P2 = 0.0f, P01 = 0.0f;
+#pragma nounroll
+    for (int s = 0; s < 2; ++s) {
+        const int n = s ? n1 : n0;
+        const int fb = cc.fb + 8 * s, pb = MVS_PIVOT_LDS4 + 8 * s, lb = 8 * s;
+        float c0[3][3];
+        ClsPend pend[3];
+        const int vlast = max(n - 1, 0);
+        {
+            const ClsFrame fr = cls_frame(fb);
+#pragma unroll
+            for (int j = 0; j < 3; ++j) pend[j] = cls_issue(fr, cls_opaque(cc.cs[j]));
+        }
+        {
+            const float4 pv = mvs_dyn_lds4[pb];
+            const ClsFrame fn = cls_frame(fb + min(1, vlast));
+            float s1r = 0.0f, s1g = 0.0f, s1b = 0.0f, s2 = 0.0f;
+#pragma unroll
+            for (int j = 0; j < 3; ++j) {
+                const unsigned cs = cls_opaque(cc.cs[j]);
+                float r, g, b;
+                cls_colour(pend[j], cs, pv.x, pv.y, pv.z, r, g, b);
+                pend[j] = cls_issue(fn, cs);
+                c0[j][0] = r; c0[j][1] = g; c0[j][2] = b;
+                s1r += r; s1g += g; s1b += b;
+                s2 = fma_(r, r, s2); s2 = fma_(g, g, s2); s2 = fma_(b, b, s2);
+            }
+            MVS_ROW_STEP4(0xB1) MVS_ROW_STEP4(0x4E) MVS_ROW_STEP4(0x141) MVS_ROW_STEP4(0x140)
+            if (lc >= lb) { P1r = s1r; P1g = s1g; P1b = s1b; P2 = s2; }
+        }
+        for (int k = 1; k < n; ++k) {
+            const float4 pv = mvs_dyn_lds4[pb + k];
+            const ClsFrame fn = cls_frame(fb + min(k + 1, vlast));
+            float s1r = 0.0f, s1g = 0.0f, s1b = 0.0f, s2 = 0.0f, s01 = 0.0f;
+#pragma unroll
+            for (int j = 0; j < 3; ++j) {
+                const unsigned cs = cls_opaque(cc.cs[j]);
+                float r, g, b;
+                cls_colour(pend[j], cs, pv.x, pv.y, pv.z, r, g, b);
+                pend[j] = cls_issue(fn, cs);
+                s1r += r; s1g += g; s1b += b;
+                s2 = fma_(r, r, s2); s2 = fma_(g, g, s2); s2 = fma_(b, b, s2);
+                s01 = fma_(r, c0[j][0], s01); s01 = fma_(g, c0[j][1], s01); s01 = fma_(b, c0[j][2], s01);
+            }
+            MVS_ROW_STEP5(0xB1) MVS_ROW_STEP5(0x4E) MVS_ROW_STEP5(0x141) MVS_ROW_STEP5(0x140)
+            if (lc == lb + k) { P1r = s1r; P1g = s1g; P1b = s1b; P2 = s2; P01 = s01; }
+        }
+    }
+    const int a0 = (wc.lane & 56) << 2;
+    if (cc.nx > 0) {
+        const float4 pv = mvs_dyn_lds4[MVS_PIVOT_LDS4 + lc];
+        ClsFrame fr;
+        fr.tlx = f.tlx; fr.tly = f.tly; fr.dxx = f.dxx; fr.dxy = f.dxy; fr.dyx = f.dyx; fr.dyy = f.dyy; fr.w = f.w;
+        fr.base = ((unsigned long long)f.img_hi << 32) | (unsigned long long)f.img_lo;
+        {
+            const int q = cc.xbase;
+            const unsigned cs = (unsigned)(q % prm.wsize) | ((unsigned)(q / prm.wsize) << 8) | (1u << 16);
+            const ClsPend pe = cls_issue(fr, cs);
+            float r, g, b;
+            cls_colour(pe, cs, pv.x, pv.y, pv.z, r, g, b);
+            const float r0 = bperm_f(a0, r), g0 = bperm_f(a0, g), b0 = bperm_f(a0, b);
+            P1r += r; P1g += g; P1b += b;
+            P2 = fma_(r, r, P2); P2 = fma_(g, g, P2); P2 = fma_(b, b, P2);
+            P01 = fma_(r, r0, P01); P01 = fma_(g, g0, P01); P01 = fma_(b, b0, P01);
+        }
+    }
+    const float m_r = P1r * prm.inv_sz, m_g = P1g * prm.inv_sz, m_b = P1b * prm.inv_sz;
+    const float ssd = fmaxf(P2 - fma_(P1b, m_b, fma_(P1g, m_g, P1r * m_r)), 0.0f);
+    const float inv_l = inv_msd(prm, ssd);
+    const float m0r = bperm_f(a0, m_r), m0g = bperm_f(a0, m_g), m0b = bperm_f(a0, m_b), inv0 = bperm_f(a0, inv_l);
+    const float dot = P01 - fma_(P1b, m0b, fma_(P1g, m0g, P1r * m0r));
+    incc_l = 1.0f - (dot * (inv0 * inv_l)) * prm.inv_3sz;
+    return okb;
+}
+
 DEV void cls_raw(const ClsPend& p, unsigned cs, float& r, float& g, float& b) {
     const Texel2 q0 = p.q0, q1 = p.q1;
     const float fm = cvt_ub2(cs);
@@ -1143,6 +1247,184 @@
     else c.ncc = 1.0f - unrobustincc(compute_incc(prm, wc, c.coord, c.normal, c.img, c.nimg, w, 1));
 }
 
+#define MVS_PEND_IMG 16
+#define MVS_PEND_GX 80
+#define MVS_PEND_GY 144
+#define MVS_PEND_W 208
+#define MVS_PEND_CTX 272
+#define MVS_PEND_XIMG 304
+#define MVS_PEND_INTS 320
+DEV float rff(float x) { return __int_as_float(rfl(__float_as_int(x))); }
+DEV void pend_store(int* st, const WaveCtx& wc, const Cand& c, float w) {
+    __syncthreads();
+    if (wc.lane == 0) {
+        float* f = reinterpret_cast<float*>(st);
+        f[0] = c.coord.x; f[1] = c.coord.y; f[2] = c.coord.z; f[3] = c.coord.w;
+        f[4] = c.normal.x; f[5] = c.normal.y; f[6] = c.normal.z; f[7] = c.normal.w;
+        f[8] = c.ncc; f[9] = c.dscale; f[10] = c.ascale; f[11] = c.tmp;
+        st[12] = c.nimg; st[13] = c.nvimg;
+    }
+    st[MVS_PEND_IMG + wc.lane] = c.img; st[MVS_PEND_GX + wc.lane] = c.gx; st[MVS_PEND_GY + wc.lane] = c.gy;
+    st[MVS_PEND_W + wc.lane] = __float_as_int(w);
+    __syncthreads();
+}
+DEV void pend_load(const int* st, const WaveCtx& wc, Cand& c, float& w) {
+    const float* f = reinterpret_cast<const float*>(st);
+    c.coord = {rff(f[0]), rff(f[1]), rff(f[2]), rff(f[3])};
+    c.normal = {rff(f[4]), rff(f[5]), rff(f[6]), rff(f[7])};
+    c.ncc = rff(f[8]); c.dscale = rff(f[9]); c.ascale = rff(f[10]); c.tmp = rff(f[11]);
+    c.nimg = rfl(st[12]); c.nvimg = rfl(st[13]);
+    c.img = st[MVS_PEND_IMG + wc.lane]; c.gx = st[MVS_PEND_GX + wc.lane]; c.gy = st[MVS_PEND_GY + wc.lane];
+    c.vimg = 0; c.vgx = 0; c.vgy = 0;
+    w = __int_as_float(st[MVS_PEND_W + wc.lane]);
+}
+DEV void cost_func4_pair(const DParams& prm, WaveCtx& wc, const RefineCtx& rc, int imgx, int sz0, int sz1, int szl, float x0, float x1, float x2,
+                         double (&fv)[2][4], const ClsConst& cc) {
+    F4 coord, normal, px, py;
+    decode(prm, rc, x0, x1, x2, coord, normal);
+    get_paxes<true>(prm, prm.views + rc.ref, coord, normal, px, py);
+    const Frame f = make_frame(prm, coord, px, py, normal, imgx, (wc.lane & 7) < szl);
+    wc.evals += 8u;
+    unsigned okm[2][4];
+    float incc_l;
+    const unsigned long long okb = eval_steps4_pair(prm, wc, cc, f, sz0, sz1, okm, incc_l);
+    const float val_l = robustincc(incc_l);
+    const int src = (int)(((cls_opaque((unsigned)wc.lane) & 3u) << 4) | ((cls_opaque((unsigned)wc.lane) & 4u) << 1));
+    const unsigned okl = (unsigned)(okb >> src) & 0xffu;
+    double num = 0.0;
+    int den = 0;
+    const int szm = max(sz0, sz1);
+    for (int i = 1; i < szm; ++i) {
+        const float v = bperm_f(4 * (src + i), val_l);
+        const bool ok = (okl >> i) & 1u;
+        num = ok ? num + (double)v : num;
+        den += ok ? 1 : 0;
+    }
+    const double q = num / (double)den;
+    const int min0 = min(prm.minImageNum, sz0), min1 = min(prm.minImageNum, sz1);
+#pragma unroll
+    for (int j = 0; j < 4; ++j) {
+        fv[0][j] = ((okm[0][j] & 1u) && rli(den, j) >= min0 - 1) ? rld(q, j) : 2.0;
+        fv[1][j] = ((okm[1][j] & 1u) && rli(den, 4 + j) >= min1 - 1) ? rld(q, 4 + j) : 2.0;
+    }
+}
+DEV void refine_patch_pair(const DParams& prm, WaveCtx& wc, int* st, Cand& c1, uint32_t k0, uint32_t k1, uint32_t k2, uint32_t k3a, uint32_t k3b, float& w1) {
+    float* const ctx = reinterpret_cast<float*>(st + MVS_PEND_CTX);
+    int* const ximg = st + MVS_PEND_XIMG;
+    const float amin = -23.99999f, amax = 23.99999f;
+    double fbest0 = 2.0, fbest1 = 2.0;
+    int sz0 = 0, sz1 = 0;
+    w1 = 0.0f;
+#pragma nounroll
+    for (int s = 0; s < 2; ++s) {
+        F4 coord = c1.coord, normal = c1.normal;
+        float dscale = c1.dscale;
+        int img = c1.img, nimg = c1.nimg;
+        if (s == 0) {
+            const float* f = reinterpret_cast<const float*>(st);
+            coord = {rff(f[0]), rff(f[1]), rff(f[2]), rff(f[3])};
+            normal = {rff(f[4]), rff(f[5]), rff(f[6]), rff(f[7])};
+            dscale = rff(f[9]); nimg = rfl(st[12]);
+            img = st[MVS_PEND_IMG + wc.lane];
+        }
+        RefineCtx rc;
+        rc.center = coord;
+        rc.ref = rli(img, 0);
+        rc.ray = nrm4(sub4(coord, ld4((prm.views + rc.ref)->center)));
+        rc.dscale = dscale;
+        rc.ascale = prm.ascaleConst;
+        const float w = compute_weights(prm, wc, coord, normal, img, nimg);
+        if (s == 0) st[MVS_PEND_W + wc.lane] = __float_as_int(w);
+        else w1 = w;
+        float x[3];
+        encode(prm, rc, coord, normal, x);
+        x[1] = fmaxf(fminf(x[1], amax), amin);
+        x[2] = fmaxf(fminf(x[2], amax), amin);
+        double fv[4];
+        float piv[3] = {128.0f, 128.0f, 128.0f};
+        cost_func4(prm, wc, rc, __shfl(img, wc.lane & 15), nimg, false, x[0], x[1], x[2], fv, piv);
+        __syncthreads();
+        if (wc.lane < 8) {
+            mvs_dyn_lds4[MVS_PIVOT_LDS4 + 8 * s + wc.lane] = make_float4(piv[0], piv[1], piv[2], 0.0f);
+            ximg[8 * s + wc.lane] = img;
+        }
+        const int sz = min(prm.tau, nimg);
+        if (wc.lane == 0) {
+            float* d = ctx + 16 * s;
+            d[0] = rc.center.x; d[1] = rc.center.y; d[2] = rc.center.z; d[3] = rc.center.w;
+            d[4] = rc.ray.x; d[5] = rc.ray.y; d[6] = rc.ray.z; d[7] = rc.ray.w;
+            d[8] = rc.dscale; d[9] = __int_as_float(rc.ref); d[10] = x[0]; d[11] = x[1]; d[12] = x[2];
+            d[13] = __int_as_float((int)rng_prefix(prm.seed, k0, k1, k2, s ? k3b : k3a)); d[14] = __int_as_float(sz); d[15] = 0.0f;
+        }
+        if (s == 0) { fbest0 = fv[0]; sz0 = sz; } else { fbest1 = fv[0]; sz1 = sz; }
+    }
+    __syncthreads();
+    const ClsConst cc = wc.cc;
+    float rd = prm.rd0, ra = prm.ra0;
+    const int g = wc.lane >> 4;
+    const uint32_t gj = (uint32_t)min(g, 2);
+    const float4* const my = reinterpret_cast<const float4*>(ctx + 16 * ((wc.lane >> 3) & 1));
+    for (int k = 0; k < prm.refine_steps; ++k) {
+        const float4 A = my[0], B = my[1], Cq = my[2], D = my[3];
+        RefineCtx rc;
+        rc.center = {A.x, A.y, A.z, A.w};
+        rc.ray = {B.x, B.y, B.z, B.w};
+        rc.dscale = Cq.x; rc.ref = __float_as_int(Cq.y); rc.ascale = prm.ascaleConst;
+        const float bx0 = Cq.z, bx1 = Cq.w, bx2 = D.x;
+        const uint32_t hp = (uint32_t)__float_as_int(D.y);
+        const int szl = __float_as_int(D.z);
+        const int imgx = ximg[wc.lane & 15];
+        const uint32_t draw = 16u + ((uint32_t)(k * 3) + gj) * 3u;
+        const float u0 = 2.0f * rng_tail(hp, draw + 0);
+        const float u1 = 2.0f * rng_tail(hp, draw + 1);
+        const float u2 = 2.0f * rng_tail(hp, draw + 2);
+        float cx0 = (gj == 1u) ? bx0 : fma_(u0, rd, bx0);
+        float cx1 = (gj == 0u) ? bx1 : fmaxf(fminf(fma_(u1, ra, bx1), amax), amin);
+        float cx2 = (gj == 0u) ? bx2 : fmaxf(fminf(fma_(u2, ra, bx2), amax), amin);
+        if (g == 3) {
+            cx0 = bx0 - (cx0 - bx0);
+            cx1 = fmaxf(fminf(bx1 - (cx1 - bx1), amax), amin);
+            cx2 = fmaxf(fminf(bx2 - (cx2 - bx2), amax), amin);
+        }
+        double fv[2][4];
+        cost_func4_pair(prm, wc, rc, imgx, sz0, sz1, szl, cx0, cx1, cx2, fv, cc);
+        __syncthreads();
+#pragma unroll
+        for (int s = 0; s < 2; ++s) {
+            int jb = 0;
+            double fstep = fv[s][0];
+#pragma unroll
+            for (int j = 1; j < 4; ++j) if (fv[s][j] < fstep) { fstep = fv[s][j]; jb = j; }
+            const double fb = s ? fbest1 : fbest0;
+            if (fstep < fb) {
+                if (s) fbest1 = fstep; else fbest0 = fstep;
+                const float n0 = rlf(cx0, 16 * jb + 8 * s), n1 = rlf(cx1, 16 * jb + 8 * s), n2 = rlf(cx2, 16 * jb + 8 * s);
+                if (wc.lane == 0) { ctx[16 * s + 10] = n0; ctx[16 * s + 11] = n1; ctx[16 * s + 12] = n2; }
+            }
+        }
+        __syncthreads();
+        rd *= 0.5f; ra *= 0.5f;
+    }
+#pragma unroll
+    for (int s = 0; s < 2; ++s) {
+        const float* d = ctx + 16 * s;
+        RefineCtx rc;
+        rc.center = {rff(d[0]), rff(d[1]), rff(d[2]), rff(d[3])};
+        rc.ray = {rff(d[4]), rff(d[5]), rff(d[6]), rff(d[7])};
+        rc.dscale = rff(d[8]); rc.ref = rfl(__float_as_int(d[9])); rc.ascale = prm.ascaleConst;
+        F4 coord, normal;
+        decode(prm, rc, rff(d[10]), rff(d[11]), rff(d[12]), coord, normal);
+        normal.w = 0.0f;
+        if (s) { c1.coord = coord; c1.normal = normal; }
+        else if (wc.lane == 0) {
+            float* f = reinterpret_cast<float*>(st);
+            f[0] = coord.x; f[1] = coord.y; f[2] = coord.z; f[3] = coord.w;
+            f[4] = normal.x; f[5] = normal.y; f[6] = normal.z; f[7] = normal.w;
+        }
+    }
+    __syncthreads();
+}
+
 DEV int refine_patch_simplex(const DParams& prm, WaveCtx& wc, Cand& c, int max_evals, float xtol, float* w_out = nullptr,
                                float* x_out = nullptr, double* f_out = nullptr) {
     RefineCtx rc;
diff --git a/mvskit_amd/csrc/mvs_engine.cpp b/mvskit_amd/csrc/mvs_engine.cpp
--- a/mvskit_amd/csrc/mvs_engine.cpp
+++ b/mvskit_amd/csrc/mvs_engine.cpp
@@ -195,6 +195,7 @@
     DevBuf<int32_t> error_flag;
     DevBuf<int32_t> big_tables, retry_jobs;
     DevBuf<int32_t> job_list;
+    int64_t sweep_pairs[6] = {0, 0, 0, 0, 0, 0};
     int64_t retried_cells = 0;
     int64_t pass_retried = 0;
     SweepArgs sa{};
@@ -1759,7 +1760,10 @@
     HIPCHK(hipStreamSynchronize(st));
     HIPCHK(hipGetLastError());
     mvs_counters sum{};
-    for (const DCounters& c : hcs) add_counters(sum, c);
+    for (const DCounters& c : hcs) {
+        add_counters(sum, c);
+        for (int k = 0; k < 6; ++k) e->sweep_pairs[k] += (int64_t)c.pair[k];
+    }
     sum.evals += fill[0]; sum.view_evals += fill[1]; sum.trimmed = (int64_t)trimmed;
     float ms = 0.0f;
     (void)hipEventElapsedTime(&ms, e->ev[0], e->ev[1]); e->timing.index_ms = ms;
@@ -2181,6 +2185,12 @@
     return MVS_OK;
 }
 
+int mvs_engine_sweep_pairs(mvs_engine* e, int64_t out[6]) {
+    if (!e || !out) return MVS_ERR_ARG;
+    for (int k = 0; k < 6; ++k) out[k] = e->sweep_pairs[k];
+    return MVS_OK;
+}
+
 int mvs_engine_last_timing(mvs_engine* e, mvs_timing* t) {
     if (!e || !t) return MVS_ERR_ARG;
     *t = e->timing;
diff --git a/mvskit_amd/csrc/mvs_kernels.hip b/mvskit_amd/csrc/mvs_kernels.hip
--- a/mvskit_amd/csrc/mvs_kernels.hip
+++ b/mvskit_amd/csrc/mvs_kernels.hip
@@ -433,6 +433,7 @@
 struct SweepAcc {
     unsigned cand, pref, patch, f0, f1, ins, rep;
     unsigned long long evals, view_evals;
+    unsigned pair[6];
 #ifdef MVS_STAGE_TIMING
     unsigned long long stage[16];
 #endif
@@ -441,6 +442,7 @@
     SweepAcc acc;
     acc.cand = acc.pref = acc.patch = acc.f0 = acc.f1 = acc.ins = acc.rep = 0u;
     acc.evals = acc.view_evals = 0ull;
+    for (int k = 0; k < 6; ++k) acc.pair[k] = 0u;
 #ifdef MVS_STAGE_TIMING
     for (int k = 0; k < 16; ++k) acc.stage[k] = 0ull;
 #endif
@@ -457,6 +459,7 @@
     if (acc.rep) atomicAdd(&C->replaced, (unsigned long long)acc.rep);
     if (acc.evals) atomicAdd(&C->evals, acc.evals);
     if (acc.view_evals) atomicAdd(&C->view_evals, acc.view_evals);
+    for (int k = 0; k < 6; ++k) if (acc.pair[k]) atomicAdd(&C->pair[k], (unsigned long long)acc.pair[k]);
 #ifdef MVS_STAGE_TIMING
     for (int k = 0; k < 12; ++k) if (acc.stage[k]) atomicAdd(&C->stage[k], acc.stage[k]);
     atomicMax(&C->stage[12], acc.stage[12]); atomicMax(&C->stage[13], acc.stage[13]);
@@ -464,7 +467,7 @@
 #endif
 }
 template <bool BIG, bool SIMPLEX = false>
-DEV void sweep_cell(const DParams& prm, const SweepArgs& a, WaveCtx& wc, SweepAcc* acc, const int64_t job, int* s_scratch, float* s_texs,
+DEV void sweep_cell(const DParams& prm, const SweepArgs& a, WaveCtx& wc, SweepAcc* acc, const int64_t job, int* s_scratch, int* s_pend, float* s_texs,
                     int* big_table, int max_evals = 0, float xtol = 0.0f) {
 #ifdef MVS_STAGE_TIMING
     unsigned long long st_acc[16] = {0, 0, 0, 0, 0, 0, 0, 0, 0, 0, 0, 0, 0, 0, 0, 0};
@@ -497,103 +500,152 @@
     const float icx = (float)(prm.csize * (2 * cx + 1) - 1) / 2.0f, icy = (float)(prm.csize * (2 * cy + 1) - 1) / 2.0f;
 
     const int nsrc = prm.view_propagation ? 3 : 2;
-    for (int sidx = 0; sidx < nsrc; ++sidx) {
+    bool pend = false, pend_failed = false;
+    uint32_t pend_k3 = 0u;
+    int pend_sz = 0;
+    unsigned n_pair = 0, n_elig = 0, n_last = 0, n_noroom = 0, n_lost = 0, n_long = 0;
+    for (int sidx = 0; sidx <= nsrc; ++sidx) {
+        const bool flush = sidx == nsrc;
         const int scx = sidx < 2 ? sxs[sidx] : cx, scy = sidx < 2 ? sys[sidx] : cy;
-        if (scx < 0 || gw <= scx || scy < 0 || gh <= scy) continue;
-        const int g = vw->cell_base + scy * gw + scx;
-        const csr_off_t sb = prm.csr_start[g];
-        const int sn = min(prm.csr_cnt[g], MVS_CAPMAX);
+        if (!flush && (scx < 0 || gw <= scx || scy < 0 || gh <= scy)) continue;
         const int as_view = sidx == 2 ? v : -1;
         int E_id = 0;
         bool E_take = false;
-        if (wc.lane < sn) { E_id = pgrid_id(prm, sb + wc.lane); E_take = (pgrid_ref(prm, sb + wc.lane) == v) != (sidx == 2); }
-        unsigned todo = (unsigned)ballot(E_take);
+        if (!flush) {
+            const int g = vw->cell_base + scy * gw + scx;
+            const csr_off_t sb = prm.csr_start[g];
+            const int sn = min(prm.csr_cnt[g], MVS_CAPMAX);
+            if (wc.lane < sn) { E_id = pgrid_id(prm, sb + wc.lane); E_take = (pgrid_ref(prm, sb + wc.lane) == v) != (sidx == 2); }
+        }
+        unsigned todo = flush ? (pend ? 1u : 0u) : (unsigned)ballot(E_take);
         while (todo) {
             const int n = __ffs((int)todo) - 1;
             todo &= todo - 1u;
             const DPatch* sp = prm.pool + rli(E_id, n);
             const int srcslot = sidx * prm.cap + n;
-            for (int it = 0; it < prm.max_propag; ++it) {
+            const int ntrial = flush ? 1 : prm.max_propag;
+            for (int it = 0; it < ntrial; ++it) {
                 ST_ADD(7, st_t)
                 const int np = L_n;
-                const uint32_t k0 = (uint32_t)a.iter, k1 = (uint32_t)v, k2 = (uint32_t)cell, k3 = (uint32_t)(srcslot * 16 + it);
+                const uint32_t k0 = (uint32_t)a.iter, k1 = (uint32_t)v, k2 = (uint32_t)cell;
+                uint32_t k3 = (uint32_t)(srcslot * 16 + it);
                 Cand c;
+                float keep_w = 0.0f;
                 int worst = -1;
-                float worst_ncc = 0.0f;
-                F3 ic;
-                if (np < prm.cap) {
-                    const float ra = rng_uniform(prm.seed, k0, k1, k2, k3, 0) * (float)prm.csize;
-                    const float rb = rng_uniform(prm.seed, k0, k1, k2, k3, 1) * (float)prm.csize;
-                    ic = {icx + ra, icy + rb, 1.0f};
+                int nfin = 1;
+                if (!flush) {
+                    float worst_ncc = 0.0f;
+                    F3 ic;
+                    if (np < prm.cap) {
+                        const float ra = rng_uniform(prm.seed, k0, k1, k2, k3, 0) * (float)prm.csize;
+                        const float rb = rng_uniform(prm.seed, k0, k1, k2, k3, 1) * (float)prm.csize;
+                        ic = {icx + ra, icy + rb, 1.0f};
+                    } else {
+                        worst = rli(L_id, prm.cap - 1);
+                        worst_ncc = rlf(L_ncc, prm.cap - 1);
+                        const DPatch* wp = worst >= MVS_NEWBASE ? a.staging + (worst - MVS_NEWBASE) : prm.pool + worst;
+                        ic = project(vw, ld4(wp->coord), prm.level);
+                    }
+                    {
+                        Cand src;
+                        load_cand(sp, wc, src);
+                        const bool gen_ok = generate_patch(prm, wc, s_scratch, src, ic, c, as_view, np >= prm.cap);
+                        ST_ADD(1, st_t)
+                        if (!gen_ok) { pend_failed |= pend; continue; }
+                    }
+                    ++n_cand;
+                    if (np >= prm.cap && c.ncc < worst_ncc) { ++n_pref; continue; }
+                    ++n_patch;
+                    const int pre_r = pre_process(prm, wc, s_scratch, c);
+                    ST_ADD(2, st_t)
+                    if (pre_r == -1) { ++n_f0; pend_failed |= pend; continue; }
+                    if (!pend && np + 1 < prm.cap) {
+                        pend_store(s_pend, wc, c, 0.0f);
+                        pend = true; pend_failed = false; pend_k3 = k3; pend_sz = min(prm.tau, c.nimg);
+                        continue;
+                    }
+                    if (pend) nfin = 2;
+                    else ++n_noroom;
                 } else {
-                    worst = rli(L_id, prm.cap - 1);
-                    worst_ncc = rlf(L_ncc, prm.cap - 1);
-                    const DPatch* wp = worst >= MVS_NEWBASE ? a.staging + (worst - MVS_NEWBASE) : prm.pool + worst;
-                    ic = project(vw, ld4(wp->coord), prm.level);
+                    pend_load(s_pend, wc, c, keep_w);
+                    k3 = pend_k3;
+                    if (pend_failed) ++n_lost; else ++n_last;
                 }
-                {
-                    Cand src;
-                    load_cand(sp, wc, src);
-                    const bool gen_ok = generate_patch(prm, wc, s_scratch, src, ic, c, as_view, np >= prm.cap);
-                    ST_ADD(1, st_t)
-                    if (!gen_ok) continue;
+                bool paired = false;
+                if (nfin == 2) {
+                    const bool fits = pend_sz <= 8 && min(prm.tau, c.nimg) <= 8;
+                    if (!fits) n_long += 2;
+                    else n_elig += 2;
+                    if constexpr (!SIMPLEX) {
+                        if (fits && a.pair) {
+                            refine_patch_pair(prm, wc, s_pend, c, k0, k1, k2, pend_k3, k3, keep_w);
+                            paired = true;
+                            n_pair += 2;
+                        }
+                    }
+                    Cand first;
+                    float first_w;
+                    pend_load(s_pend, wc, first, first_w);
+                    pend_store(s_pend, wc, c, keep_w);
+                    c = first; keep_w = first_w;
+                    const uint32_t t = k3; k3 = pend_k3; pend_k3 = t;
                 }
-                ++n_cand;
-                if (np >= prm.cap && c.ncc < worst_ncc) { ++n_pref; continue; }
-                ++n_patch;
-                const int pre_r = pre_process(prm, wc, s_scratch, c);
-                ST_ADD(2, st_t)
-                if (pre_r == -1) { ++n_f0; continue; }
-                float keep_w;
-                if constexpr (SIMPLEX) (void)refine_patch_simplex(prm, wc, c, max_evals, xtol, &keep_w);
-                else refine_patch(prm, wc, c, k0, k1, k2, k3, &keep_w);
-                ST_ADD(3, st_t)
-                const int post_r = post_process(prm, wc, s_scratch, s_texs, tstride, c, keep_w, true);
-                ST_ADD(4, st_t)
-                if (post_r == -1) { ++n_f1; continue; }
-                if (prm.depth >= 2 && prm.enable_check) {
-                    __syncthreads();
-                    if (wc.lane < MVS_CAPMAX) s_scratch[wc.lane] = L_id;
-                    __syncthreads();
-                    #ifdef MVS_STAGE_TIMING
-                    const CheckCtx cx{a.staging, v, cell, L_n, s_scratch, st_acc};
+                pend = false;
+                for (int fi = 0; fi < nfin; ++fi) {
+                    if (fi == 1) { pend_load(s_pend, wc, c, keep_w); k3 = pend_k3; }
+                    if (!paired) {
+                        if constexpr (SIMPLEX) (void)refine_patch_simplex(prm, wc, c, max_evals, xtol, &keep_w);
+                        else refine_patch(prm, wc, c, k0, k1, k2, k3, &keep_w);
+                    }
+                    ST_ADD(3, st_t)
+                    const int post_r = post_process(prm, wc, s_scratch, s_texs, tstride, c, keep_w, true);
+                    ST_ADD(4, st_t)
+                    if (post_r == -1) { ++n_f1; continue; }
+                    if (prm.depth >= 2 && prm.enable_check) {
+                        __syncthreads();
+                        if (wc.lane < MVS_CAPMAX) s_scratch[wc.lane] = L_id;
+                        __syncthreads();
+                        #ifdef MVS_STAGE_TIMING
+                        const CheckCtx cx{a.staging, v, cell, L_n, s_scratch, st_acc};
 #else
-                    const CheckCtx cx{a.staging, v, cell, L_n, s_scratch, nullptr};
-#endif
-                    const int chk_r = check_patch<BIG>(prm, wc, cx, c, s_texs, a.error_flag, big_table);
-                    ST_ADD(5, st_t)
-                    if (!BIG && chk_r < 0) { gave_up = true; break; }
-                    if (chk_r) { ++n_f1; continue; }
+                        const CheckCtx cx{a.staging, v, cell, L_n, s_scratch, nullptr};
+#endif
+                        const int chk_r = check_patch<BIG>(prm, wc, cx, c, s_texs, a.error_flag, big_table);
+                        ST_ADD(5, st_t)
+                        if (!BIG && chk_r < 0) { gave_up = true; break; }
+                        if (chk_r) { ++n_f1; continue; }
+                    }
+                    unsigned long long slot64 = 0;
+                    if (wc.lane == 0) slot64 = atomicAdd(a.stage_counter, 1ull);
+                    const int64_t slot = ((int64_t)rfl((int)(slot64 >> 32)) << 32) | (uint32_t)rfl((int)(slot64 & 0xffffffffull));
+                    if (slot >= a.staging_cap || ns >= a.maxstage) {
+                        if (wc.lane == 0) atomicOr(a.error_flag, 1);
+                        continue;
+                    }
+                    if (L_n == prm.cap) {
+                        if (wc.lane == 0) {
+                            if (worst >= MVS_NEWBASE) a.staging[worst - MVS_NEWBASE].flags &= ~1;
+                            else a.kill[worst] = 1;
+                        }
+                        --L_n;
+                        ++n_rep;
+                    } else ++n_ins;
+                    store_cand(a.staging + slot, wc, c, 1 | (v << 8), cell);
+                    if (wc.lane == 0) a.job_stage[job * a.maxstage + ns] = (int32_t)slot;
+                    ++ns;
+                    const bool lands = ballot(wc.lane < c.nimg && c.img == v && c.gy * gw + c.gx == cell) != 0ull;
+                    if (lands) {
+                        const int nid = MVS_NEWBASE + (int)slot;
+                        const int pos = __popcll(ballot(wc.lane < L_n && rank_before(L_ncc, L_id, c.ncc, nid)));
+                        const int up_id = __shfl_up(L_id, 1);
+                        const float up_ncc = __shfl_up(L_ncc, 1);
+                        if (wc.lane > pos) { L_id = up_id; L_ncc = up_ncc; }
+                        if (wc.lane == pos) { L_id = nid; L_ncc = c.ncc; }
+                        ++L_n;
+                    }
+                    ST_ADD(6, st_t)
                 }
-                unsigned long long slot64 = 0;
-                if (wc.lane == 0) slot64 = atomicAdd(a.stage_counter, 1ull);
-                const int64_t slot = ((int64_t)rfl((int)(slot64 >> 32)) << 32) | (uint32_t)rfl((int)(slot64 & 0xffffffffull));
-                if (slot >= a.staging_cap || ns >= a.maxstage) {
-                    if (wc.lane == 0) atomicOr(a.error_flag, 1);
-                    continue;
-                }
-                if (np == prm.cap) {
-                    if (wc.lane == 0) {
-                        if (worst >= MVS_NEWBASE) a.staging[worst - MVS_NEWBASE].flags &= ~1;
-                        else a.kill[worst] = 1;
-                    }
-                    --L_n;
-                    ++n_rep;
-                } else ++n_ins;
-                store_cand(a.staging + slot, wc, c, 1 | (v << 8), cell);
-                if (wc.lane == 0) a.job_stage[job * a.maxstage + ns] = (int32_t)slot;
-                ++ns;
-                const bool lands = ballot(wc.lane < c.nimg && c.img == v && c.gy * gw + c.gx == cell) != 0ull;
-                if (lands) {
-                    const int nid = MVS_NEWBASE + (int)slot;
-                    const int pos = __popcll(ballot(wc.lane < L_n && rank_before(L_ncc, L_id, c.ncc, nid)));
-                    const int up_id = __shfl_up(L_id, 1);
-                    const float up_ncc = __shfl_up(L_ncc, 1);
-                    if (wc.lane > pos) { L_id = up_id; L_ncc = up_ncc; }
-                    if (wc.lane == pos) { L_id = nid; L_ncc = c.ncc; }
-                    ++L_n;
-                }
-                ST_ADD(6, st_t)
+                if (gave_up) break;
             }
             if (gave_up) break;
         }
@@ -607,6 +659,8 @@
     {
         acc->cand += n_cand; acc->pref += n_pref; acc->patch += n_patch; acc->f0 += n_f0; acc->f1 += n_f1; acc->ins += n_ins; acc->rep += n_rep;
         acc->evals += wc.evals; acc->view_evals += wc.view_evals;
+        acc->pair[0] += n_pair; acc->pair[5] += n_elig;
+        acc->pair[1] += n_last; acc->pair[2] += n_noroom; acc->pair[3] += n_lost; acc->pair[4] += n_long;
 #ifdef MVS_STAGE_TIMING
         st_acc[0] = ST_NOW() - st_begin;
         for (int k = 0; k < 12; ++k) acc->stage[k] += st_acc[k];
@@ -617,7 +671,7 @@
 }
 
 template <bool SIMPLEX>
-DEV void sweep_resident(const DParams& prm, const SweepArgs& a, int* s_scratch, float* s_texs, int max_evals, float xtol) {
+DEV void sweep_resident(const DParams& prm, const SweepArgs& a, int* s_scratch, int* s_pend, float* s_texs, int max_evals, float xtol) {
     WaveCtx wc = make_wave_ctx(prm);
     SweepAcc acc = sweep_acc_zero();
     for (unsigned step = 0; step < MVS_SWEEP_QUEUES; ++step) {
@@ -632,44 +686,48 @@
             if (k >= ntake) break;
             const int64_t job = a.job_list[qbegin + (int32_t)k];
             __syncthreads();
-            sweep_cell<false, SIMPLEX>(prm, a, wc, &acc, job, s_scratch, s_texs, nullptr, max_evals, xtol);
+            sweep_cell<false, SIMPLEX>(prm, a, wc, &acc, job, s_scratch, s_pend, s_texs, nullptr, max_evals, xtol);
         }
     }
     if (wc.lane == 0) sweep_acc_flush(a, acc, blockIdx.x & (MVS_COUNTER_SLOTS - 1));
 }
 __global__ __launch_bounds__(64, MVS_SWEEP_WAVES) void k_sweep(DParams prm, SweepArgs a) {
     __shared__ int s_scratch[192];
+    __shared__ __attribute__((aligned(16))) int s_pend[MVS_PEND_INTS];
     extern __shared__ float s_texs[];
-    sweep_resident<false>(prm, a, s_scratch, s_texs, 0, 0.0f);
+    sweep_resident<false>(prm, a, s_scratch, s_pend, s_texs, 0, 0.0f);
 }
 __global__ __launch_bounds__(64, MVS_SWEEP_WAVES) void k_sweep_simplex(DParams prm, SweepArgs a, int max_evals, float xtol) {
     __shared__ int s_scratch[192];
+    __shared__ __attribute__((aligned(16))) int s_pend[MVS_PEND_INTS];
     extern __shared__ float s_texs[];
-    sweep_resident<true>(prm, a, s_scratch, s_texs, max_evals, xtol);
+    sweep_resident<true>(prm, a, s_scratch, s_pend, s_texs, max_evals, xtol);
 }
 template <bool SIMPLEX>
-DEV void sweep_retry_cell(const DParams& prm, const SweepArgs& a, const int64_t job, int* s_scratch, float* s_texs, int* big_table, int max_evals, float xtol) {
+DEV void sweep_retry_cell(const DParams& prm, const SweepArgs& a, const int64_t job, int* s_scratch, int* s_pend, float* s_texs, int* big_table, int max_evals, float xtol) {
     WaveCtx wc = make_wave_ctx(prm);
     SweepAcc acc = sweep_acc_zero();
-    sweep_cell<true, SIMPLEX>(prm, a, wc, &acc, job, s_scratch, s_texs, big_table, max_evals, xtol);
+    sweep_cell<true, SIMPLEX>(prm, a, wc, &acc, job, s_scratch, s_pend, s_texs, big_table, max_evals, xtol);
     if (wc.lane == 0) sweep_acc_flush(a, acc, (unsigned)(job & (MVS_COUNTER_SLOTS - 1)));
 }
 __global__ __launch_bounds__(64, 1) void k_sweep_retry(DParams prm, SweepArgs a, int nretry) {
     __shared__ int s_scratch[192];
+    __shared__ __attribute__((aligned(16))) int s_pend[MVS_PEND_INTS];
     extern __shared__ float s_texs[];
     int* big_table = a.big_tables + (size_t)blockIdx.x * MVS_FILTER2_HASH_CAP;
     for (int k = blockIdx.x; k < nretry; k += gridDim.x) {
         __syncthreads();
-        sweep_retry_cell<false>(prm, a, (int64_t)a.retry_jobs[k], s_scratch, s_texs, big_table, 0, 0.0f);
+        sweep_retry_cell<false>(prm, a, (int64_t)a.retry_jobs[k], s_scratch, s_pend, s_texs, big_table, 0, 0.0f);
     }
 }
 __global__ __launch_bounds__(64, 1) void k_sweep_retry_simplex(DParams prm, SweepArgs a, int nretry, int max_evals, float xtol) {
     __shared__ int s_scratch[192];
+    __shared__ __attribute__((aligned(16))) int s_pend[MVS_PEND_INTS];
     extern __shared__ float s_texs[];
     int* big_table = a.big_tables + (size_t)blockIdx.x * MVS_FILTER2_HASH_CAP;
     for (int k = blockIdx.x; k < nretry; k += gridDim.x) {
         __syncthreads();
-        sweep_retry_cell<true>(prm, a, (int64_t)a.retry_jobs[k], s_scratch, s_texs, big_table, max_evals, xtol);
+        sweep_retry_cell<true>(prm, a, (int64_t)a.retry_jobs[k], s_scratch, s_pend, s_texs, big_table, max_evals, xtol);
     }
 }
 
@@ -1230,6 +1288,12 @@
     const size_t need = texs > chk ? texs : chk;
     return need > (size_t)MVS_FRAME_LDS_BYTES ? need : (size_t)MVS_FRAME_LDS_BYTES;
 }
+static SweepArgs sweep_args_with_switches(const SweepArgs& a) {
+    SweepArgs b = a;
+    const char* p = getenv("MVS_SWEEP_PAIR");
+    b.pair = (p && atoi(p) == 0) ? 0 : 1;
+    return b;
+}
 void mvsk_sweep(const DParams& prm, const SweepArgs& a, const RefineSel& rs, hipStream_t st) {
     const int64_t nloc = a.job_hi - a.job_lo;
     if (nloc <= 0) return;
@@ -1244,8 +1308,9 @@
         const long cap = atol(g);
         if (cap > 0) nblocks = std::min<int64_t>(nblocks, cap);
     }
-    if (rs.simplex) hipLaunchKernelGGL(k_sweep_simplex, dim3((unsigned)nblocks), dim3(64), lds, st, prm, a, rs.max_evals, rs.xtol);
-    else hipLaunchKernelGGL(k_sweep, dim3((unsigned)nblocks), dim3(64), lds, st, prm, a);
+    const SweepArgs b = sweep_args_with_switches(a);
+    if (rs.simplex) hipLaunchKernelGGL(k_sweep_simplex, dim3((unsigned)nblocks), dim3(64), lds, st, prm, b, rs.max_evals, rs.xtol);
+    else hipLaunchKernelGGL(k_sweep, dim3((unsigned)nblocks), dim3(64), lds, st, prm, b);
 }
 void mvsk_job_work(const DParams& prm, const SweepArgs& a, int mode, int shift, int32_t* work, hipStream_t st) {
     if (a.njobs > 0) hipLaunchKernelGGL(k_job_work, dim3(nblk(a.njobs, 256)), dim3(256), 0, st, prm, a, mode, shift, work);
@@ -1269,8 +1334,9 @@
 void mvsk_sweep_retry(const DParams& prm, const SweepArgs& a, int nretry, const RefineSel& rs, hipStream_t st) {
     if (nretry <= 0) return;
     const dim3 grid((unsigned)std::min(nretry, MVS_BIG_SLOTS));
-    if (rs.simplex) hipLaunchKernelGGL(k_sweep_retry_simplex, grid, dim3(64), mvsk_sweep_lds_bytes(prm), st, prm, a, nretry, rs.max_evals, rs.xtol);
-    else hipLaunchKernelGGL(k_sweep_retry, grid, dim3(64), mvsk_sweep_lds_bytes(prm), st, prm, a, nretry);
+    const SweepArgs b = sweep_args_with_switches(a);
+    if (rs.simplex) hipLaunchKernelGGL(k_sweep_retry_simplex, grid, dim3(64), mvsk_sweep_lds_bytes(prm), st, prm, b, nretry, rs.max_evals, rs.xtol);
+    else hipLaunchKernelGGL(k_sweep_retry, grid, dim3(64), mvsk_sweep_lds_bytes(prm), st, prm, b, nretry);
 }
 void mvsk_commit_count(const SweepArgs& a, int32_t* cnt, hipStream_t st) { hipLaunchKernelGGL(k_commit_count, dim3(nblk(a.njobs, 256)), dim3(256), 0, st, a, cnt); }
 void mvsk_commit_copy(const SweepArgs& a, const int32_t* base, DPatch* dst, int64_t dst_cap, int32_t* per_view, int keep_key, hipStream_t st) {
diff --git a/mvskit_amd/csrc/mvs_types.h b/mvskit_amd/csrc/mvs_types.h
--- a/mvskit_amd/csrc/mvs_types.h
+++ b/mvskit_amd/csrc/mvs_types.h
@@ -85,6 +85,7 @@
 struct DCounters {
     unsigned long long candidates, prefiltered, patches, fail0, fail1, inserted, replaced, evals, view_evals, trimmed;
     unsigned long long stage[16];
+    unsigned long long pair[6];
 };
 
 struct SweepArgs {
@@ -110,6 +111,7 @@
     uint32_t* cursors;
     const int32_t* job_list;
     const int32_t* list_bounds;
+    int32_t pair;
 };
 
 struct SeedChainArgs {
diff --git a/mvskit_amd/engine.py b/mvskit_amd/engine.py
--- a/mvskit_amd/engine.py
+++ b/mvskit_amd/engine.py
@@ -26,7 +26,7 @@
     "mvs_default_seed_random", "mvs_engine_seed_random", "mvs_engine_seed_random_hypotheses",
     "mvs_default_seed_points", "mvs_engine_seed_points", "mvs_engine_seed_points_hypotheses", "mvs_engine_depth_ranges",
     "mvs_default_maps_config", "mvs_engine_render_maps", "mvs_engine_fused_points",
-    "mvs_engine_tsdf", "mvs_engine_extract_mesh", "mvs_engine_mesh",
+    "mvs_engine_tsdf", "mvs_engine_extract_mesh", "mvs_engine_mesh", "mvs_engine_sweep_pairs",
 ]
 PLY_ASCII, PLY_BINARY_LE = 0, 1
 PLY_VERTEX_DTYPE = np.dtype([("xyz", "<f4", (3,)), ("normal", "<f4", (3,)), ("rgb", "u1", (3,))])
@@ -184,6 +184,8 @@
         L.mvs_default_maps_config.restype = None
         L.mvs_engine_render_maps.argtypes = [vp, C.POINTER(MapsConfig), C.POINTER(ViewMaps), vp]
         L.mvs_engine_fused_points.argtypes = [vp, C.POINTER(MapsConfig), C.c_int64, vp, C.POINTER(C.c_int64)]
+    if hasattr(L, "mvs_engine_sweep_pairs"):
+        L.mvs_engine_sweep_pairs.argtypes = [vp, C.POINTER(C.c_int64)]
     if hasattr(L, "mvs_engine_tsdf"):
         L.mvs_engine_tsdf.argtypes = [vp, C.POINTER(MapsConfig), C.POINTER(Volume), vp, vp]
         L.mvs_engine_extract_mesh.argtypes = [vp, C.POINTER(Volume), vp, vp, C.c_int64, vp, C.c_int64, vp, C.POINTER(C.c_int64), C.POINTER(C.c_int64)]
@@ -532,6 +534,13 @@
                 "exchange_ms": t.exchange_ms, "exchange_bytes": int(t.exchange_bytes), "check_retried_cells": int(t.check_retried_cells),
                 "sweep_jobs_listed": int(t.sweep_jobs_listed)}
 
+    SWEEP_PAIR_KEYS = ("paired", "alone_no_partner", "alone_no_room", "alone_partner_failed", "alone_long_list", "can_pair")
+
+    def sweep_pairs(self):
+        out = (C.c_int64 * 6)()
+        self._check(self.L.mvs_engine_sweep_pairs(self.h, out))
+        return dict(zip(self.SWEEP_PAIR_KEYS, (int(x) for x in out)))
+
     def depth_normal_map(self, view, kind):
         gw, gh = self.grid_dims(view)
         d = np.zeros((gh, gw), np.float32)
```

After: 31.14 million (median of 6 runs). +4.1%, better.
